# ofsouzap/DistributedMandelbrot

Hardware: AMD Instinct MI355X
Metric: G pixel-iterations/s on 4096^2 tile, max_iter=1000 fp64 (higher is better)
Workload: dtype f64

## Files before the change

distributedmandelbrot_amd/_lib.py:

```python
from __future__ import annotations

import ctypes as C
import importlib.util
import os
import sys

HERE = os.path.dirname(os.path.abspath(__file__))
SO_PATH = os.path.join(HERE, "libmbk_hip.so")

MBK_OK, MBK_ERR_INVALID, MBK_ERR_NO_DEVICE, MBK_ERR_HIP, MBK_ERR_NOMEM, MBK_ERR_NET = range(6)
MBK_WANT_COUNTS = 0x1
MBK_WANT_BYTES = 0x2
MBK_KERNEL_DEFAULT = 0x000
MBK_KERNEL_SIMPLE = 0x100
MBK_KERNEL_ASM = 0x200
MBK_KERNEL_REFILL = 0x300
MBK_KERNEL_GROUP = 0x400
MBK_KERNEL_SCAN = 0x500
KERNELS = {"default": MBK_KERNEL_DEFAULT, "simple": MBK_KERNEL_SIMPLE, "asm": MBK_KERNEL_ASM,
           "refill": MBK_KERNEL_REFILL, "group": MBK_KERNEL_GROUP, "scan": MBK_KERNEL_SCAN}
OPTIONS = {name: i for i, name in enumerate(
    ["order", "waves_per_wg", "group_steps", "exact_steps", "probe_steps", "scan_waves", "scan_xcd_map", "scan_col_period", "heavy_share",
     "rf_livemin", "rf_patience", "rf_batch", "rf_waves", "cycle_detect", "probe_mid", "prepass_overlap", "exact_long", "scan_inline", "wave_limit", "units_min_light", "xcd_balance", "m_late", "h_settled", "classify_wg", "scan_strip", "cycle_window", "spill_first", "spill_lanes", "spill_min_mrd", "spill_min_blocks", "spill_cyc_shift"])}
MBK_PRECISION_F32 = 0x1000
MBK_LAZY_UNIFORM = 0x2000
MBK_DEEP_BLA = 0x8000
PRECISIONS = {"f64": 0, "f32": MBK_PRECISION_F32}
MBK_SLOTS = 4
MBK_WORKER_DEPTH = 3
MBK_INFO_SCAN_WG_PER_CU = 100
MBK_INFO_XCD_SHARE = 110
MBK_INFO_SPILL = 130
MBK_CODEC_RAW = 0x00
MBK_CODEC_RLE = 0x01
MBK_CHUNK_DEFINITION = 4096
MBK_CHUNK_BYTES = 4096 * 4096
MBK_ABI_VERSION = 5
MBK_RENDER_BYTES = 0
MBK_RENDER_SMOOTH = 1
MBK_RENDER_DISTANCE = 3
MBK_RENDER_DISTANCE_REL = 4
MBK_RENDER_EQUALIZED = 5
RENDER_SOURCES = {"bytes": MBK_RENDER_BYTES, "smooth": MBK_RENDER_SMOOTH, "distance": MBK_RENDER_DISTANCE,
                  "distance_rel": MBK_RENDER_DISTANCE_REL, "equalized": MBK_RENDER_EQUALIZED}
MBK_HISTOGRAM_MAX_MRD = 1 << 20
RENDER_SUPERSAMPLES = (1, 2, 3, 4, 8)
MBK_RENDER_BAND_BYTES = 256 << 20
MBK_STREAM_OK, MBK_STREAM_BAD_CODEC, MBK_STREAM_BAD_SIZE, MBK_STREAM_ZERO_RUN, MBK_STREAM_TOO_LONG, MBK_STREAM_TOO_SHORT = range(6)
STREAM_REASONS = {MBK_STREAM_OK: "MBK_STREAM_OK", MBK_STREAM_BAD_CODEC: "MBK_STREAM_BAD_CODEC", MBK_STREAM_BAD_SIZE: "MBK_STREAM_BAD_SIZE",
                  MBK_STREAM_ZERO_RUN: "MBK_STREAM_ZERO_RUN", MBK_STREAM_TOO_LONG: "MBK_STREAM_TOO_LONG",
                  MBK_STREAM_TOO_SHORT: "MBK_STREAM_TOO_SHORT"}
CHUNK_SCALES = (1, 2, 4, 8, 16, 32, 64)
MBK_DENSITY_MAX_CELLS = 1 << 28
MBK_DENSITY_LINEAR = 0
MBK_DENSITY_SQRT = 1
DENSITY_MODES = {"linear": MBK_DENSITY_LINEAR, "sqrt": MBK_DENSITY_SQRT}
DENSITY_FACTORS = (1, 2, 4, 8)


class mbk_view(C.Structure):
    _fields_ = [("start_r", C.c_double), ("start_i", C.c_double),
                ("range_r", C.c_double), ("range_i", C.c_double),
                ("width", C.c_uint32), ("height", C.c_uint32),
                ("col0", C.c_uint32), ("row0", C.c_uint32),
                ("ncols", C.c_uint32), ("nrows", C.c_uint32)]


class mbk_deep_view(C.Structure):
    _fields_ = [("range_r", C.c_double), ("range_i", C.c_double),
                ("width", C.c_uint32), ("height", C.c_uint32),
                ("col0", C.c_uint32), ("row0", C.c_uint32),
                ("ncols", C.c_uint32), ("nrows", C.c_uint32)]


class mbk_deep_xview(C.Structure):
    _fields_ = [("range_r", C.c_double), ("range_i", C.c_double), ("exp2", C.c_int32),
                ("width", C.c_uint32), ("height", C.c_uint32),
                ("col0", C.c_uint32), ("row0", C.c_uint32),
                ("ncols", C.c_uint32), ("nrows", C.c_uint32)]


class mbk_render_spec(C.Structure):
    _fields_ = [("source", C.c_uint32), ("supersample", C.c_uint32), ("palette", C.c_void_p),
                ("palette_len", C.c_uint32), ("inside", C.c_uint8 * 4),
                ("scale", C.c_double), ("offset", C.c_double), ("max_band_rows", C.c_uint32)]


class mbk_chunk_spec(C.Structure):
    _fields_ = [("palette", C.c_void_p), ("scale", C.c_uint32)]


class mbk_interior_render_spec(C.Structure):
    _fields_ = [("supersample", C.c_uint32), ("palette", C.c_void_p), ("palette_len", C.c_uint32),
                ("unknown", C.c_uint8 * 4), ("outside", C.c_uint8 * 4), ("scale", C.c_double), ("max_band_rows", C.c_uint32)]


class mbk_density_target(C.Structure):
    _fields_ = [("start_r", C.c_double), ("start_i", C.c_double), ("range_r", C.c_double), ("range_i", C.c_double),
                ("width", C.c_uint32), ("height", C.c_uint32)]


class mbk_density_stats(C.Structure):
    _fields_ = [("deposits", C.c_uint64), ("dropped", C.c_uint64)]


class mbk_density_render_spec(C.Structure):
    _fields_ = [("mode", C.c_uint32), ("factor", C.c_uint32), ("palette", C.c_void_p), ("palette_len", C.c_uint32),
                ("scale", C.c_double), ("offset", C.c_double)]


class mbk_stats(C.Structure):
    _fields_ = [("kernel_ms", C.c_float), ("d2h_ms", C.c_float),
                ("pixel_iterations", C.c_uint64), ("never_pixels", C.c_uint64),
                ("all_bytes_zero", C.c_uint32), ("all_bytes_one", C.c_uint32),
                ("rle_runs", C.c_uint64)]


class mbk_device_info(C.Structure):
    _fields_ = [("name", C.c_char * 128), ("arch", C.c_char * 64),
                ("compute_units", C.c_int), ("clock_mhz", C.c_int),
                ("wavefront_size", C.c_int), ("total_mem", C.c_uint64)]


class mbk_worker_report(C.Structure):
    _fields_ = [("leased", C.c_uint64), ("accepted", C.c_uint64), ("rejected", C.c_uint64), ("resets", C.c_uint64),
                ("uniform_tiles", C.c_uint64), ("pixel_iterations", C.c_uint64),
                ("kernel_ms_sum", C.c_double), ("seconds", C.c_double), ("net_retries", C.c_uint64)]


NET_OPTIONS = {name: i for i, name in enumerate(
    ["max_connections", "connect_timeout_ms", "io_timeout_ms", "retries", "backoff_ms", "stop", "peak_connections", "feeder_slots"])}


FEEDER_SUBMIT = C.CFUNCTYPE(C.c_int, C.c_void_p, C.c_int, C.c_uint32, C.c_uint32, C.c_uint32, C.c_uint32, C.c_void_p)
FEEDER_WAIT = C.CFUNCTYPE(C.c_int, C.c_void_p, C.c_int, C.POINTER(mbk_stats))
FEEDER_ALLOC = C.CFUNCTYPE(C.c_void_p, C.c_void_p, C.c_uint64)
FEEDER_RELEASE = C.CFUNCTYPE(None, C.c_void_p, C.c_void_p)
FEEDER_ON_TILE = C.CFUNCTYPE(None, C.c_void_p, C.POINTER(C.c_uint32 * 4), C.POINTER(mbk_stats), C.c_int)


class mbk_feeder_ops(C.Structure):
    _fields_ = [("user", C.c_void_p), ("submit", FEEDER_SUBMIT), ("wait", FEEDER_WAIT), ("alloc", FEEDER_ALLOC),
                ("release", FEEDER_RELEASE), ("on_tile", FEEDER_ON_TILE)]


SIGNATURES = {
    "mbk_abi_version": (C.c_int, []),
    "mbk_device_count": (C.c_int, [C.POINTER(C.c_int)]),
    "mbk_create": (C.c_int, [C.c_int, C.POINTER(C.c_void_p)]),
    "mbk_destroy": (None, [C.c_void_p]),
    "mbk_last_error": (C.c_char_p, [C.c_void_p]),
    "mbk_get_device_info": (C.c_int, [C.c_void_p, C.POINTER(mbk_device_info)]),
    "mbk_device_pci_bus_id": (C.c_int, [C.c_void_p, C.c_char_p, C.c_int]),
    "mbk_host_alloc": (C.c_int, [C.c_void_p, C.c_uint64, C.POINTER(C.c_void_p)]),
    "mbk_host_free": (C.c_int, [C.c_void_p, C.c_void_p]),
    "mbk_datachunk_geometry": (C.c_int, [C.c_uint32, C.c_uint32, C.c_uint32,
                                         C.POINTER(C.c_double), C.POINTER(C.c_double),
                                         C.POINTER(C.c_double)]),
    "mbk_view_outside_circle": (C.c_int, [C.POINTER(mbk_view), C.c_uint32, C.POINTER(C.c_int)]),
    "mbk_view_needs_literal_doubling": (C.c_int, [C.POINTER(mbk_view), C.c_uint32, C.POINTER(C.c_int)]),
    "mbk_view_launch": (C.c_int, [C.c_void_p, C.POINTER(mbk_view), C.c_uint32, C.c_uint32,
                                  C.c_void_p, C.c_void_p, C.c_void_p]),
    "mbk_view_compute": (C.c_int, [C.c_void_p, C.POINTER(mbk_view), C.c_uint32, C.c_uint32,
                                   C.c_void_p, C.c_void_p, C.POINTER(mbk_stats)]),
    "mbk_datachunk": (C.c_int, [C.c_void_p, C.c_uint32, C.c_uint32, C.c_uint32, C.c_uint32,
                                C.c_void_p, C.c_void_p, C.POINTER(mbk_stats)]),
    "mbk_view_launch_smooth": (C.c_int, [C.c_void_p, C.POINTER(mbk_view), C.c_uint32, C.c_uint32,
                                         C.c_void_p, C.c_void_p, C.c_void_p]),
    "mbk_view_compute_smooth": (C.c_int, [C.c_void_p, C.POINTER(mbk_view), C.c_uint32, C.c_uint32,
                                          C.c_void_p, C.c_void_p, C.POINTER(mbk_stats)]),
    "mbk_view_launch_distance": (C.c_int, [C.c_void_p, C.POINTER(mbk_view), C.c_uint32, C.c_uint32,
                                           C.c_void_p, C.c_void_p, C.c_void_p]),
    "mbk_view_compute_distance": (C.c_int, [C.c_void_p, C.POINTER(mbk_view), C.c_uint32, C.c_uint32,
                                            C.c_void_p, C.c_void_p, C.POINTER(mbk_stats)]),
    "mbk_distance_value_host": (C.c_double, [C.c_double, C.c_double, C.c_int32]),
    "mbk_datachunk_submit": (C.c_int, [C.c_void_p, C.c_int, C.c_uint32, C.c_uint32, C.c_uint32, C.c_uint32,
                                       C.c_void_p, C.c_void_p]),
    "mbk_datachunk_submit_ex": (C.c_int, [C.c_void_p, C.c_int, C.c_uint32, C.c_uint32, C.c_uint32, C.c_uint32,
                                          C.c_void_p, C.c_void_p, C.c_uint32]),
    "mbk_view_submit": (C.c_int, [C.c_void_p, C.c_int, C.POINTER(mbk_view), C.c_uint32, C.c_uint32,
                                  C.c_void_p, C.c_void_p]),
    "mbk_wait": (C.c_int, [C.c_void_p, C.c_int, C.POINTER(mbk_stats)]),
    "mbk_serialize_last": (C.c_int, [C.c_void_p, C.c_void_p, C.c_uint64, C.POINTER(C.c_uint64),
                                     C.POINTER(C.c_uint32)]),
    "mbk_set_option": (C.c_int, [C.c_void_p, C.c_int, C.c_uint32]),
    "mbk_get_option": (C.c_int, [C.c_void_p, C.c_int, C.POINTER(C.c_uint32)]),
    "mbk_quantise_counts": (C.c_int, [C.c_void_p, C.c_void_p, C.c_uint64, C.c_uint32, C.c_void_p]),
    "mbk_units_plan": (C.c_int, [C.c_uint32, C.c_uint32, C.c_uint32, C.c_void_p, C.c_void_p]),
    "mbk_units_lookup": (C.c_int, [C.c_void_p, C.c_uint32, C.c_void_p, C.c_void_p]),
    "mbk_reduce_counts": (C.c_int, [C.c_void_p, C.c_void_p, C.c_uint64, C.c_uint32, C.c_void_p,
                                    C.POINTER(mbk_stats)]),
    "mbk_worker_run": (C.c_int, [C.c_void_p, C.c_char_p, C.c_uint16, C.c_uint64, C.c_uint32,
                                 C.POINTER(mbk_worker_report)]),
    "mbk_net_set_option": (C.c_int, [C.c_int, C.c_uint32]),
    "mbk_net_get_option": (C.c_int, [C.c_int, C.POINTER(C.c_uint32)]),
    "mbk_feeder_run": (C.c_int, [C.POINTER(mbk_feeder_ops), C.c_char_p, C.c_uint16, C.c_uint64, C.c_uint32,
                                 C.POINTER(mbk_worker_report)]),
    "mbk_deep_orbit_create": (C.c_int, [C.c_char_p, C.c_char_p, C.c_uint32, C.c_uint32, C.POINTER(C.c_void_p)]),
    "mbk_deep_orbit_destroy": (None, [C.c_void_p]),
    "mbk_deep_orbit_info": (C.c_int, [C.c_void_p, C.POINTER(C.c_uint32), C.POINTER(C.c_uint32), C.POINTER(C.c_uint32),
                                      C.POINTER(C.c_uint32)]),
    "mbk_deep_orbit_read": (C.c_int, [C.c_void_p, C.c_void_p, C.c_void_p, C.c_uint64]),
    "mbk_deep_view_launch": (C.c_int, [C.c_void_p, C.c_void_p, C.POINTER(mbk_deep_view), C.c_uint32, C.c_uint32,
                                       C.c_void_p, C.c_void_p, C.c_void_p, C.c_void_p]),
    "mbk_deep_view_compute": (C.c_int, [C.c_void_p, C.c_void_p, C.POINTER(mbk_deep_view), C.c_uint32, C.c_uint32,
                                        C.c_void_p, C.c_void_p, C.c_void_p, C.POINTER(mbk_stats)]),
    "mbk_deep_view_submit": (C.c_int, [C.c_void_p, C.c_int, C.c_void_p, C.POINTER(mbk_deep_view), C.c_uint32, C.c_uint32,
                                       C.c_void_p, C.c_void_p]),
    "mbk_deep_view_launch_distance": (C.c_int, [C.c_void_p, C.c_void_p, C.POINTER(mbk_deep_view), C.c_uint32, C.c_uint32,
                                                C.c_void_p, C.c_void_p, C.c_void_p]),
    "mbk_deep_view_compute_distance": (C.c_int, [C.c_void_p, C.c_void_p, C.POINTER(mbk_deep_view), C.c_uint32, C.c_uint32,
                                                 C.c_void_p, C.c_void_p, C.POINTER(mbk_stats)]),
    "mbk_deep_distance_value_host": (C.c_double, [C.c_double, C.c_double, C.c_int32, C.c_double, C.c_int32]),
    "mbk_deep_bla_info": (C.c_int, [C.c_void_p, C.POINTER(mbk_deep_view), C.POINTER(C.c_uint32), C.POINTER(C.c_uint64)]),
    "mbk_deep_bla_read": (C.c_int, [C.c_void_p, C.POINTER(mbk_deep_view), C.c_uint32, C.c_void_p, C.c_void_p, C.c_void_p,
                                    C.c_void_p, C.c_void_p, C.c_uint64]),
    "mbk_deep_bla_count_host": (C.c_int, [C.c_void_p, C.POINTER(mbk_deep_view), C.c_uint32, C.c_uint32, C.c_uint32,
                                          C.POINTER(C.c_int32), C.POINTER(C.c_double), C.POINTER(C.c_uint64)]),
    "mbk_deep_orbit_read_wide": (C.c_int, [C.c_void_p, C.c_void_p, C.c_void_p, C.c_void_p, C.c_uint64]),
    "mbk_deep_xview_launch": (C.c_int, [C.c_void_p, C.c_void_p, C.POINTER(mbk_deep_xview), C.c_uint32, C.c_uint32,
                                        C.c_void_p, C.c_void_p, C.c_void_p, C.c_void_p]),
    "mbk_deep_xview_compute": (C.c_int, [C.c_void_p, C.c_void_p, C.POINTER(mbk_deep_xview), C.c_uint32, C.c_uint32,
                                         C.c_void_p, C.c_void_p, C.c_void_p, C.POINTER(mbk_stats)]),
    "mbk_deep_xview_submit": (C.c_int, [C.c_void_p, C.c_int, C.c_void_p, C.POINTER(mbk_deep_xview), C.c_uint32, C.c_uint32,
                                        C.c_void_p, C.c_void_p]),
    "mbk_deep_xview_count_host": (C.c_int, [C.c_void_p, C.POINTER(mbk_deep_xview), C.c_uint32, C.c_uint32, C.c_uint32,
                                            C.POINTER(C.c_int32), C.POINTER(C.c_double)]),
    "mbk_deep_xview_render_launch": (C.c_int, [C.c_void_p, C.c_void_p, C.POINTER(mbk_deep_xview), C.c_uint32, C.c_uint32,
                                               C.POINTER(mbk_render_spec), C.c_void_p, C.c_void_p]),
    "mbk_deep_xview_render_compute": (C.c_int, [C.c_void_p, C.c_void_p, C.POINTER(mbk_deep_xview), C.c_uint32, C.c_uint32,
                                                C.POINTER(mbk_render_spec), C.c_void_p, C.POINTER(mbk_stats)]),
    "mbk_deep_xview_render_equalized_launch": (C.c_int, [C.c_void_p, C.c_void_p, C.POINTER(mbk_deep_xview), C.c_uint32, C.c_uint32,
                                                         C.POINTER(mbk_render_spec), C.c_void_p, C.c_uint32, C.c_void_p,
                                                         C.c_void_p]),
    "mbk_deep_xview_render_equalized_compute": (C.c_int, [C.c_void_p, C.c_void_p, C.POINTER(mbk_deep_xview), C.c_uint32,
                                                          C.c_uint32, C.POINTER(mbk_render_spec), C.c_void_p, C.c_uint32,
                                                          C.c_void_p, C.POINTER(mbk_stats)]),
    "mbk_deep_xview_histogram_launch": (C.c_int, [C.c_void_p, C.c_void_p, C.POINTER(mbk_deep_xview), C.c_uint32, C.c_uint32,
                                                  C.c_void_p, C.c_void_p]),
    "mbk_deep_xview_histogram_compute": (C.c_int, [C.c_void_p, C.c_void_p, C.POINTER(mbk_deep_xview), C.c_uint32, C.c_uint32,
                                                   C.c_void_p, C.POINTER(mbk_stats)]),
    "mbk_view_render_launch": (C.c_int, [C.c_void_p, C.POINTER(mbk_view), C.c_uint32, C.c_uint32,
                                         C.POINTER(mbk_render_spec), C.c_void_p, C.c_void_p]),
    "mbk_view_render_compute": (C.c_int, [C.c_void_p, C.POINTER(mbk_view), C.c_uint32, C.c_uint32,
                                          C.POINTER(mbk_render_spec), C.c_void_p, C.POINTER(mbk_stats)]),
    "mbk_deep_view_render_launch": (C.c_int, [C.c_void_p, C.c_void_p, C.POINTER(mbk_deep_view), C.c_uint32, C.c_uint32,
                                              C.POINTER(mbk_render_spec), C.c_void_p, C.c_void_p]),
    "mbk_deep_view_render_compute": (C.c_int, [C.c_void_p, C.c_void_p, C.POINTER(mbk_deep_view), C.c_uint32, C.c_uint32,
                                               C.POINTER(mbk_render_spec), C.c_void_p, C.POINTER(mbk_stats)]),
    "mbk_palette_viewer": (C.c_int, [C.c_void_p]),
    "mbk_render_resolve_host": (C.c_int, [C.POINTER(mbk_render_spec), C.c_uint32, C.c_uint32, C.c_void_p, C.c_void_p,
                                          C.c_void_p, C.c_void_p]),
    "mbk_counts_histogram": (C.c_int, [C.c_void_p, C.c_void_p, C.c_uint64, C.c_uint32, C.c_void_p, C.c_void_p]),
    "mbk_view_histogram_launch": (C.c_int, [C.c_void_p, C.POINTER(mbk_view), C.c_uint32, C.c_uint32, C.c_void_p, C.c_void_p]),
    "mbk_deep_view_histogram_launch": (C.c_int, [C.c_void_p, C.c_void_p, C.POINTER(mbk_deep_view), C.c_uint32, C.c_uint32,
                                                 C.c_void_p, C.c_void_p]),
    "mbk_view_histogram_compute": (C.c_int, [C.c_void_p, C.POINTER(mbk_view), C.c_uint32, C.c_uint32, C.c_void_p,
                                             C.POINTER(mbk_stats)]),
    "mbk_deep_view_histogram_compute": (C.c_int, [C.c_void_p, C.c_void_p, C.POINTER(mbk_deep_view), C.c_uint32, C.c_uint32,
                                                  C.c_void_p, C.POINTER(mbk_stats)]),
    "mbk_counts_histogram_host": (C.c_int, [C.c_void_p, C.c_uint64, C.c_uint32, C.c_void_p]),
    "mbk_equalize_lut_host": (C.c_int, [C.c_void_p, C.c_uint32, C.c_void_p]),
    "mbk_equalize_value_host": (C.c_double, [C.c_void_p, C.c_uint32, C.c_double]),
    "mbk_view_render_equalized_launch": (C.c_int, [C.c_void_p, C.POINTER(mbk_view), C.c_uint32, C.c_uint32,
                                                   C.POINTER(mbk_render_spec), C.c_void_p, C.c_uint32, C.c_void_p, C.c_void_p]),
    "mbk_view_render_equalized_compute": (C.c_int, [C.c_void_p, C.POINTER(mbk_view), C.c_uint32, C.c_uint32,
                                                    C.POINTER(mbk_render_spec), C.c_void_p, C.c_uint32, C.c_void_p,
                                                    C.POINTER(mbk_stats)]),
    "mbk_deep_view_render_equalized_launch": (C.c_int, [C.c_void_p, C.c_void_p, C.POINTER(mbk_deep_view), C.c_uint32, C.c_uint32,
                                                        C.POINTER(mbk_render_spec), C.c_void_p, C.c_uint32, C.c_void_p,
                                                        C.c_void_p]),
    "mbk_deep_view_render_equalized_compute": (C.c_int, [C.c_void_p, C.c_void_p, C.POINTER(mbk_deep_view), C.c_uint32, C.c_uint32,
                                                         C.POINTER(mbk_render_spec), C.c_void_p, C.c_uint32, C.c_void_p,
                                                         C.POINTER(mbk_stats)]),
    "mbk_render_resolve_equalized_host": (C.c_int, [C.POINTER(mbk_render_spec), C.c_void_p, C.c_uint32, C.c_uint32, C.c_uint32,
                                                    C.c_void_p, C.c_void_p, C.c_void_p]),
    "mbk_julia_view_launch": (C.c_int, [C.c_void_p, C.POINTER(mbk_view), C.c_double, C.c_double, C.c_uint32, C.c_uint32,
                                        C.c_void_p, C.c_void_p, C.c_void_p, C.c_void_p]),
    "mbk_julia_view_compute": (C.c_int, [C.c_void_p, C.POINTER(mbk_view), C.c_double, C.c_double, C.c_uint32, C.c_uint32,
                                         C.c_void_p, C.c_void_p, C.c_void_p, C.POINTER(mbk_stats)]),
    "mbk_julia_view_submit": (C.c_int, [C.c_void_p, C.c_int, C.POINTER(mbk_view), C.c_double, C.c_double, C.c_uint32, C.c_uint32,
                                        C.c_void_p, C.c_void_p]),
    "mbk_julia_view_render_launch": (C.c_int, [C.c_void_p, C.POINTER(mbk_view), C.c_double, C.c_double, C.c_uint32, C.c_uint32,
                                               C.POINTER(mbk_render_spec), C.c_void_p, C.c_void_p]),
    "mbk_julia_view_render_compute": (C.c_int, [C.c_void_p, C.POINTER(mbk_view), C.c_double, C.c_double, C.c_uint32, C.c_uint32,
                                                C.POINTER(mbk_render_spec), C.c_void_p, C.POINTER(mbk_stats)]),
    "mbk_julia_view_render_equalized_launch": (C.c_int, [C.c_void_p, C.POINTER(mbk_view), C.c_double, C.c_double, C.c_uint32,
                                                         C.c_uint32, C.POINTER(mbk_render_spec), C.c_void_p, C.c_uint32,
                                                         C.c_void_p, C.c_void_p]),
    "mbk_julia_view_render_equalized_compute": (C.c_int, [C.c_void_p, C.POINTER(mbk_view), C.c_double, C.c_double, C.c_uint32,
                                                          C.c_uint32, C.POINTER(mbk_render_spec), C.c_void_p, C.c_uint32,
                                                          C.c_void_p, C.POINTER(mbk_stats)]),
    "mbk_julia_view_histogram_launch": (C.c_int, [C.c_void_p, C.POINTER(mbk_view), C.c_double, C.c_double, C.c_uint32, C.c_uint32,
                                                  C.c_void_p, C.c_void_p]),
    "mbk_julia_view_histogram_compute": (C.c_int, [C.c_void_p, C.POINTER(mbk_view), C.c_double, C.c_double, C.c_uint32, C.c_uint32,
                                                   C.c_void_p, C.POINTER(mbk_stats)]),
    "mbk_julia_count_host": (C.c_int, [C.c_double, C.c_double, C.c_double, C.c_double, C.c_uint32, C.POINTER(C.c_int32),
                                       C.POINTER(C.c_double)]),
    "mbk_view_interior_launch": (C.c_int, [C.c_void_p, C.POINTER(mbk_view), C.c_uint32, C.c_uint32, C.c_void_p, C.c_void_p,
                                           C.c_void_p, C.c_void_p]),
    "mbk_view_interior_compute": (C.c_int, [C.c_void_p, C.POINTER(mbk_view), C.c_uint32, C.c_uint32, C.c_void_p, C.c_void_p,
                                            C.c_void_p, C.POINTER(mbk_stats)]),
    "mbk_interior_host": (C.c_int, [C.c_double, C.c_double, C.c_uint32, C.POINTER(C.c_int32), C.POINTER(C.c_int32),
                                    C.POINTER(C.c_int32), C.POINTER(C.c_double)]),
    "mbk_view_interior_render_launch": (C.c_int, [C.c_void_p, C.POINTER(mbk_view), C.c_uint32, C.c_uint32,
                                                  C.POINTER(mbk_interior_render_spec), C.c_void_p, C.c_void_p]),
    "mbk_view_interior_render_compute": (C.c_int, [C.c_void_p, C.POINTER(mbk_view), C.c_uint32, C.c_uint32,
                                                   C.POINTER(mbk_interior_render_spec), C.c_void_p, C.POINTER(mbk_stats)]),
    "mbk_interior_resolve_host": (C.c_int, [C.POINTER(mbk_interior_render_spec), C.c_uint32, C.c_uint32, C.c_void_p, C.c_void_p,
                                            C.c_void_p, C.c_void_p]),
    "mbk_view_density_launch": (C.c_int, [C.c_void_p, C.POINTER(mbk_view), C.POINTER(mbk_density_target), C.c_uint32, C.c_uint32,
                                          C.c_uint32, C.c_uint32, C.c_void_p, C.c_void_p]),
    "mbk_view_density_compute": (C.c_int, [C.c_void_p, C.POINTER(mbk_view), C.POINTER(mbk_density_target), C.c_uint32, C.c_uint32,
                                           C.c_uint32, C.c_uint32, C.c_void_p, C.POINTER(mbk_stats),
                                           C.POINTER(mbk_density_stats)]),
    "mbk_density_max": (C.c_int, [C.c_void_p, C.c_void_p, C.c_uint64, C.POINTER(C.c_uint32), C.POINTER(C.c_uint64), C.c_void_p]),
    "mbk_density_render_launch": (C.c_int, [C.c_void_p, C.c_void_p, C.c_uint32, C.c_uint32, C.POINTER(mbk_density_render_spec),
                                            C.c_void_p, C.c_void_p]),
    "mbk_density_render_compute": (C.c_int, [C.c_void_p, C.c_void_p, C.c_uint32, C.c_uint32, C.POINTER(mbk_density_render_spec),
                                             C.c_void_p, C.POINTER(mbk_stats)]),
    "mbk_density_cell_host": (C.c_int, [C.POINTER(mbk_density_target), C.c_double, C.c_double, C.POINTER(C.c_uint32),
                                        C.POINTER(C.c_uint32), C.POINTER(C.c_int)]),
    "mbk_density_accumulate_host": (C.c_int, [C.POINTER(mbk_view), C.POINTER(mbk_density_target), C.c_uint32, C.c_uint32, C.c_uint32,
                                              C.c_void_p, C.POINTER(mbk_density_stats)]),
    "mbk_density_resolve_host": (C.c_int, [C.POINTER(mbk_density_render_spec), C.c_uint32, C.c_uint32, C.c_void_p, C.c_void_p]),
    "mbk_density_build_info": (C.c_int, []),
    "mbk_chunk_stream_check": (C.c_int, [C.c_void_p, C.c_uint64, C.c_uint64, C.POINTER(C.c_uint32), C.POINTER(C.c_uint64),
                                         C.POINTER(C.c_uint32)]),
    "mbk_chunk_decode_host": (C.c_int, [C.c_void_p, C.c_uint64, C.c_uint64, C.c_void_p]),
    "mbk_chunk_resolve_host": (C.c_int, [C.POINTER(mbk_chunk_spec), C.c_void_p, C.c_void_p, C.c_uint64]),
    "mbk_chunk_decode_launch": (C.c_int, [C.c_void_p, C.c_void_p, C.c_uint64, C.c_uint64, C.c_void_p, C.c_void_p, C.c_void_p]),
    "mbk_chunk_render_launch": (C.c_int, [C.c_void_p, C.c_void_p, C.c_uint64, C.POINTER(mbk_chunk_spec), C.c_void_p, C.c_uint64,
                                          C.c_void_p, C.c_void_p]),
    "mbk_chunk_decode_compute": (C.c_int, [C.c_void_p, C.c_void_p, C.c_uint64, C.c_uint64, C.c_void_p, C.POINTER(mbk_stats)]),
    "mbk_chunk_render_compute": (C.c_int, [C.c_void_p, C.c_void_p, C.c_uint64, C.POINTER(mbk_chunk_spec), C.c_void_p, C.c_uint64,
                                           C.POINTER(mbk_stats)]),
}

_lib = None


def _share_hip_runtime_with_torch() -> None:
# ... 35 lines not shown
```

distributedmandelbrot_amd/csrc/mbk_api.hip:

```cpp
#include "../../include/mbk.h"

#include <hip/hip_runtime.h>

#include <cmath>
#include <cstdio>
#include <cstdlib>
#include <algorithm>
#include <cstring>
#include <new>
#include <string>
#include <vector>

#include "mbk_kernels.h"
#include "mbk_refill.h"
#include "mbk_persist.h"
#include "mbk_scan.h"
#include "mbk_units.h"
#include "mbk_spill.h"
#include "mbk_feeder.h"
#include "mbk_deep_orbit.h"
#include "mbk_deep.h"
#include "mbk_deep_bla.h"
#include "mbk_deep_wide.h"
#include "mbk_histogram.h"
#include "mbk_render.h"
#include "mbk_chunks.h"
#include "mbk_distance.h"
#include "mbk_interior.h"
#include "mbk_deep_distance.h"
#include "mbk_julia.h"
#include "mbk_density.h"

using mbk::Axis;
using mbk::ReduceOut;
using mbk::ReduceSlot;
using mbk::TileArgs;
using mbk::WorkQueues;

static const int kOrderRing = 3;

struct OrderRing {
    uint32_t *d_order[kOrderRing] = {};
    uint32_t *d_ctl = nullptr;
    bool ctl_dirty = true;
    size_t order_cap = 0;
    unsigned order_turn = 0;
    hipStream_t aux = nullptr;
    uint32_t aux_prio = 0;
    int pp_last = -1;
    hipEvent_t ev_cls[kOrderRing] = {};
    hipEvent_t ev_done[kOrderRing] = {};
    bool done_valid[kOrderRing] = {};

    void drop_lists()
    {
        for (int k = 0; k < kOrderRing; ++k) {
            if (d_order[k]) (void)hipFree(d_order[k]);
            d_order[k] = nullptr;
            done_valid[k] = false;
        }
        order_cap = 0;
    }
    void drop_aux()
    {
        if (aux) (void)hipStreamDestroy(aux);
        aux = nullptr;
        for (int k = 0; k < kOrderRing; ++k) {
            if (ev_cls[k]) (void)hipEventDestroy(ev_cls[k]);
            if (ev_done[k]) (void)hipEventDestroy(ev_done[k]);
            ev_cls[k] = ev_done[k] = nullptr;
            done_valid[k] = false;
        }
    }
    void release()
    {
        if (aux) (void)hipStreamSynchronize(aux);
        drop_lists();
        drop_aux();
        if (d_ctl) (void)hipFree(d_ctl);
        *this = OrderRing();
    }
};

struct SpillBuffers {
    void *d_z = nullptr;
    uint32_t *d_meta = nullptr, *d_cnt = nullptr, *d_chunks = nullptr, *d_src = nullptr;
    unsigned long long *d_total = nullptr;
    size_t cap_slots = 0, cap_blocks = 0;

    void release()
    {
        for (void *q : {d_z, (void *)d_meta, (void *)d_cnt, (void *)d_chunks, (void *)d_src, (void *)d_total})
            if (q) (void)hipFree(q);
        *this = SpillBuffers();
    }
};

struct StreamScratch {
    hipStream_t stream = nullptr;
    OrderRing ring;
    WorkQueues *d_queues = nullptr;
    mbk::ScanCursors *d_cursors = nullptr;
    uint32_t *d_entries = nullptr;
    size_t scan_cap_blocks = 0;
    unsigned scan_turn = 0;
    bool cursors_dirty = false;
    uint32_t *h_hint = nullptr;
    SpillBuffers spill;
    ReduceSlot *d_red = nullptr;
    ReduceSlot *h_red = nullptr;
    unsigned long long *h_stamps = nullptr;
    double xcd_f[8] = {0.125, 0.125, 0.125, 0.125, 0.125, 0.125, 0.125, 0.125};
    uint32_t xcd_issued = 0, xcd_consumed = 0;
    struct SharesUsed { uint32_t seq, switches; float f[8]; } xcd_ring[64] = {};
    void *d_render = nullptr;
    size_t render_cap = 0;
    uint32_t *d_palette = nullptr;
    std::vector<uint32_t> palette;
    uint8_t *d_chunk = nullptr;
    size_t chunk_cap_n = 0;
    uint8_t *d_chunk_bytes = nullptr;
    uint32_t *h_chunk_status = nullptr;
    int32_t *d_dist_counts = nullptr;
    size_t dist_cap_px = 0;
    double *d_lut = nullptr;
    size_t lut_cap = 0;
    std::vector<double> lut;
    uint32_t *d_density_bands = nullptr;
    mbk::DensityMax *d_density_max = nullptr;
};
static const size_t kMaxStreamScratch = 64;
static const uint32_t kStampSlots = 16, kShareRing = 64;

struct Slot {
    hipStream_t stream = nullptr;
    hipEvent_t ev_k0 = nullptr, ev_k1 = nullptr, ev_c0 = nullptr, ev_c1 = nullptr;
    int32_t *d_counts = nullptr;
    uint8_t *d_bytes = nullptr;
    size_t cap_px = 0;
    ReduceSlot *d_red = nullptr;
    ReduceSlot *h_red = nullptr;
    bool busy = false;
    bool with_bytes = false;
    uint8_t *lazy_h_bytes = nullptr;
    size_t lazy_px = 0;
    bool immediate = false;
    mbk_stats imm = {};
};

struct mbk_ctx {
    int device = -1;
    Slot s[MBK_SLOTS];
    std::vector<StreamScratch> scratch;
    size_t last_px = 0;
    double *d_smooth = nullptr;
    size_t smooth_cap_px = 0;
    uint32_t *d_rgba = nullptr;
    size_t rgba_cap_px = 0;
    unsigned long long *d_hist = nullptr;
    size_t hist_cap = 0;
    uint32_t *d_density = nullptr;
    size_t density_cap = 0;
    unsigned long long *d_density_stat = nullptr;
    uint8_t *d_rle = nullptr;
    size_t rle_cap_px = 0;
    uint32_t opt[MBK_OPT_COUNT_];
    hipStream_t last_tile_stream = nullptr;
    uint32_t stream_switches = 0;
    int scan_occ[2][2] = {{0, 0}, {0, 0}};
    int scan_occ_inline[2] = {0, 0};
    uint32_t wave_limit_lds[8] = {0, 0, 0, 0, 0, 0, 0, 0};
    uint32_t spill_launches = 0;
    hipStream_t last_spill_stream = nullptr;
    struct ProbeKey { Axis re, im; uint32_t col0, row0, ncols, nrows; } probe_key = {};
    double probe_share = 0.0;
    bool probe_valid = false;
    struct DeepCopy {
        uint64_t id;
        double4 *d;
        mbk::WideEntry *d_wide;
        bool has_bla;
        uint64_t dcmax_bits;
        double *d_rc;
        double4 *d_ab;
        uint32_t levels;
        uint32_t off[mbk::kBlaMaxLevels];
    };
    std::vector<DeepCopy> deep;
    hipDeviceProp_t prop;
    std::string err;
};

struct mbk_deep_orbit {
    mbk::DeepOrbit o;
};

static thread_local std::string g_err;

static int fail(mbk_ctx *ctx, int code, const std::string &msg)
{
    if (ctx) ctx->err = msg;
    g_err = msg;
    return code;
}

#define MBK_HIP(ctx, call)                                                                  \
    do {                                                                                    \
        hipError_t e_ = (call);                                                             \
        if (e_ != hipSuccess) {                                                             \
            return fail((ctx), MBK_ERR_HIP,                                                 \
                        std::string(#call) + ": " + hipGetErrorString(e_));                 \
        }                                                                                   \
    } while (0)


static Axis make_axis(double start, double range, uint32_t n)
{
    Axis a;
    std::memset(&a, 0, sizeof(a));
    a.start = start;
    a.n = n;
    volatile double stop = start + range;
    if (n <= 1) {
        a.last = start;
        a.div = 1.0;
        return a;
    }
    volatile double delta = stop - start;
    volatile double div = (double)(n - 1);
    volatile double step = delta / div;
    a.last = stop;
    a.delta = delta;
    a.div = div;
    a.step = step;
    a.step_is_zero = (step == 0.0) ? 1u : 0u;
    return a;
}

static double axis_value_host(const Axis &a, uint32_t k)
{
    if (k + 1u == a.n) return a.last;
    volatile double y;
    if (a.step_is_zero) {
        volatile double q = (double)k / a.div;
        y = q * a.delta;
    } else {
        y = (double)k * a.step;
    }
    volatile double v = y + a.start;
    return v;
}

static bool axis_end_is_regular(const Axis &a)
{
    if (a.n <= 1 || a.step_is_zero) return false;
    volatile double y = (double)(a.n - 1u) * a.step;
    volatile double v = y + a.start;
    return v == a.last;
}

static const double kMaxCoord = 0x1p500;
static const double kSafeImagMin = 0x1p-900;

static uint32_t coprime_multiplier(uint32_t n)
{
    if (n < 4) return 1u;
    uint64_t m = (uint64_t)((double)n * 0.6180339887498949);
    if (m < 1) m = 1;
    for (;; ++m) {
        uint64_t a = m, b = n;
        while (b) {
            const uint64_t t = a % b;
            a = b;
            b = t;
        }
        if (a == 1) return (uint32_t)(m % n);
    }
}

static bool axis_has_tiny_nonzero(const Axis &a, uint32_t k0, uint32_t cnt, bool f32)
{
    const double thr = f32 ? 0x1p-100 : kSafeImagMin;
    auto value = [&](uint32_t k) { const double y = axis_value_host(a, k); return f32 ? (double)(float)y : y; };
    auto tiny = [&](double y) { return y != 0.0 && std::fabs(y) < thr; };
    if (cnt == 0) return false;
    uint32_t end = k0 + cnt;
    if (a.n >= 1u && end == a.n) {
        if (tiny(value(a.n - 1u))) return true;
        if (--end == k0) return false;
    }
    const double first = value(k0), last = value(end - 1u);
    if (tiny(first) || tiny(last)) return true;
    if ((first > 0.0 && last > 0.0) || (first < 0.0 && last < 0.0) || first == last) return false;
    const double s = last > first ? 1.0 : -1.0;
    auto lower = [&](bool strict) {
        uint32_t lo = k0, hi = end;
        while (lo < hi) {
            const uint32_t mid = lo + (hi - lo) / 2u;
            const double y = s * value(mid);
            if (strict ? y > 0.0 : y >= 0.0) hi = mid;
            else lo = mid + 1u;
        }
        return lo;
    };
    const uint32_t ge = lower(false), gt = lower(true);
    if (ge > k0 && tiny(value(ge - 1u))) return true;
    if (gt < end && tiny(value(gt))) return true;
    return false;
}

static int validate_view(mbk_ctx *ctx, const mbk_view *v, bool *safe_doubling, bool f32 = false)
{
    if (!v) return fail(ctx, MBK_ERR_INVALID, "view is NULL");
    if (v->width == 0 || v->height == 0) return fail(ctx, MBK_ERR_INVALID, "empty view");
    if (v->ncols == 0 || v->nrows == 0) return fail(ctx, MBK_ERR_INVALID, "empty window");
    if ((uint64_t)v->col0 + v->ncols > v->width || (uint64_t)v->row0 + v->nrows > v->height)
        return fail(ctx, MBK_ERR_INVALID, "window exceeds the view");
    if ((uint64_t)v->ncols * v->nrows > (1ull << 31))
        return fail(ctx, MBK_ERR_INVALID, "window larger than 2^31 pixels");
    const double vals[6] = {v->start_r, v->start_i, v->range_r, v->range_i,
                            v->start_r + v->range_r, v->start_i + v->range_i};
    const double max_coord = f32 ? 0x1p60 : kMaxCoord;
    for (double x : vals)
        if (!std::isfinite(x) || std::fabs(x) > max_coord)
            return fail(ctx, MBK_ERR_INVALID, f32 ? "view coordinates must be finite and |x| <= 2^60 (fp32)"
// ... 13 lines not shown

static void free_scratch(StreamScratch &sc)
{
    sc.ring.release();
    sc.spill.release();
    if (sc.d_queues) (void)hipFree(sc.d_queues);
    if (sc.d_cursors) (void)hipFree(sc.d_cursors);
    if (sc.d_entries) (void)hipFree(sc.d_entries);
    if (sc.h_hint) (void)hipHostFree(sc.h_hint);
    if (sc.h_stamps) (void)hipHostFree(sc.h_stamps);
    if (sc.d_red) (void)hipFree(sc.d_red);
    if (sc.h_red) (void)hipHostFree(sc.h_red);
    if (sc.d_render) (void)hipFree(sc.d_render);
    if (sc.d_palette) (void)hipFree(sc.d_palette);
    if (sc.d_chunk) (void)hipFree(sc.d_chunk);
    if (sc.d_chunk_bytes) (void)hipFree(sc.d_chunk_bytes);
    if (sc.h_chunk_status) (void)hipHostFree(sc.h_chunk_status);
    if (sc.d_dist_counts) (void)hipFree(sc.d_dist_counts);
    if (sc.d_lut) (void)hipFree(sc.d_lut);
    if (sc.d_density_bands) (void)hipFree(sc.d_density_bands);
    if (sc.d_density_max) (void)hipFree(sc.d_density_max);
    sc = StreamScratch();
}

static int get_scratch(mbk_ctx *ctx, hipStream_t stream, StreamScratch **out)
{
    for (StreamScratch &sc : ctx->scratch)
        if (sc.stream == stream) {
            *out = &sc;
            return MBK_OK;
        }
    if (ctx->scratch.size() >= kMaxStreamScratch) {
        MBK_HIP(ctx, hipDeviceSynchronize());
        for (StreamScratch &sc : ctx->scratch) free_scratch(sc);
        ctx->scratch.clear();
    }
    ctx->scratch.emplace_back();
    StreamScratch &sc = ctx->scratch.back();
    sc.stream = stream;
    *out = &sc;
    MBK_HIP(ctx, hipHostMalloc((void **)&sc.h_hint, 2 * sizeof(uint32_t), hipHostMallocDefault));
    sc.h_hint[0] = sc.h_hint[1] = 0xffffffffu;
    return MBK_OK;
}

static void set_window_facts(TileArgs &a, bool f32);
static void shares_from_fractions(const double *f, uint32_t *cum);
static double window_heavy_share(const TileArgs &a);
static double window_heavy_share(mbk_ctx *ctx, const TileArgs &a);

static void xcd_shares_update(const mbk_ctx *ctx, StreamScratch &sc)
{
    const unsigned long long kMask = 0xffffffffffffull;
    uint32_t first = sc.xcd_issued >= kStampSlots ? sc.xcd_issued - kStampSlots + 1u : 1u;
    first = std::max(first, sc.xcd_consumed + 1u);
    for (uint32_t c = first; c <= sc.xcd_issued; ++c) {
        const volatile unsigned long long *st = sc.h_stamps + (size_t)(c % kStampSlots) * mbk::kStampWords;
        const StreamScratch::SharesUsed &used = sc.xcd_ring[c % kShareRing];
        if (used.seq != c) continue;
        const StreamScratch::SharesUsed &before = sc.xcd_ring[(c - 1u) % kShareRing], &after = sc.xcd_ring[(c + 1u) % kShareRing];
        const bool alone = c > 1u && before.seq == c - 1u && before.switches == used.switches &&
                           (c == sc.xcd_issued ? ctx->stream_switches == used.switches : after.seq == c + 1u && after.switches == used.switches);
        unsigned long long v[mbk::kStampWords];
        bool whole = true;
        for (uint32_t i = 0; i < mbk::kStampWords; ++i) {
            v[i] = st[i];
            whole = whole && (v[i] >> 48) == (c & 0xffffu);
        }
        if (!whole) continue;
        unsigned long long start = v[0] & kMask;
        for (uint32_t x = 1; x < 8u; ++x)
            if ((((v[x] & kMask) - start) & kMask) >> 47) start = v[x] & kMask;
        double T[8], tmin = 1e300, tmax = 0.0, speed[8], sum = 0.0;
        for (uint32_t x = 0; x < 8u; ++x) {
            unsigned long long last = 0;
            for (uint32_t t = 0; t < mbk::kStampTail; ++t)
                last = std::max(last, ((v[8u + x * mbk::kStampTail + t] & kMask) - start) & kMask);
            T[x] = (double)last;
            tmin = std::min(tmin, T[x]);
            tmax = std::max(tmax, T[x]);
        }
        sc.xcd_consumed = c;
        if (!alone || tmin < 1000.0 || tmax > 1.25 * tmin) continue;
        for (uint32_t x = 0; x < 8u; ++x) {
            speed[x] = (double)used.f[x] / T[x];
            sum += speed[x];
        }
        double fs = 0.0;
        for (uint32_t x = 0; x < 8u; ++x) {
            const double f = 0.7 * sc.xcd_f[x] + 0.3 * speed[x] / sum;
            sc.xcd_f[x] = std::min(0.14, std::max(0.11, f));
            fs += sc.xcd_f[x];
        }
        for (uint32_t x = 0; x < 8u; ++x) sc.xcd_f[x] /= fs;
    }
}

struct FuseStats { ReduceSlot *slots; bool counts_unwanted; bool fused; };

static uint32_t quant_table4(int32_t mrd, bool want_bytes)
{
    uint32_t qtab = 0u;
    if (want_bytes && mrd > 0)
        for (uint32_t c = 1; c <= 4u; ++c)
            qtab |= (uint32_t)(((uint64_t)c * 256u + (uint32_t)mrd - 1u) / (uint32_t)mrd & 0xffu) << (8u * (c - 1u));
    return qtab;
}

struct BlockLaunchPlan {
    uint32_t wpw, by;
    dim3 grid, block;
    uint32_t order_mode, probe_steps;
    bool cyc, units, ordered;
    double unit_share;
};

static BlockLaunchPlan block_launch_plan(mbk_ctx *ctx, TileArgs &a, uint32_t kernel, bool safe, bool f32)
{
    BlockLaunchPlan p;
    p.wpw = ctx->opt[MBK_OPT_WAVES_PER_WG];
    a.blocks_x = (a.ncols + 8u * p.wpw - 1u) / (8u * p.wpw);
    p.by = (a.nrows + 7u) / 8u;
    set_window_facts(a, f32);
    p.cyc = ctx->opt[MBK_OPT_CYCLE_DETECT] != 0u;
    p.grid = dim3(a.blocks_x * p.by);
    p.block = dim3(64u * p.wpw);
    p.order_mode = ctx->opt[MBK_OPT_ORDER];
    p.probe_steps = ctx->opt[MBK_OPT_PROBE_STEPS];
    a.perm_mul = p.order_mode == 1 ? coprime_multiplier(p.grid.x) : 1u;
    a.order = nullptr;
    p.units = p.order_mode == 3 && p.wpw == 1u && kernel == MBK_KERNEL_GROUP && !safe && a.smooth == nullptr &&
              (a.counts || a.bytes) && !(a.bytes && a.quant_wide) && a.blocks_x % 8u == 0u && a.blocks_x <= 2048u &&
              a.fast_bx_end > 0u && a.fast_by_end > 0u && (f32 || ctx->opt[MBK_OPT_GROUP_STEPS] == 16u) &&
              p.grid.x >= 16384u && (uint32_t)a.mrd > 2u * p.probe_steps && p.by <= 0xffffu;
    p.unit_share = 0.0;
    if (p.units) {
        p.unit_share = window_heavy_share(ctx, a);
        p.units = (1.0 - p.unit_share) * 65536.0 >= (double)ctx->opt[MBK_OPT_UNITS_MIN_LIGHT];
    }
    p.ordered = p.order_mode >= 2 && p.grid.x >= 16384u && (uint32_t)a.mrd > 2u * p.probe_steps && a.blocks_x <= 0xffffu && p.by <= 0xffffu;
    return p;
}

struct OrderList {
    StreamScratch *sc = nullptr;
    unsigned k = 0;
    uint32_t *list = nullptr;
    hipStream_t pre = nullptr;
    bool overlap = false;
    bool whole = false;
    ~OrderList() { if (sc && !whole) sc->ring.ctl_dirty = true; }
};

static int acquire_order_list(mbk_ctx *ctx, hipStream_t stream, uint32_t nblocks, OrderList *out)
{
    StreamScratch *sc = nullptr;
    int rc = get_scratch(ctx, stream, &sc);
    if (rc != MBK_OK) return rc;
    OrderRing &ring = sc->ring;
    const uint32_t pp_mode = ctx->opt[MBK_OPT_PREPASS_OVERLAP];
    const bool overlap = pp_mode != 0u;
    const uint32_t want_prio = pp_mode == 2u ? 2u : 1u;
    if (ring.pp_last != (int)pp_mode) {
        if (ring.pp_last >= 0) {
            MBK_HIP(ctx, hipStreamSynchronize(stream));
            if (ring.aux) MBK_HIP(ctx, hipStreamSynchronize(ring.aux));
        }
        for (int k = 0; k < kOrderRing; ++k) ring.done_valid[k] = false;
        ring.pp_last = (int)pp_mode;
    }
    if (overlap && ring.aux && ring.aux_prio != want_prio) {
        MBK_HIP(ctx, hipStreamSynchronize(stream));
        MBK_HIP(ctx, hipStreamSynchronize(ring.aux));
        ring.drop_aux();
    }
    if (overlap && !ring.aux) {
        if (want_prio == 2u) {
            int least = 0, greatest = 0;
            MBK_HIP(ctx, hipDeviceGetStreamPriorityRange(&least, &greatest));
            MBK_HIP(ctx, hipStreamCreateWithPriority(&ring.aux, hipStreamNonBlocking, greatest));
        } else {
            MBK_HIP(ctx, hipStreamCreateWithFlags(&ring.aux, hipStreamNonBlocking));
        }
        ring.aux_prio = want_prio;
        for (int k = 0; k < kOrderRing; ++k) {
            MBK_HIP(ctx, hipEventCreateWithFlags(&ring.ev_cls[k], hipEventDisableTiming));
            MBK_HIP(ctx, hipEventCreateWithFlags(&ring.ev_done[k], hipEventDisableTiming));
        }
    }
    if (nblocks > ring.order_cap) {
        MBK_HIP(ctx, hipStreamSynchronize(stream));
        if (ring.aux) MBK_HIP(ctx, hipStreamSynchronize(ring.aux));
        ring.drop_lists();
        for (int k = 0; k < kOrderRing; ++k)
            MBK_HIP(ctx, hipMalloc((void **)&ring.d_order[k], mbk::units_list_words(nblocks) * sizeof(uint32_t)));
        ring.order_cap = nblocks;
    }
    const unsigned k = ring.order_turn++ % (unsigned)kOrderRing;
    if (overlap && ring.done_valid[k]) MBK_HIP(ctx, hipStreamWaitEvent(ring.aux, ring.ev_done[k], 0));
    out->k = k;
    out->list = ring.d_order[k];
    out->pre = overlap ? ring.aux : stream;
    out->overlap = overlap;
    out->sc = sc;
    return MBK_OK;
}

static int enqueue_units_prepass(mbk_ctx *ctx, TileArgs &a, const BlockLaunchPlan &p, const OrderList &ol, hipStream_t stream)
{
    StreamScratch *sc = ol.sc;
    OrderRing &ring = sc->ring;
    const uint32_t hs = p.cyc ? ctx->opt[MBK_OPT_H_SETTLED] : 0u;
    const double settle_thr = hs ? std::pow(10.0, -(double)hs) : 0.0;
    if (!ring.d_ctl) {
        MBK_HIP(ctx, hipMalloc((void **)&ring.d_ctl, (size_t)kOrderRing * 8u * sizeof(uint32_t)));
        ring.ctl_dirty = true;
    }
    if (ring.ctl_dirty) {
        if (ring.aux) MBK_HIP(ctx, hipStreamSynchronize(ring.aux));
        MBK_HIP(ctx, hipStreamSynchronize(stream));
        MBK_HIP(ctx, hipMemsetAsync(ring.d_ctl, 0, (size_t)kOrderRing * 8u * sizeof(uint32_t), ol.pre));
        ring.ctl_dirty = false;
    }
    uint32_t *ctl = ring.d_ctl + 8u * ol.k;
    const uint32_t balance = ctx->opt[MBK_OPT_XCD_BALANCE] == 1u && (p.cyc || ctx->prop.multiProcessorCount != 256)
                                 ? 0u : ctx->opt[MBK_OPT_XCD_BALANCE];
    static const double kUneven[8] = {0.110, 0.140, 0.125, 0.120, 0.130, 0.125, 0.115, 0.135};
    if (balance == 1u && !sc->h_stamps) {
        MBK_HIP(ctx, hipHostMalloc((void **)&sc->h_stamps, (size_t)kStampSlots * mbk::kStampWords * sizeof(unsigned long long),
                                   hipHostMallocDefault));
        std::memset(sc->h_stamps, 0xff, (size_t)kStampSlots * mbk::kStampWords * sizeof(unsigned long long));
    }
    if (balance == 1u) xcd_shares_update(ctx, *sc);
    mbk::XcdShares w;
    double f[8];
    const uint32_t seq = ++sc->xcd_issued;
    StreamScratch::SharesUsed &used = sc->xcd_ring[seq % kShareRing];
    used.seq = seq;
    used.switches = ctx->stream_switches;
    for (uint32_t x = 0; x < 8u; ++x) {
        f[x] = balance == 1u ? sc->xcd_f[x] : (balance == 2u ? kUneven[x] : 0.125);
        used.f[x] = (float)f[x];
    }
    shares_from_fractions(f, w.cum);
    a.plan = ol.list + ((2u * (size_t)p.grid.x + 5u + 15u) & ~(size_t)15u);
    a.stamps = balance == 1u ? sc->h_stamps + (size_t)(seq % kStampSlots) * mbk::kStampWords : nullptr;
    a.stamp_tag = seq & 0xffffu;
    const uint32_t cwg = ctx->opt[MBK_OPT_CLASSIFY_WG];
    hipLaunchKernelGGL(mbk::classify_units_kernel, dim3((p.grid.x + cwg - 1u) / cwg), dim3(cwg), 0, ol.pre, a, p.grid.x,
                       (int32_t)p.probe_steps, ol.list, ctl, (int32_t)ctx->opt[MBK_OPT_M_LATE], settle_thr, ctl + 3, (uint32_t *)a.plan, w,
                       a.stamps ? 1u : 0u);
    return MBK_OK;
}

static int enqueue_classify_prepass(mbk_ctx *ctx, const TileArgs &a, const BlockLaunchPlan &p, const OrderList &ol, bool *mid_first)
{
    const uint32_t nblocks = p.grid.x;
    uint32_t *cursors = ol.list + nblocks;
    MBK_HIP(ctx, hipMemsetAsync(cursors, 0, 3 * sizeof(uint32_t), ol.pre));
    *mid_first = p.order_mode == 3 && ctx->opt[MBK_OPT_PROBE_MID] > p.probe_steps && ctx->opt[MBK_OPT_M_LATE] >= 2u &&
                 ctx->opt[MBK_OPT_M_LATE] <= p.probe_steps;
    hipLaunchKernelGGL(mbk::classify_blocks_kernel, dim3((nblocks + 1023u) / 1024u), dim3(1024), 0, ol.pre, a,
                       nblocks, 8u * p.wpw, (int32_t)p.probe_steps, (int32_t)(*mid_first ? ctx->opt[MBK_OPT_M_LATE] : ctx->opt[MBK_OPT_PROBE_MID]),
                       ol.list, cursors);
    return MBK_OK;
}

static bool spill_wanted(const mbk_ctx *ctx, const TileArgs &a, const BlockLaunchPlan &p, uint32_t kernel, bool safe, bool f32)
{
    const uint32_t spill_first = ctx->opt[MBK_OPT_SPILL_FIRST], spill_lanes = ctx->opt[MBK_OPT_SPILL_LANES];
    return !p.units && a.order != nullptr && p.order_mode >= 2u && kernel == MBK_KERNEL_GROUP && !safe && a.smooth == nullptr && p.wpw == 1u &&
           (a.counts || a.bytes) && spill_first != 0u && (f32 || ctx->opt[MBK_OPT_GROUP_STEPS] == 16u) &&
           (uint32_t)a.mrd >= ctx->opt[MBK_OPT_SPILL_MIN_MRD] && (uint32_t)a.mrd < (1u << 26) &&
           ((uint64_t)p.grid.x >> ctx->opt[MBK_OPT_SPILL_MIN_BLOCKS]) != 0ull &&
           (uint64_t)a.mrd > (uint64_t)ctx->opt[MBK_OPT_EXACT_STEPS] + spill_first + 66u &&
           (uint64_t)p.grid.x * spill_lanes < (1ull << 32) && a.fast_bx_end > 0u && a.fast_by_end > 0u;
}

static int acquire_spill(mbk_ctx *ctx, StreamScratch *sc, hipStream_t stream, TileArgs &a, uint32_t nblocks, SpillBuffers **out)
{
    SpillBuffers &sp = sc->spill;
    const uint32_t spill_lanes = ctx->opt[MBK_OPT_SPILL_LANES];
    const size_t slots = (size_t)nblocks * spill_lanes, nchunks = (nblocks + mbk::kSpillChunk - 1u) / mbk::kSpillChunk;
    *out = nullptr;
    if (slots > sp.cap_slots || nblocks > sp.cap_blocks) {
        MBK_HIP(ctx, hipStreamSynchronize(stream));
        sp.release();
        const bool got = hipMalloc(&sp.d_z, slots * 16u) == hipSuccess &&
                         hipMalloc((void **)&sp.d_meta, slots * sizeof(uint32_t)) == hipSuccess &&
                         hipMalloc((void **)&sp.d_src, slots * sizeof(uint32_t)) == hipSuccess &&
                         hipMalloc((void **)&sp.d_cnt, (size_t)nblocks * sizeof(uint32_t)) == hipSuccess &&
                         hipMalloc((void **)&sp.d_chunks, (nchunks * mbk::kSpillLevels + 1u) * sizeof(uint32_t)) == hipSuccess &&
                         hipMalloc((void **)&sp.d_total, sizeof(unsigned long long)) == hipSuccess;
        if (got) {
            sp.cap_slots = slots;
            sp.cap_blocks = nblocks;
        } else {
            (void)hipGetLastError();
            sp.release();
        }
    }
    if (sp.cap_slots >= slots && sp.cap_blocks >= nblocks && sp.d_z) {
        a.spill_first = ctx->opt[MBK_OPT_SPILL_FIRST];
        a.spill_lanes = spill_lanes;
        a.spill_win_shift = ctx->opt[MBK_OPT_SPILL_CYC_SHIFT];
        a.spill_z = sp.d_z;
        a.spill_meta = sp.d_meta;
        a.spill_cnt = sp.d_cnt;
        MBK_HIP(ctx, hipMemsetAsync(sp.d_cnt, 0, (size_t)nblocks * sizeof(uint32_t), stream));
        *out = &sp;
    }
    return MBK_OK;
}

typedef void (*UnitsKernel)(TileArgs, uint32_t);
typedef void (*BlockKernel)(TileArgs);
typedef void (*SpillKernel)(TileArgs, const uint32_t *, const unsigned long long *, uint32_t);

static UnitsKernel pick_units_kernel(bool f32, bool cyc, bool stats, bool counts, bool bytes)
{
    static const UnitsKernel forms[4][4] = {
        {mbk::tile_units_kernel<float, 8, true, false, true, true>, mbk::tile_units_kernel<float, 8, true, true, true>,
         mbk::tile_units_kernel<float, 8, true, false, true>, mbk::tile_units_kernel<float, 8, true, true, false>},
        {mbk::tile_units_kernel<float, 8, false, false, true, true>, mbk::tile_units_kernel<float, 8, false, true, true>,
         mbk::tile_units_kernel<float, 8, false, false, true>, mbk::tile_units_kernel<float, 8, false, true, false>},
        {mbk::tile_units_kernel<double, 16, true, false, true, true>, mbk::tile_units_kernel<double, 16, true, true, true>,
         mbk::tile_units_kernel<double, 16, true, false, true>, mbk::tile_units_kernel<double, 16, true, true, false>},
        {mbk::tile_units_kernel<double, 16, false, false, true, true>, mbk::tile_units_kernel<double, 16, false, true, true>,
         mbk::tile_units_kernel<double, 16, false, false, true>, mbk::tile_units_kernel<double, 16, false, true, false>},
    };
    return forms[(f32 ? 0 : 2) + (cyc ? 0 : 1)][stats ? 0 : (counts && bytes) ? 1 : bytes ? 2 : 3];
}

static BlockKernel pick_block_kernel(uint32_t kernel, bool safe, bool f32, bool cyc, uint32_t group_steps, bool spill)
{
    if (spill && f32 && cyc) return mbk::tile_asm_kernel<float, true, 8, true, true>;
    if (spill && f32) return mbk::tile_asm_kernel<float, true, 8, false, true>;
    if (spill && cyc) return mbk::tile_asm_kernel<double, true, 16, true, true>;
    if (spill) return mbk::tile_asm_kernel<double, true, 16, false, true>;
    if (f32 && safe) return mbk::tile_asm_kernel<float, false, 0>;
    if (f32 && kernel == MBK_KERNEL_ASM) return mbk::tile_asm_kernel<float, true, 0>;
    if (f32 && cyc) return mbk::tile_asm_kernel<float, true, 8, true>;
    if (f32) return mbk::tile_asm_kernel<float, true, 8>;
    if (safe) return mbk::tile_asm_kernel<double, false, 0>;
    if (kernel == MBK_KERNEL_ASM) return mbk::tile_asm_kernel<double, true, 0>;
    if (group_steps == 32 && !cyc) return mbk::tile_asm_kernel<double, true, 32>;
    if (group_steps >= 16 && cyc) return mbk::tile_asm_kernel<double, true, 16, true>;
    if (group_steps >= 16) return mbk::tile_asm_kernel<double, true, 16>;
    if (group_steps == 8 && cyc) return mbk::tile_asm_kernel<double, true, 8, true>;
    if (group_steps == 8) return mbk::tile_asm_kernel<double, true, 8>;
    return mbk::tile_asm_kernel<double, true, 4>;
}

static SpillKernel pick_spill_kernels(bool f32, bool cyc)
{
    if (f32 && cyc) return mbk::tile_spill_kernel<float, true>;
    if (f32) return mbk::tile_spill_kernel<float, false>;
    if (cyc) return mbk::tile_spill_kernel<double, true>;
    return mbk::tile_spill_kernel<double, false>;
}

static void enqueue_units_tile(mbk_ctx *ctx, TileArgs &a, const BlockLaunchPlan &p, bool f32, uint32_t lds, hipStream_t stream, FuseStats *fuse)
{
    const double est = (double)p.grid.x * (p.unit_share + (1.0 - p.unit_share) / 8.0);
    const uint32_t cus = (uint32_t)ctx->prop.multiProcessorCount;
    uint32_t g = (uint32_t)std::min<double>((double)p.grid.x, est * 1.15 + 2048.0);
    g = (std::max(std::max(g, std::min(p.grid.x, cus * 64u)), 16384u) + 7u) & ~7u;
    a.unit_stride = g;
    const bool stats = fuse != nullptr && fuse->slots != nullptr && fuse->counts_unwanted && a.bytes != nullptr;
    if (stats) {
        a.stats = fuse->slots;
        a.counts = nullptr;
        fuse->fused = true;
    }
    hipLaunchKernelGGL(pick_units_kernel(f32, p.cyc, stats, a.counts != nullptr, a.bytes != nullptr), dim3(g), dim3(64), lds, stream, a,
                       quant_table4(a.mrd, a.bytes != nullptr));
}

static int enqueue_spill_second_pass(mbk_ctx *ctx, const TileArgs &a, const SpillBuffers &sp, uint32_t nblocks, bool f32, bool cyc, hipStream_t stream)
{
    const uint32_t nchunks = (nblocks + mbk::kSpillChunk - 1u) / mbk::kSpillChunk;
    hipLaunchKernelGGL(mbk::spill_count_kernel, dim3(nchunks), dim3(mbk::kSpillChunk), 0, stream, sp.d_cnt, nblocks, nchunks, sp.d_chunks);
    hipLaunchKernelGGL(mbk::rle_scan_kernel, dim3(1), dim3(1024), 0, stream, sp.d_chunks, nchunks * mbk::kSpillLevels, sp.d_total);
    hipLaunchKernelGGL(mbk::spill_expand_kernel, dim3(nchunks), dim3(mbk::kSpillChunk), 0, stream, sp.d_cnt, nblocks, nchunks,
                       sp.d_chunks, a.spill_lanes, sp.d_src);
    const uint32_t nwg = (uint32_t)std::min<uint64_t>(((uint64_t)nblocks * a.spill_lanes + 63u) / 64u, 16384u);
    const uint32_t lds2 = 0u;
    hipLaunchKernelGGL(pick_spill_kernels(f32, cyc), dim3(nwg), dim3(64), lds2, stream, a, sp.d_src, sp.d_total, nwg);
    MBK_HIP(ctx, hipGetLastError());
    ++ctx->spill_launches;
    ctx->last_spill_stream = stream;
    return MBK_OK;
}

static int launch_blocks(mbk_ctx *ctx, TileArgs a, uint32_t kernel, bool safe, bool f32, hipStream_t stream, FuseStats *fuse = nullptr)
{
    const BlockLaunchPlan p = block_launch_plan(ctx, a, kernel, safe, f32);
    OrderList ol;
    if (p.ordered) {
        int rc = acquire_order_list(ctx, stream, p.grid.x, &ol);
        if (rc != MBK_OK) return rc;
        OrderRing &ring = ol.sc->ring;
        bool mid_first = false;
        rc = p.units ? enqueue_units_prepass(ctx, a, p, ol, stream) : enqueue_classify_prepass(ctx, a, p, ol, &mid_first);
        if (rc != MBK_OK) return rc;
        if (ol.overlap) {
            MBK_HIP(ctx, hipEventRecord(ring.ev_cls[ol.k], ring.aux));
            MBK_HIP(ctx, hipStreamWaitEvent(stream, ring.ev_cls[ol.k], 0));
        }
        a.order = ol.list;
        a.ngrid = p.grid.x;
        a.order_mid = mid_first ? 2u : (ctx->opt[MBK_OPT_PROBE_MID] <= p.probe_steps ? 1u : 0u);
    }
    SpillBuffers *spill = nullptr;
    if (spill_wanted(ctx, a, p, kernel, safe, f32)) {
        const int rc = acquire_spill(ctx, ol.sc, stream, a, p.grid.x, &spill);
        if (rc != MBK_OK) return rc;
    }
    const uint32_t lds = p.wpw == 1u ? ctx->wave_limit_lds[ctx->opt[MBK_OPT_WAVE_LIMIT] & 7u] : 0u;
    if (p.units && a.order)
        enqueue_units_tile(ctx, a, p, f32, lds, stream, fuse);
    else
        hipLaunchKernelGGL(pick_block_kernel(kernel, safe, f32, p.cyc, ctx->opt[MBK_OPT_GROUP_STEPS], spill != nullptr), p.grid, p.block, lds, stream, a);
    const hipError_t e = hipGetLastError();
    if (e != hipSuccess) return fail(ctx, MBK_ERR_HIP, std::string("tile launch: ") + hipGetErrorString(e));
    if (ol.overlap) {
        MBK_HIP(ctx, hipEventRecord(ol.sc->ring.ev_done[ol.k], stream));
        ol.sc->ring.done_valid[ol.k] = true;
    }
    if (spill) {
        const int rc = enqueue_spill_second_pass(ctx, a, *spill, p.grid.x, f32, p.cyc, stream);
        if (rc != MBK_OK) return rc;
    }
    ol.whole = true;
    return MBK_OK;
}

static bool window_may_touch_ring(const TileArgs &a, double margin = 1e-6)
{
    const double x0 = axis_value_host(a.re, a.col0), x1 = axis_value_host(a.re, a.col0 + a.ncols - 1u);
    const double y0 = axis_value_host(a.im, a.row0), y1 = axis_value_host(a.im, a.row0 + a.nrows - 1u);
    const double xlo = std::fmin(x0, x1), xhi = std::fmax(x0, x1), ylo = std::fmin(y0, y1), yhi = std::fmax(y0, y1);
    const double dx = (xlo <= 0.0 && 0.0 <= xhi) ? 0.0 : std::fmin(std::fabs(xlo), std::fabs(xhi));
    const double dy = (ylo <= 0.0 && 0.0 <= yhi) ? 0.0 : std::fmin(std::fabs(ylo), std::fabs(yhi));
    const double fx = std::fmax(std::fabs(xlo), std::fabs(xhi)), fy = std::fmax(std::fabs(ylo), std::fabs(yhi));
    const double rmin2 = dx * dx + dy * dy, rmax2 = fx * fx + fy * fy;
    return !(rmax2 < 4.0 - margin || rmin2 > 4.0 + margin);
}

static void set_window_facts(TileArgs &a, bool f32)
{
    a.ring_possible = window_may_touch_ring(a, f32 ? 2e-3 : 1e-6) ? 1u : 0u;
    a.fast_bx_end = a.fast_by_end = 0u;
    if (a.re.step_is_zero || a.im.step_is_zero) return;
    const uint64_t re_n = (uint64_t)a.re.n - (axis_end_is_regular(a.re) ? 0u : 1u), im_n = (uint64_t)a.im.n - (axis_end_is_regular(a.im) ? 0u : 1u);
    const uint64_t cols_ok = std::min<uint64_t>(a.ncols, re_n - std::min<uint64_t>(a.col0, re_n));
    const uint64_t rows_ok = std::min<uint64_t>(a.nrows, im_n - std::min<uint64_t>(a.row0, im_n));
    a.fast_bx_end = (uint32_t)(cols_ok / 8u);
    a.fast_by_end = (uint32_t)(rows_ok / 8u);
}

static int launch_refill(mbk_ctx *ctx, const TileArgs &a, bool safe, hipStream_t stream)
{
    const bool eligible = !safe && a.mrd >= 2 && a.counts != nullptr && !a.re.step_is_zero &&
                          !a.im.step_is_zero && !window_may_touch_ring(a, 1e-6);
    const uint32_t cols_ok = a.re.n > 0 ? std::min<uint64_t>(a.ncols, (uint64_t)(a.re.n - 1u) - std::min<uint64_t>(a.col0, a.re.n - 1u)) : 0u;
    const uint32_t rows_ok = a.im.n > 0 ? std::min<uint64_t>(a.nrows, (uint64_t)(a.im.n - 1u) - std::min<uint64_t>(a.row0, a.im.n - 1u)) : 0u;
    const uint32_t icols = eligible ? (cols_ok / 8u) * 8u : 0u, irows = eligible ? (rows_ok / 8u) * 8u : 0u;
    if (icols == 0 || irows == 0) return launch_blocks(ctx, a, MBK_KERNEL_GROUP, safe, false, stream);

    mbk::PersistArgs q;
    std::memset(&q, 0, sizeof(q));
    q.re_start = a.re.start;
    q.re_step = a.re.step;
    q.im_start = a.im.start;
    q.im_step = a.im.step;
    q.col0 = a.col0;
    q.row0 = a.row0;
    q.pitch = a.out_pitch;
    q.bxn = icols / 8u;
    q.nblocks = q.bxn * (irows / 8u);
    q.total = (uint32_t)a.mrd - 1u;
    q.livemin = ctx->opt[MBK_OPT_RF_LIVEMIN];
    q.patience = ctx->opt[MBK_OPT_RF_PATIENCE];
    q.batch = ctx->opt[MBK_OPT_RF_BATCH];
    q.counts = a.counts;
    StreamScratch *sc = nullptr;
    int rcs = get_scratch(ctx, stream, &sc);
    if (rcs != MBK_OK) return rcs;
    if (!sc->d_queues) MBK_HIP(ctx, hipMalloc((void **)&sc->d_queues, sizeof(WorkQueues)));
    WorkQueues *wq = sc->d_queues;
    hipLaunchKernelGGL(mbk::init_queues_kernel, dim3(1), dim3(64), 0, stream, wq, q.nblocks);
    uint32_t waves = (uint32_t)ctx->prop.multiProcessorCount * 4u * ctx->opt[MBK_OPT_RF_WAVES];
    if (waves > q.nblocks) waves = q.nblocks;
    hipLaunchKernelGGL(mbk::tile_persist_kernel, dim3((waves + 3u) / 4u), dim3(256), 0, stream, q, wq);
    MBK_HIP(ctx, hipGetLastError());
    TileArgs e = a;
    e.bytes = nullptr;
    if (icols < a.ncols) {
        e.col0 = a.col0 + icols;
        e.ncols = a.ncols - icols;
        e.out_col0 = a.out_col0 + icols;
        int rc = launch_blocks(ctx, e, MBK_KERNEL_GROUP, safe, false, stream);
        if (rc != MBK_OK) return rc;
    }
    if (irows < a.nrows) {
        e = a;
        e.bytes = nullptr;
        e.ncols = icols;
        e.row0 = a.row0 + irows;
        e.nrows = a.nrows - irows;
        e.out_row0 = a.out_row0 + irows;
        int rc = launch_blocks(ctx, e, MBK_KERNEL_GROUP, safe, false, stream);
        if (rc != MBK_OK) return rc;
    }
    if (a.bytes) {
        const uint64_t npx = (uint64_t)a.ncols * a.nrows;
        hipLaunchKernelGGL(mbk::quantise_kernel, dim3(2048), dim3(256), 0, stream, a.counts, a.bytes, npx, a.mrd,
                           a.quant_wide, a.quant_rcp);
        MBK_HIP(ctx, hipGetLastError());
    }
    return MBK_OK;
}

static double window_heavy_share(const TileArgs &a)
{
    const uint32_t k = 16;
    uint32_t inside = 0;
    for (uint32_t j = 0; j < k; ++j) {
        const double ci = axis_value_host(a.im, a.row0 + (uint32_t)(((uint64_t)(2u * j + 1u) * a.nrows) / (2u * k)));
        for (uint32_t i = 0; i < k; ++i) {
            const double cr = axis_value_host(a.re, a.col0 + (uint32_t)(((uint64_t)(2u * i + 1u) * a.ncols) / (2u * k)));
            double zr = cr, zi = ci;
            bool in = true;
            for (int n = 0; n < 4 && in; ++n) {
                const double t = zr * zr - zi * zi + cr;
                zi = 2.0 * zr * zi + ci;
                zr = t;
                in = zr * zr + zi * zi < 4.0;
            }
            inside += in ? 1u : 0u;
        }
    }
    return (double)inside / (double)(k * k);
}

static double window_heavy_share(mbk_ctx *ctx, const TileArgs &a)
{
    mbk_ctx::ProbeKey k;
    std::memset(&k, 0, sizeof(k));
    k.re = a.re;
    k.im = a.im;
    k.col0 = a.col0;
    k.row0 = a.row0;
    k.ncols = a.ncols;
    k.nrows = a.nrows;
    if (ctx->probe_valid && std::memcmp(&k, &ctx->probe_key, sizeof(k)) == 0) return ctx->probe_share;
// ... 466 lines not shown
        case Target::kDeep: set_geometry(p.deep, p.g); break;
        case Target::kJulia:
        case Target::kPlain: set_geometry(p.view, p.g); break;
    }
    return p;
}

struct BandPlan {
    uint32_t ncols, nrows, tile_cols, band_rows;
    size_t cap_px() const { return (size_t)tile_cols * band_rows; }
};

static BandPlan band_plan(uint32_t ncols, uint32_t nrows, uint64_t bytes_per_px, uint32_t max_rows = 0u)
{
    const uint64_t budget = MBK_RENDER_BAND_BYTES - 1024u;
    BandPlan p = {ncols, nrows, ncols, 1u};
    if ((uint64_t)ncols * bytes_per_px <= budget)
        p.band_rows = (uint32_t)std::min<uint64_t>(nrows, budget / ((uint64_t)ncols * bytes_per_px));
    else
        p.tile_cols = (uint32_t)(budget / bytes_per_px);
    if (max_rows) p.band_rows = std::min(p.band_rows, max_rows);
    return p;
}

template <typename Piece>
static int for_each_band(mbk_ctx *ctx, const BandPlan &p, const int32_t *d_counts, uint64_t samples_per_px, uint32_t mrd,
                         hipStream_t stream, Slot *stat, Piece piece)
{
    for (uint32_t r = 0; r < p.nrows; r += p.band_rows) {
        const uint32_t nr = std::min(p.band_rows, p.nrows - r);
        for (uint32_t c = 0; c < p.ncols; c += p.tile_cols) {
            const uint32_t nc = std::min(p.tile_cols, p.ncols - c);
            const bool is_last = r + nr == p.nrows && c + nc == p.ncols;
            int rc = piece(r, c, nr, nc, is_last);
            if (rc != MBK_OK) return rc;
            if (stat) {
                if (is_last) MBK_HIP(ctx, hipEventRecord(stat->ev_k1, stream));
                rc = launch_reduce(ctx, stat->d_red, stat->h_red, d_counts, nullptr, (uint64_t)nc * nr * samples_per_px, mrd, stream, false);
                if (rc != MBK_OK) return rc;
            }
        }
    }
    return MBK_OK;
}


static double deep_step(double range, uint32_t n)
{
    if (n <= 1u) return 0.0;
    volatile double s = range / (double)(n - 1u);
    return s;
}

static double deep_dc(uint32_t k, uint32_t n, double range)
{
    volatile double dc = ((double)k - (double)(n - 1u) * 0.5) * deep_step(range, n);
    return dc;
}

template <typename V>
static bool deep_ranges_within(const V *v, double lo)
{
    for (double r : {v->range_r, v->range_i})
        if (!std::isfinite(r) || !(r >= lo) || !(r <= 4.0)) return false;
    return true;
}

template <typename V, typename FlagRules, typename RangeRules>
static int validate_deep_view(mbk_ctx *ctx, const mbk_deep_orbit *orbit, const V *v, uint32_t mrd, uint32_t flags, FlagRules flag_rules,
                              RangeRules range_rules)
{
    if (!orbit) return fail(ctx, MBK_ERR_INVALID, "orbit is NULL");
    if (!v) return fail(ctx, MBK_ERR_INVALID, "view is NULL");
    int rc = flag_rules();
    if (rc != MBK_OK) return rc;
    if (v->width == 0 || v->height == 0) return fail(ctx, MBK_ERR_INVALID, "empty view");
    if (v->ncols == 0 || v->nrows == 0) return fail(ctx, MBK_ERR_INVALID, "empty window");
    if ((uint64_t)v->col0 + v->ncols > v->width || (uint64_t)v->row0 + v->nrows > v->height)
        return fail(ctx, MBK_ERR_INVALID, "window exceeds the view");
    if ((uint64_t)v->ncols * v->nrows > (1ull << 31)) return fail(ctx, MBK_ERR_INVALID, "window larger than 2^31 pixels");
    rc = range_rules();
    if (rc != MBK_OK) return rc;
    if (mrd > orbit->o.mrd) return fail(ctx, MBK_ERR_INVALID, "mrd exceeds the mrd the reference orbit was computed for");
    if ((flags & MBK_WANT_BYTES) && mrd == 0) return fail(ctx, MBK_ERR_INVALID, "mrd == 0 has no quantised form (division by zero)");
    return MBK_OK;
}

template <typename Args, typename V>
static void fill_deep_window(Args &a, const V *v, uint32_t mrd)
{
    a.half_r = (double)(v->width - 1u) * 0.5;
    a.half_i = (double)(v->height - 1u) * 0.5;
    a.step_r = deep_step(v->range_r, v->width);
    a.step_i = deep_step(v->range_i, v->height);
    a.col0 = v->col0;
    a.row0 = v->row0;
    a.ncols = v->ncols;
    a.nrows = v->nrows;
    a.blocks_x = (v->ncols + 7u) / 8u;
    a.mrd = (int32_t)mrd;
}

template <typename Args>
static void fill_outputs(Args &a, uint32_t mrd, int32_t *d_counts, uint8_t *d_bytes, double *d_smooth)
{
    a.quant_wide = (mrd >= (1u << 23)) ? 1u : 0u;
    a.quant_rcp = mrd ? 1.0 / (double)mrd : 0.0;
    a.counts = d_counts;
    a.bytes = d_bytes;
    a.smooth = d_smooth;
}

template <typename Args>
static dim3 block_grid(const Args &a) { return dim3(a.blocks_x * ((a.nrows + 7u) / 8u)); }


extern "C" {

int mbk_abi_version(void) { return MBK_ABI_VERSION; }

int mbk_device_count(int *count)
{
    if (!count) return fail(nullptr, MBK_ERR_INVALID, "count is NULL");
    int n = 0;
    hipError_t e = hipGetDeviceCount(&n);
    if (e != hipSuccess) {
        *count = 0;
        return fail(nullptr, MBK_ERR_NO_DEVICE, std::string("hipGetDeviceCount: ") + hipGetErrorString(e));
    }
    *count = n;
    return MBK_OK;
}

int mbk_create(int device, mbk_ctx **out)
{
    if (!out) return fail(nullptr, MBK_ERR_INVALID, "out is NULL");
    *out = nullptr;
    int n = 0;
    hipError_t e = hipGetDeviceCount(&n);
    if (e != hipSuccess || n <= 0)
        return fail(nullptr, MBK_ERR_NO_DEVICE,
                    std::string("no HIP device visible (") + hipGetErrorString(e) +
                        "); libmbk_hip has no CPU fallback");
    if (device < 0 || device >= n) return fail(nullptr, MBK_ERR_NO_DEVICE, "device index out of range");
    mbk_ctx *ctx = new (std::nothrow) mbk_ctx();
    if (!ctx) return fail(nullptr, MBK_ERR_NOMEM, "out of host memory");
    ctx->device = device;
    static const uint32_t kDefaults[MBK_OPT_COUNT_] = {
         3u,  1u,  16u,  8u,  32u,
         8u,  1u,  4u,  655u,
         48u,  256u,  1u,  8u,  1u,
         65537u,  1u,  0u,  1u,  0u,
         32768u,  0u,  8u,  6u,  1024u,
         1u,  32u,  256u,  16u,  2048u,  19u,  5u};
    std::memcpy(ctx->opt, kDefaults, sizeof(kDefaults));
#define MBK_CREATE_HIP(call)                                                        \
    do {                                                                            \
        hipError_t e2_ = (call);                                                    \
        if (e2_ != hipSuccess) {                                                    \
            fail(nullptr, MBK_ERR_HIP, std::string(#call) + ": " + hipGetErrorString(e2_)); \
            mbk_destroy(ctx);                                                       \
            return MBK_ERR_HIP;                                                     \
        }                                                                           \
    } while (0)
    MBK_CREATE_HIP(hipSetDevice(device));
    MBK_CREATE_HIP(hipGetDeviceProperties(&ctx->prop, device));
    if (std::strncmp(ctx->prop.gcnArchName, "gfx950", 6) != 0) {
        fail(nullptr, MBK_ERR_NO_DEVICE,
             std::string("device is ") + ctx->prop.gcnArchName + ", this library is built for gfx950 only");
        mbk_destroy(ctx);
        return MBK_ERR_NO_DEVICE;
    }
    for (Slot &sl : ctx->s) {
        MBK_CREATE_HIP(hipStreamCreateWithFlags(&sl.stream, hipStreamNonBlocking));
        MBK_CREATE_HIP(hipEventCreate(&sl.ev_k0));
        MBK_CREATE_HIP(hipEventCreate(&sl.ev_k1));
        MBK_CREATE_HIP(hipEventCreate(&sl.ev_c0));
        MBK_CREATE_HIP(hipEventCreate(&sl.ev_c1));
        MBK_CREATE_HIP(hipMalloc((void **)&sl.d_red, sizeof(ReduceSlot) * mbk::kReduceSlots));
        MBK_CREATE_HIP(hipHostMalloc((void **)&sl.h_red, sizeof(ReduceSlot) * mbk::kReduceSlots, hipHostMallocDefault));
    }
    {
        const void *fns[2][2] = {{(const void *)mbk::tile_light_kernel<double, true, true>, (const void *)mbk::tile_todo_kernel<double>},
                                 {(const void *)mbk::tile_light_kernel<float, true, true>, (const void *)mbk::tile_todo_kernel<float>}};
        for (int f = 0; f < 2; ++f)
            for (int k = 0; k < 2; ++k) {
                int n = 0;
                MBK_CREATE_HIP(hipOccupancyMaxActiveBlocksPerMultiprocessor(&n, fns[f][k], 64, 0));
                ctx->scan_occ[f][k] = n > 0 ? n : 1;
            }
        const void *fi[2][6] = {{(const void *)mbk::tile_light_kernel<double, true, true, 2>, (const void *)mbk::tile_light_kernel<double, true, true, 1>,
                                 (const void *)mbk::tile_light_kernel<double, true, true, 2, true>, (const void *)mbk::tile_light_kernel<double, false, true, 2, true>,
                                 (const void *)mbk::tile_light_kernel<double, true, false, 2, true>, (const void *)mbk::tile_light_kernel<double, true, false, 1>},
                                {(const void *)mbk::tile_light_kernel<float, true, true, 2>, (const void *)mbk::tile_light_kernel<float, true, true, 1>,
                                 (const void *)mbk::tile_light_kernel<float, true, true, 2, true>, (const void *)mbk::tile_light_kernel<float, false, true, 2, true>,
                                 (const void *)mbk::tile_light_kernel<float, true, false, 2, true>, (const void *)mbk::tile_light_kernel<float, true, false, 1>}};
        for (int f = 0; f < 2; ++f) {
            int least = 0;
            for (int k = 0; k < 6; ++k) {
                int n = 0;
                MBK_CREATE_HIP(hipOccupancyMaxActiveBlocksPerMultiprocessor(&n, fi[f][k], 64, 0));
                n = n > 0 ? n : 1;
                least = (k == 0 || n < least) ? n : least;
            }
            ctx->scan_occ_inline[f] = least;
        }
    }
    {
        const void *fn = (const void *)mbk::tile_asm_kernel<double, true, 16, false>;
        for (int k = 1; k <= 7; ++k) {
            uint32_t lo = 0, hi = 65536;
            int n = 0;
            MBK_CREATE_HIP(hipOccupancyMaxActiveBlocksPerMultiprocessor(&n, fn, 64, hi));
            if (n > 4 * k) {
                ctx->wave_limit_lds[k] = hi;
                continue;
            }
            while (hi - lo > 64) {
                const uint32_t mid = (lo + hi) / 2;
                MBK_CREATE_HIP(hipOccupancyMaxActiveBlocksPerMultiprocessor(&n, fn, 64, mid));
                if (n > 4 * k) lo = mid;
                else hi = mid;
            }
            ctx->wave_limit_lds[k] = hi;
        }
    }
#undef MBK_CREATE_HIP
    *out = ctx;
    return MBK_OK;
}

void mbk_destroy(mbk_ctx *ctx)
{
    if (!ctx) return;
    if (ctx->device >= 0) (void)hipSetDevice(ctx->device);
    for (Slot &sl : ctx->s) {
        if (sl.stream) (void)hipStreamSynchronize(sl.stream);
        if (sl.d_counts) (void)hipFree(sl.d_counts);
        if (sl.d_bytes) (void)hipFree(sl.d_bytes);
        if (sl.d_red) (void)hipFree(sl.d_red);
        if (sl.h_red) (void)hipHostFree(sl.h_red);
        if (sl.ev_k0) (void)hipEventDestroy(sl.ev_k0);
        if (sl.ev_k1) (void)hipEventDestroy(sl.ev_k1);
        if (sl.ev_c0) (void)hipEventDestroy(sl.ev_c0);
        if (sl.ev_c1) (void)hipEventDestroy(sl.ev_c1);
        if (sl.stream) (void)hipStreamDestroy(sl.stream);
    }
    if (!ctx->scratch.empty() || !ctx->deep.empty()) (void)hipDeviceSynchronize();
    for (StreamScratch &sc : ctx->scratch) free_scratch(sc);
    for (mbk_ctx::DeepCopy &c : ctx->deep) free_deep_copy(c);
    if (ctx->d_rle) (void)hipFree(ctx->d_rle);
    if (ctx->d_smooth) (void)hipFree(ctx->d_smooth);
    if (ctx->d_rgba) (void)hipFree(ctx->d_rgba);
    if (ctx->d_hist) (void)hipFree(ctx->d_hist);
    if (ctx->d_density) (void)hipFree(ctx->d_density);
    if (ctx->d_density_stat) (void)hipFree(ctx->d_density_stat);
    delete ctx;
}

const char *mbk_last_error(const mbk_ctx *ctx) { return ctx ? ctx->err.c_str() : g_err.c_str(); }

int mbk_get_device_info(mbk_ctx *ctx, mbk_device_info *info)
{
    if (!ctx || !info) return fail(ctx, MBK_ERR_INVALID, "NULL argument");
    std::memset(info, 0, sizeof(*info));
    std::snprintf(info->name, sizeof(info->name), "%s", ctx->prop.name);
    std::snprintf(info->arch, sizeof(info->arch), "%s", ctx->prop.gcnArchName);
    info->compute_units = ctx->prop.multiProcessorCount;
    info->clock_mhz = ctx->prop.clockRate / 1000;
    info->wavefront_size = ctx->prop.warpSize;
    info->total_mem = ctx->prop.totalGlobalMem;
    return MBK_OK;
}

int mbk_device_pci_bus_id(mbk_ctx *ctx, char *buf, int len)
{
    if (!ctx || !buf || len < 16) return fail(ctx, MBK_ERR_INVALID, "buffer of at least 16 bytes needed");
    MBK_HIP(ctx, hipDeviceGetPCIBusId(buf, len, ctx->device));
    return MBK_OK;
}

int mbk_host_alloc(mbk_ctx *ctx, uint64_t bytes, void **out)
{
    if (!ctx || !out || bytes == 0) return fail(ctx, MBK_ERR_INVALID, "bad argument");
    MBK_HIP(ctx, hipSetDevice(ctx->device));
    MBK_HIP(ctx, hipHostMalloc(out, bytes, hipHostMallocDefault));
    return MBK_OK;
}

int mbk_host_free(mbk_ctx *ctx, void *ptr)
{
    if (!ctx) return fail(ctx, MBK_ERR_INVALID, "ctx is NULL");
    if (!ptr) return MBK_OK;
    MBK_HIP(ctx, hipSetDevice(ctx->device));
    MBK_HIP(ctx, hipHostFree(ptr));
    return MBK_OK;
}

int mbk_datachunk_geometry(uint32_t level, uint32_t index_real, uint32_t index_imag,
                           double *start_r, double *start_i, double *range)
{
    if (!start_r || !start_i || !range) return fail(nullptr, MBK_ERR_INVALID, "NULL output pointer");
    if (level == 0) return fail(nullptr, MBK_ERR_INVALID, "level must be > 0 (DataChunk.cs:99-100)");
    if (index_real >= level || index_imag >= level)
        return fail(nullptr, MBK_ERR_INVALID, "chunk index must be < level (DataChunk.cs:102-106)");
    volatile double chunk_range = (2.0 - (-2.0)) / (double)level;
    volatile double pr = chunk_range * (double)index_real;
// ... 326 lines not shown
static int launch_interior(mbk_ctx *ctx, const mbk_view *v, uint32_t mrd, uint32_t flags, bool safe, int32_t *d_counts,
                           int32_t *d_period, double *d_distance, hipStream_t stream)
{
    const size_t px = (size_t)v->ncols * v->nrows;
    if (!d_counts) {
        StreamScratch *sc = nullptr;
        int rc = get_scratch(ctx, stream, &sc);
        if (rc == MBK_OK) rc = grow(ctx, sc->d_dist_counts, sc->dist_cap_px, px, px * sizeof(int32_t));
        if (rc != MBK_OK) return rc;
        d_counts = sc->d_dist_counts;
    }
    int rc = launch_tile(ctx, v, mrd, (flags & MBK_KERNEL_MASK) | MBK_WANT_COUNTS, d_counts, nullptr, stream);
    if (rc != MBK_OK) return rc;
    mbk::InteriorArgs a;
    std::memset(&a, 0, sizeof(a));
    fill_window(a, v);
    a.blocks_x = (v->ncols + 7u) / 8u;
    a.mrd = (int32_t)mrd;
    a.counts_in = d_counts;
    a.period = d_period;
    a.distance = d_distance;
    const dim3 grid(a.blocks_x * ((v->nrows + 7u) / 8u)), block(64);
    if (safe) hipLaunchKernelGGL(mbk::interior_kernel<false>, grid, block, 0, stream, a);
    else hipLaunchKernelGGL(mbk::interior_kernel<true>, grid, block, 0, stream, a);
    MBK_HIP(ctx, hipGetLastError());
    return MBK_OK;
}

int mbk_view_interior_launch(mbk_ctx *ctx, const mbk_view *view, uint32_t mrd, uint32_t flags, int32_t *d_counts,
                             int32_t *d_period, double *d_distance, void *hip_stream)
{
    if (!ctx || (!d_period && !d_distance)) return fail(ctx, MBK_ERR_INVALID, "NULL argument");
    bool safe = false;
    int rc = interior_check(ctx, view, mrd, flags, &safe);
    if (rc != MBK_OK) return rc;
    MBK_HIP(ctx, hipSetDevice(ctx->device));
    return launch_interior(ctx, view, mrd, flags, safe, d_counts, d_period, d_distance, (hipStream_t)hip_stream);
}

int mbk_view_interior_compute(mbk_ctx *ctx, const mbk_view *view, uint32_t mrd, uint32_t flags, int32_t *h_counts,
                              int32_t *h_period, double *h_distance, mbk_stats *stats)
{
    if (!ctx || !view || (!h_period && !h_distance)) return fail(ctx, MBK_ERR_INVALID, "NULL argument");
    bool safe = false;
    int rc = interior_check(ctx, view, mrd, flags, &safe);
    if (rc != MBK_OK) return rc;
    rc = sync_begin(ctx);
    if (rc != MBK_OK) return rc;
    const size_t px = (size_t)view->ncols * view->nrows;
    return compute_values(ctx, px, mrd, h_counts, h_distance, stats,
                          [&](int32_t *d_counts, double *d_distance, hipStream_t stream) {
                              return launch_interior(ctx, view, mrd, flags, safe, d_counts, h_period ? (int32_t *)(d_distance + px) : nullptr,
                                                     h_distance ? d_distance : nullptr, stream);
                          },
                          true, h_period);
}

int mbk_interior_host(double c_r, double c_i, uint32_t mrd, int32_t *count, int32_t *period, int32_t *cycle_len, double *de)
{
    if (!count) return fail(nullptr, MBK_ERR_INVALID, "count is NULL");
    if (mrd > 0x7fffffffu) return fail(nullptr, MBK_ERR_INVALID, "mrd must fit int32 (calc_mb_value returns int32)");
    double mag = 0.0, d = 0.0;
    int32_t L = 0, p = 0;
    *count = mbk::julia_count<false>(c_r, c_i, c_r, c_i, (int32_t)mrd, &mag);
    mbk::interior_pixel<false>(c_r, c_i, (int32_t)mrd, *count, L, p, d);
    if (period) *period = p;
    if (cycle_len) *cycle_len = L;
    if (de) *de = d;
    return MBK_OK;
}

int mbk_serialize_last(mbk_ctx *ctx, uint8_t *h_out, uint64_t cap, uint64_t *size, uint32_t *codec)
{
    if (!ctx || !h_out || !size || !codec) return fail(ctx, MBK_ERR_INVALID, "NULL argument");
    int rc = sync_begin(ctx);
    if (rc != MBK_OK) return rc;
    const size_t n = ctx->last_px;
    if (n == 0) return fail(ctx, MBK_ERR_INVALID, "no tile with quantised bytes has been computed on this ctx");
    const uint32_t nblocks = (uint32_t)((n + mbk::kRleBlock - 1) / mbk::kRleBlock);
    auto align = [](size_t x) { return (x + 255) & ~(size_t)255; };
    const size_t max_runs = n / 5 + 1;
    const size_t off_cnt = 0, off_tot = align(off_cnt + (size_t)nblocks * 4), off_start = align(off_tot + 8),
                 off_val = align(off_start + max_runs * 4), off_out = align(off_val + max_runs),
                 total_bytes = off_out + 1 + n;
    rc = grow(ctx, ctx->d_rle, ctx->rle_cap_px, n, total_bytes);
    if (rc != MBK_OK) return rc;
    uint32_t *d_cnt = (uint32_t *)(ctx->d_rle + off_cnt);
    unsigned long long *d_tot = (unsigned long long *)(ctx->d_rle + off_tot);
    uint32_t *d_start = (uint32_t *)(ctx->d_rle + off_start);
    uint8_t *d_val = ctx->d_rle + off_val, *d_out = ctx->d_rle + off_out;
    hipStream_t s = ctx->s[0].stream;
    hipLaunchKernelGGL(mbk::rle_count_kernel, dim3(nblocks), dim3(mbk::kRleBlock), 0, s, ctx->s[0].d_bytes, (uint64_t)n, d_cnt);
    hipLaunchKernelGGL(mbk::rle_scan_kernel, dim3(1), dim3(1024), 0, s, d_cnt, nblocks, d_tot);
    MBK_HIP(ctx, hipGetLastError());
    unsigned long long runs = 0;
    MBK_HIP(ctx, hipMemcpyAsync(&runs, d_tot, sizeof(runs), hipMemcpyDeviceToHost, s));
    MBK_HIP(ctx, hipStreamSynchronize(s));
    const uint64_t raw_size = 1 + (uint64_t)n, rle_size = 1 + 5 * (uint64_t)runs;
    const bool use_rle = rle_size < raw_size;
    *codec = use_rle ? MBK_CODEC_RLE : MBK_CODEC_RAW;
    *size = use_rle ? rle_size : raw_size;
    if (cap < *size) return fail(ctx, MBK_ERR_INVALID, "output buffer too small for the serialised chunk");
    if (use_rle) {
        hipLaunchKernelGGL(mbk::rle_scatter_kernel, dim3(nblocks), dim3(mbk::kRleBlock), 0, s, ctx->s[0].d_bytes,
                           (uint64_t)n, d_cnt, d_start, d_val);
        hipLaunchKernelGGL(mbk::rle_emit_kernel, dim3((uint32_t)((runs + 255) / 256)), dim3(256), 0, s, d_start,
                           d_val, (uint64_t)runs, (uint64_t)n, d_out);
        MBK_HIP(ctx, hipGetLastError());
        MBK_HIP(ctx, hipMemcpyAsync(h_out, d_out, rle_size, hipMemcpyDeviceToHost, s));
    } else {
        h_out[0] = MBK_CODEC_RAW;
        MBK_HIP(ctx, hipMemcpyAsync(h_out + 1, ctx->s[0].d_bytes, n, hipMemcpyDeviceToHost, s));
    }
    MBK_HIP(ctx, hipStreamSynchronize(s));
    return MBK_OK;
}

int mbk_set_option(mbk_ctx *ctx, int option, uint32_t value)
{
    if (!ctx) return fail(ctx, MBK_ERR_INVALID, "ctx is NULL");
    bool ok = false;
    switch (option) {
        case MBK_OPT_ORDER: ok = value <= 3u; break;
        case MBK_OPT_WAVES_PER_WG: ok = value == 1u || value == 2u || value == 4u; break;
        case MBK_OPT_GROUP_STEPS: ok = value == 4u || value == 8u || value == 16u || value == 32u; break;
        case MBK_OPT_EXACT_STEPS: ok = value <= 4096u; break;
        case MBK_OPT_PROBE_STEPS: ok = value >= 2u && value <= 65536u; break;
        case MBK_OPT_SCAN_WAVES: ok = value >= 1u && value <= 8u; break;
        case MBK_OPT_SCAN_XCD_MAP: ok = value <= 1u; break;
        case MBK_OPT_SCAN_COL_PERIOD: ok = value <= 65536u; break;
        case MBK_OPT_HEAVY_SHARE: ok = value <= 65536u; break;
        case MBK_OPT_RF_LIVEMIN: ok = value <= 63u; break;
        case MBK_OPT_RF_PATIENCE: ok = value >= 16u && value <= (1u << 20); break;
        case MBK_OPT_RF_BATCH: ok = value >= 1u && value <= 64u; break;
        case MBK_OPT_RF_WAVES: ok = value >= 1u && value <= 8u; break;
        case MBK_OPT_CYCLE_DETECT: ok = value <= 1u; break;
        case MBK_OPT_PROBE_MID: ok = value >= 2u && value <= 65537u; break;
        case MBK_OPT_PREPASS_OVERLAP: ok = value <= 2u; break;
        case MBK_OPT_CLASSIFY_WG: ok = value >= 64u && value <= 1024u && value % 64u == 0u; break;
        case MBK_OPT_SCAN_STRIP: ok = value <= 1u; break;
        case MBK_OPT_CYCLE_WINDOW: ok = value <= 65536u; break;
        case MBK_OPT_EXACT_LONG: ok = value <= 4096u; break;
        case MBK_OPT_SCAN_INLINE: ok = value <= 1u; break;
        case MBK_OPT_WAVE_LIMIT: ok = value <= 7u; break;
        case MBK_OPT_UNITS_MIN_LIGHT: ok = value <= 65536u; break;
        case MBK_OPT_XCD_BALANCE: ok = value <= 2u; break;
        case MBK_OPT_M_LATE: ok = value <= 65536u; break;
        case MBK_OPT_H_SETTLED: ok = value <= 30u; break;
        case MBK_OPT_SPILL_FIRST: ok = value <= 65536u && value % 32u == 0u; break;
        case MBK_OPT_SPILL_LANES: ok = value >= 1u && value <= 32u; break;
        case MBK_OPT_SPILL_MIN_MRD: ok = true; break;
        case MBK_OPT_SPILL_MIN_BLOCKS: ok = value <= 31u; break;
        case MBK_OPT_SPILL_CYC_SHIFT: ok = value <= 31u; break;
        default: return fail(ctx, MBK_ERR_INVALID, "unknown MBK_OPT_* selector");
    }
    if (!ok) return fail(ctx, MBK_ERR_INVALID, "option value out of range");
    ctx->opt[option] = value;
    return MBK_OK;
}

int mbk_get_option(mbk_ctx *ctx, int option, uint32_t *value)
{
    if (!ctx || !value) return fail(ctx, MBK_ERR_INVALID, "NULL argument");
    if (option >= MBK_INFO_SCAN_WG_PER_CU && option < MBK_INFO_SCAN_WG_PER_CU + 4) {
        const int k = option - MBK_INFO_SCAN_WG_PER_CU;
        *value = (uint32_t)ctx->scan_occ[k >> 1][k & 1];
        return MBK_OK;
    }
    if (option >= MBK_INFO_XCD_SHARE && option < MBK_INFO_XCD_SHARE + 10) {
        const StreamScratch *best = nullptr;
        for (const StreamScratch &sc : ctx->scratch)
            if (!best || sc.xcd_consumed > best->xcd_consumed) best = &sc;
        const int k = option - MBK_INFO_XCD_SHARE;
        *value = !best ? 0u : k < 8 ? (uint32_t)std::lround(best->xcd_f[k] * 1048576.0) : k == 8 ? best->xcd_consumed : best->xcd_issued;
        return MBK_OK;
    }
    if (option == MBK_INFO_SPILL || option == MBK_INFO_SPILL + 1) {
        *value = ctx->spill_launches;
        if (option == MBK_INFO_SPILL) {
            *value = 0u;
            for (const StreamScratch &sc : ctx->scratch)
                if (sc.stream == ctx->last_spill_stream && sc.spill.d_total && ctx->spill_launches) {
                    unsigned long long t = 0;
                    MBK_HIP(ctx, hipSetDevice(ctx->device));
                    MBK_HIP(ctx, hipStreamSynchronize(sc.stream));
                    MBK_HIP(ctx, hipMemcpy(&t, sc.spill.d_total, sizeof(t), hipMemcpyDeviceToHost));
                    *value = (uint32_t)std::min<unsigned long long>(t, 0xffffffffull);
                }
        }
        return MBK_OK;
    }
    if (option < 0 || option >= MBK_OPT_COUNT_) return fail(ctx, MBK_ERR_INVALID, "unknown MBK_OPT_* selector");
    *value = ctx->opt[option];
    return MBK_OK;
}

static void shares_from_fractions(const double *f, uint32_t *cum)
{
    double c = 0.0;
    for (uint32_t x = 0; x < 8u; ++x) {
        c += f[x];
        cum[x] = x == 7u ? (1u << 24) : (uint32_t)std::lround(std::min(1.0, std::max(0.0, c)) * (double)(1u << 24));
    }
}

int mbk_units_plan(uint32_t n_h, uint32_t n_v, uint32_t n_m, const double *fractions, uint32_t *plan)
{
    if (!fractions || !plan) return MBK_ERR_INVALID;
    if ((uint64_t)n_h + n_v + n_m > 0x7fffffffull) return MBK_ERR_INVALID;
    uint32_t cum[8];
    shares_from_fractions(fractions, cum);
    mbk::units_plan(n_h, n_v, n_m, cum, 0u, plan, 0u, 0u);
    return MBK_OK;
}

int mbk_units_lookup(const uint32_t *plan, uint32_t id, uint32_t *list, uint32_t *index)
{
    if (!plan || !list || !index) return MBK_ERR_INVALID;
    const uint32_t x = id & 7u;
    bool is_h = false;
    uint32_t i = 0;
    *list = 0u;
    *index = 0u;
    if (id >= plan[2] || !mbk::units_lookup(id, plan[3], plan[4], plan[8u + x], plan[16u + x], plan[24u + x], plan[32u + x], is_h, i))
        return MBK_OK;
    *list = is_h ? 1u : (i < plan[1] ? 2u : 3u);
    *index = is_h ? i : (i < plan[1] ? i : i - plan[1]);
    return MBK_OK;
}

int mbk_quantise_counts(mbk_ctx *ctx, const int32_t *h_counts, uint64_t n, uint32_t mrd, uint8_t *h_bytes)
{
    if (!ctx || !h_counts || !h_bytes) return fail(ctx, MBK_ERR_INVALID, "NULL argument");
    if (mrd == 0 || mrd > 0x7fffffffu) return fail(ctx, MBK_ERR_INVALID, "mrd must be in [1, 2^31)");
    if (n == 0) return MBK_OK;
    if (n > (1ull << 31)) return fail(ctx, MBK_ERR_INVALID, "more than 2^31 counts");
    int rc = sync_begin(ctx);
    if (rc != MBK_OK) return rc;
    Slot &sl = ctx->s[0];
    rc = ensure_buffers(ctx, sl, (size_t)n);
    if (rc != MBK_OK) return rc;
    MBK_HIP(ctx, hipMemcpyAsync(sl.d_counts, h_counts, n * sizeof(int32_t), hipMemcpyHostToDevice, sl.stream));
    hipLaunchKernelGGL(mbk::quantise_kernel, dim3(2048), dim3(256), 0, sl.stream, sl.d_counts, sl.d_bytes, n,
                       (int32_t)mrd, mrd >= (1u << 23) ? 1u : 0u, 1.0 / (double)mrd);
    MBK_HIP(ctx, hipGetLastError());
    MBK_HIP(ctx, hipMemcpyAsync(h_bytes, sl.d_bytes, n, hipMemcpyDeviceToHost, sl.stream));
    MBK_HIP(ctx, hipStreamSynchronize(sl.stream));
    ctx->last_px = 0;
    return MBK_OK;
}

int mbk_reduce_counts(mbk_ctx *ctx, const int32_t *d_counts, uint64_t n, uint32_t mrd,
                      void *hip_stream, mbk_stats *stats)
{
    if (!ctx || !d_counts || !stats) return fail(ctx, MBK_ERR_INVALID, "NULL argument");
    MBK_HIP(ctx, hipSetDevice(ctx->device));
    hipStream_t s = (hipStream_t)hip_stream;
    StreamScratch *sc = nullptr;
    int rc = get_scratch(ctx, s, &sc);
    if (rc != MBK_OK) return rc;
    if (!sc->d_red) {
        MBK_HIP(ctx, hipMalloc((void **)&sc->d_red, sizeof(ReduceSlot) * mbk::kReduceSlots));
        MBK_HIP(ctx, hipHostMalloc((void **)&sc->h_red, sizeof(ReduceSlot) * mbk::kReduceSlots, hipHostMallocDefault));
    }
    rc = launch_reduce(ctx, sc->d_red, sc->h_red, d_counts, nullptr, n, mrd, s);
    if (rc != MBK_OK) return rc;
    MBK_HIP(ctx, hipStreamSynchronize(s));
    std::memset(stats, 0, sizeof(*stats));
    fill_stats_from_reduce(sc->h_red, stats, false);
    return MBK_OK;
}


int mbk_deep_orbit_create(const char *center_r, const char *center_i, uint32_t precision_bits, uint32_t mrd,
                          mbk_deep_orbit **out)
{
    if (!out) return fail(nullptr, MBK_ERR_INVALID, "out is NULL");
    *out = nullptr;
    mbk_deep_orbit *o = new (std::nothrow) mbk_deep_orbit();
    if (!o) return fail(nullptr, MBK_ERR_NOMEM, "out of host memory");
    std::string why;
    bool ok = false;
    try {
        ok = mbk::build_deep_orbit(center_r, center_i, precision_bits, mrd, &o->o, &why);
    } catch (const std::bad_alloc &) {
        delete o;
        return fail(nullptr, MBK_ERR_NOMEM, "out of host memory for the reference orbit");
    }
    if (!ok) {
        delete o;
        return fail(nullptr, MBK_ERR_INVALID, why);
    }
    *out = o;
    return MBK_OK;
}

void mbk_deep_orbit_destroy(mbk_deep_orbit *orbit) { delete orbit; }

int mbk_deep_orbit_info(const mbk_deep_orbit *orbit, uint32_t *length, uint32_t *escaped, uint32_t *precision_bits,
                        uint32_t *mrd)
{
    if (!orbit) return fail(nullptr, MBK_ERR_INVALID, "orbit is NULL");
    if (length) *length = orbit->o.length;
    if (escaped) *escaped = orbit->o.escaped;
    if (precision_bits) *precision_bits = orbit->o.precision_bits;
    if (mrd) *mrd = orbit->o.mrd;
    return MBK_OK;
}

int mbk_deep_orbit_read(const mbk_deep_orbit *orbit, double *zr, double *zi, uint64_t n)
{
    if (!orbit || !zr || !zi) return fail(nullptr, MBK_ERR_INVALID, "NULL argument");
    const uint64_t entries = (uint64_t)orbit->o.length + 1u;
    if (n < entries) return fail(nullptr, MBK_ERR_INVALID, "the output holds fewer than length + 1 entries");
    for (uint64_t k = 0; k < entries; ++k) {
        zr[k] = orbit->o.table[4 * k];
        zi[k] = orbit->o.table[4 * k + 1];
    }
    return MBK_OK;
}

int mbk_deep_orbit_read_wide(const mbk_deep_orbit *orbit, double *xr, double *xi, int32_t *xe, uint64_t n)
{
    if (!orbit || !xr || !xi || !xe) return fail(nullptr, MBK_ERR_INVALID, "NULL argument");
    const uint64_t entries = (uint64_t)orbit->o.length + 1u;
    if (n < entries) return fail(nullptr, MBK_ERR_INVALID, "the output holds fewer than length + 1 entries");
    for (uint64_t k = 0; k < entries; ++k) {
        xr[k] = orbit->o.wide[k].xr;
        xi[k] = orbit->o.wide[k].xi;
        xe[k] = orbit->o.wide[k].xe;
    }
    return MBK_OK;
}

static const size_t kMaxDeepCopies = 8;

static int deep_copy(mbk_ctx *ctx, const mbk_deep_orbit *orbit, mbk_ctx::DeepCopy **out)
{
    for (mbk_ctx::DeepCopy &c : ctx->deep)
        if (c.id == orbit->o.id) {
            *out = &c;
            return MBK_OK;
        }
    if (ctx->deep.size() >= kMaxDeepCopies) {
        MBK_HIP(ctx, hipDeviceSynchronize());
        for (mbk_ctx::DeepCopy &c : ctx->deep) free_deep_copy(c);
        ctx->deep.clear();
    }
    const size_t bytes = orbit->o.table.size() * sizeof(double);
    double4 *d = nullptr;
    MBK_HIP(ctx, hipMalloc((void **)&d, bytes));
    const hipError_t e = hipMemcpy(d, orbit->o.table.data(), bytes, hipMemcpyHostToDevice);
    if (e != hipSuccess) {
        (void)hipFree(d);
        return fail(ctx, MBK_ERR_HIP, std::string("hipMemcpy (reference orbit): ") + hipGetErrorString(e));
    }
    mbk_ctx::DeepCopy c = mbk_ctx::DeepCopy();
    c.id = orbit->o.id;
    c.d = d;
    ctx->deep.push_back(c);
    *out = &ctx->deep.back();
    return MBK_OK;
}

static int validate_deep(mbk_ctx *ctx, const mbk_deep_orbit *orbit, const mbk_deep_view *v, uint32_t mrd, uint32_t flags)
{
    return validate_deep_view(
        ctx, orbit, v, mrd, flags,
        [&]() -> int {
            if (flags & ~(MBK_WANT_COUNTS | MBK_WANT_BYTES | MBK_DEEP_BLA))
                return fail(ctx, MBK_ERR_INVALID, "deep views take MBK_WANT_COUNTS / MBK_WANT_BYTES / MBK_DEEP_BLA only (no kernel selection, no fp32)");
            if ((flags & MBK_DEEP_BLA) && orbit->o.length > (1u << 31))
                return fail(ctx, MBK_ERR_INVALID, "MBK_DEEP_BLA: the orbit is longer than 2^31 (the table's indices are 32 bits wide)");
            return MBK_OK;
        },
        [&]() -> int {
            if (!deep_ranges_within(v, 0x1p-960)) return fail(ctx, MBK_ERR_INVALID, "deep view ranges must be finite and lie in [2^-960, 4]");
            return MBK_OK;
        });
}
// ... 1882 lines not shown
```

distributedmandelbrot_amd/csrc/mbk_kernels.h:

```cpp
#pragma once

#include <hip/hip_runtime.h>
#include <stdint.h>

namespace mbk {

struct Axis {
    double start;
    double step;
    double last;
    double delta;
    double div;
    uint32_t n;
    uint32_t step_is_zero;
};

struct ReduceSlot;

constexpr uint32_t kSpillLevels = 12;

struct TileArgs {
    Axis re, im;
    uint32_t col0, row0, ncols, nrows;
    uint32_t blocks_x;
    uint32_t out_pitch, out_col0, out_row0;
    int32_t mrd;
    uint32_t quant_wide;
    double quant_rcp;
    uint32_t exact_steps;
    uint32_t exact_steps_long;
    uint32_t ring_possible;
    uint32_t fast_bx_end, fast_by_end;
    uint32_t perm_mul;
    const uint32_t *order;
    uint32_t ngrid;
    uint32_t order_mid;
    uint32_t unit_stride;
    uint32_t stamp_tag;
    const uint32_t *plan;
    unsigned long long *stamps;
    int32_t *counts;
    uint8_t *bytes;
    double *smooth;
    ReduceSlot *stats;
    uint32_t cyc_window;
    uint32_t spill_first;
    uint32_t spill_lanes;
    uint32_t spill_win_shift;
    void *spill_z;
    uint32_t *spill_meta;
    uint32_t *spill_cnt;
};

__device__ __forceinline__ double axis_value(const Axis &a, uint32_t k)
{
    double y;
    if (a.step_is_zero) {
        double q = (double)k / a.div;
        y = q * a.delta;
    } else {
        y = (double)k * a.step;
    }
    double v = y + a.start;
    return (k + 1u == a.n) ? a.last : v;
}

__device__ __forceinline__ uint8_t quantise(int32_t count, int32_t mrd, uint32_t wide, double rcp)
{
    if (wide) {
        uint64_t x = (uint64_t)(uint32_t)count * 256ull + (uint64_t)(uint32_t)mrd - 1ull;
        return (uint8_t)(x / (uint64_t)(uint32_t)mrd);
    }
    const uint32_t x = (uint32_t)count * 256u + (uint32_t)mrd - 1u;
    return (uint8_t)(uint32_t)__builtin_fma((double)x, rcp, 0x1p-30);
}
__device__ __forceinline__ uint8_t quantise(int32_t count, const TileArgs &p)
{
    return quantise(count, p.mrd, p.quant_wide, p.quant_rcp);
}

__device__ __forceinline__ double smooth_value(int32_t count, double m)
{
    return count > 0 ? (double)count + 1.0 - log2(0.5 * log(m)) : 0.0;
}

template <bool kFmaDouble>
__device__ __forceinline__ int32_t escape_count(double cr, double ci, int32_t mrd)
{
    double zr = cr, zi = ci;
    double a = zr * zr, b = zi * zi;
    int32_t result = 0;
    for (int32_t n = 1; n < mrd; ++n) {
        double t = a - b;
        double zi_new;
        if (kFmaDouble) {
            double p = zr * zi;
            zi_new = __builtin_fma(2.0, p, ci);
        } else {
            double w = 2.0 * zr;
            double u = w * zi;
            zi_new = u + ci;
        }
        zr = t + cr;
        zi = zi_new;
        a = zr * zr;
        b = zi * zi;
        double m = a + b;
        if (m >= 4.0) {
            result = n;
            break;
        }
    }
    return result;
}

template <bool kFmaDouble>
__global__ __launch_bounds__(256) void tile_simple_kernel(TileArgs p)
{
    const uint32_t lane = threadIdx.x & 63u;
    const uint32_t wave = threadIdx.x >> 6;
    const uint32_t by = blockIdx.x / p.blocks_x, bx = blockIdx.x - by * p.blocks_x;
    const uint32_t lc = bx * 32u + wave * 8u + (lane & 7u);
    const uint32_t lr = by * 8u + (lane >> 3);
    if (lc >= p.ncols || lr >= p.nrows) return;
    const double cr = axis_value(p.re, p.col0 + lc);
    const double ci = axis_value(p.im, p.row0 + lr);
    const int32_t count = escape_count<kFmaDouble>(cr, ci, p.mrd);
    const size_t o = (size_t)lr * p.ncols + lc;
    if (p.counts) p.counts[o] = count;
    if (p.bytes) p.bytes[o] = quantise(count, p);
}

#define MBK_T double
#define MBK_F "f64"
#define MBK_CI_FROM_T64 "v_add_f64 %[ci], %[t64], %[start]\n"
#define MBK_CR_FROM_T64 "v_add_f64 %[cr], %[t64], %[start]\n"
#define MBK_CYC_BITS "u64"
#define MBK_CYC_MOV "b64"
#include "mbk_loops.inc"
#undef MBK_T
#undef MBK_F
#undef MBK_CI_FROM_T64
#undef MBK_CR_FROM_T64
#undef MBK_CYC_BITS
#undef MBK_CYC_MOV
#define MBK_T float
#define MBK_F "f32"
#define MBK_CI_FROM_T64 "v_add_f64 %[t64], %[t64], %[start]\nv_cvt_f32_f64 %[ci], %[t64]\n"
#define MBK_CR_FROM_T64 "v_add_f64 %[t64], %[t64], %[start]\nv_cvt_f32_f64 %[cr], %[t64]\n"
#define MBK_CYC_BITS "u32"
#define MBK_CYC_MOV "b32"
#include "mbk_loops.inc"
#undef MBK_T
#undef MBK_F
#undef MBK_CI_FROM_T64
#undef MBK_CR_FROM_T64
#undef MBK_CYC_BITS
#undef MBK_CYC_MOV


template <typename T, bool kFmaDouble, int kGroup, bool kCycle = false>
__device__ __forceinline__ int32_t block_pixel(const TileArgs &p, uint32_t ucol, uint32_t urow, uint32_t lx, uint32_t ly,
                                               bool long_groups, bool interior = false)
{
    const uint32_t lc = ucol + lx, lr = urow + ly;
    T cr, ci;
    bool ring_test = kGroup != 0 && kFmaDouble;
    if (interior) {
        cr = (T)((double)(p.col0 + lc) * p.re.step + p.re.start);
        ci = (T)((double)(p.row0 + lr) * p.im.step + p.im.start);
        ring_test = ring_test && p.ring_possible != 0u;
    } else {
        if (lc >= p.ncols || lr >= p.nrows) return -1;
        cr = (T)axis_value(p.re, p.col0 + lc);
        ci = (T)axis_value(p.im, p.row0 + lr);
    }
    int32_t count;
    T m = 0;
    if (kGroup != 0 && kFmaDouble) {
        bool risky = false;
        if (ring_test) {
            const T c2 = cr * cr + ci * ci;
            const T margin = sizeof(T) == 8 ? (T)1e-9 : (T)1e-3;
            risky = __ballot(__builtin_fabs((double)(c2 - (T)4)) < (double)margin) != 0ull;
        }
        if (risky) {
            count = escape_count_asm<true>(cr, ci, p.mrd, &m);
        } else if (kGroup == 32) {
            count = long_groups ? escape_count_group<32, false>(cr, ci, p.mrd, &m, p.exact_steps_long)
                                : escape_count_group<8, false>(cr, ci, p.mrd, &m, p.exact_steps);
        } else if (kGroup == 16) {
            count = long_groups ? escape_count_group<16, kCycle>(cr, ci, p.mrd, &m, p.exact_steps_long, p.cyc_window)
                                : escape_count_group<8, kCycle>(cr, ci, p.mrd, &m, p.exact_steps, p.cyc_window);
        } else {
            count = escape_count_group<kGroup == 8 ? 8 : 4, kCycle>(cr, ci, p.mrd, &m, p.exact_steps, p.cyc_window);
        }
    } else {
        count = escape_count_asm<kFmaDouble>(cr, ci, p.mrd, &m);
    }
    const size_t ubase = (size_t)(urow + p.out_row0) * p.out_pitch + ucol + p.out_col0;
    const uint32_t loff = ly * p.out_pitch + lx;
    if (p.counts) (p.counts + ubase)[loff] = count;
    if (p.bytes) (p.bytes + ubase)[loff] = quantise(count, p);
    if (p.smooth) (p.smooth + ubase)[loff] = smooth_value(count, (double)m);
// ... 391 lines not shown
```

distributedmandelbrot_amd/csrc/mbk_units.h:

```cpp
#pragma once

#include "mbk_refill.h"

namespace mbk {

__host__ __device__ inline size_t units_settled_base(size_t n) { return 2u * n + 64u; }
__host__ __device__ inline size_t units_list_words(size_t n) { return 3u * n + 64u; }

struct XcdShares { uint32_t cum[8]; };
__host__ __device__ inline void units_plan(uint32_t n_h, uint32_t n_v, uint32_t n_m, const uint32_t *cum, uint32_t stamps, uint32_t *plan,
                                           uint32_t n_ml, uint32_t n_hs);

__device__ __forceinline__ int32_t probe_settling(double cr, double ci, int32_t cap, double *delta)
{
    double zr = cr, zi = ci;
    int32_t n = 1;
    for (; n < cap - 9; ++n) {
        const double t = zr * zr - zi * zi;
        zi = __builtin_fma(2.0, zr * zi, ci);
        zr = t + cr;
        if (zr * zr + zi * zi >= 4.0) { *delta = 1e300; return n; }
    }
    double hr[9], hi[9];
#pragma unroll
    for (int k = 0; k < 9; ++k) hr[k] = hi[k] = 1e150;
    for (; n < cap; ++n) {
        const double t = zr * zr - zi * zi;
        zi = __builtin_fma(2.0, zr * zi, ci);
        zr = t + cr;
        if (zr * zr + zi * zi >= 4.0) { *delta = 1e300; return n; }
#pragma unroll
        for (int k = 8; k > 0; --k) { hr[k] = hr[k - 1]; hi[k] = hi[k - 1]; }
        hr[0] = zr;
        hi[0] = zi;
    }
    double d = 1e300;
#pragma unroll
    for (int k = 1; k <= 8; ++k) {
        if (k == 7) continue;
        const double dr = hr[0] - hr[k], di = hi[0] - hi[k], q = dr * dr + di * di;
        d = q < d ? q : d;
    }
    *delta = d;
    return 0;
}

__global__ __launch_bounds__(1024) void classify_units_kernel(TileArgs p, uint32_t nregions, int32_t probe_steps,
                                                              uint32_t *order, uint32_t *counters, int32_t m_late, double settle_thr,
                                                              uint32_t *extra, uint32_t *plan, XcdShares shares, uint32_t stamps)
{
    __shared__ uint32_t s_last;
    __shared__ uint32_t s_cnt[5][16], s_base[5];
    const uint32_t r = blockIdx.x * blockDim.x + threadIdx.x;
    const uint32_t lane = threadIdx.x & 63u, wave = threadIdx.x >> 6;
    const bool valid = r < nregions;
    uint32_t cls = 5u;
    uint32_t by = 0, bx = 0;
    if (valid) {
        by = r / p.blocks_x;
        bx = r - by * p.blocks_x;
        uint32_t lc = bx * 8u + 4u, lr = by * 8u + 4u;
        lc = lc < p.ncols ? lc : p.ncols - 1u;
        lr = lr < p.nrows ? lr : p.nrows - 1u;
        const double cr = axis_value(p.re, p.col0 + lc), ci = axis_value(p.im, p.row0 + lr);
        const int32_t cap = p.mrd < probe_steps ? p.mrd : probe_steps;
        double delta = 1e300;
        const int32_t cnt = cap > 1 ? (settle_thr > 0.0 ? probe_settling(cr, ci, cap, &delta) : escape_count<true>(cr, ci, cap)) : 1;
        const bool regular = bx < p.fast_bx_end && by < p.fast_by_end;
        cls = cnt == 0 ? (delta <= settle_thr ? 4u : 0u) : (cnt <= 3 && regular ? 1u : (m_late > 0 && cnt >= m_late ? 3u : 2u));
    }
    const unsigned long long vmask = __ballot(cls == 1u);
    const uint32_t seg = (uint32_t)(vmask >> (lane & ~7u)) & 0xffu;
    const bool emit[5] = {cls == 0u, (lane & 7u) == 0u && seg != 0u, cls == 2u, cls == 3u, cls == 4u};
    unsigned long long m[5];
#pragma unroll
    for (uint32_t k = 0; k < 5u; ++k) {
        m[k] = __ballot(emit[k]);
        if (lane == 0) s_cnt[k][wave] = (uint32_t)__popcll(m[k]);
    }
    __syncthreads();
    if (threadIdx.x < 5u) {
        const uint32_t k = threadIdx.x, nw = (blockDim.x + 63u) >> 6;
        uint32_t t = 0;
        for (uint32_t w = 0; w < nw; ++w) {
            const uint32_t c = s_cnt[k][w];
            s_cnt[k][w] = t;
            t += c;
        }
        s_base[k] = t ? atomicAdd(k < 3u ? &counters[k] : &extra[k - 3u], t) : 0u;
    }
    __syncthreads();
    const unsigned long long below = (1ull << lane) - 1ull;
    if (emit[0]) order[s_base[0] + s_cnt[0][wave] + (uint32_t)__popcll(m[0] & below)] = (by << 16) | bx;
    if (emit[1]) order[nregions - 1u - (s_base[1] + s_cnt[1][wave] + (uint32_t)__popcll(m[1] & below))] = (by << 16) | ((bx >> 3) << 8) | seg;
    if (emit[2]) order[nregions + 3u + s_base[2] + s_cnt[2][wave] + (uint32_t)__popcll(m[2] & below)] = (by << 16) | bx;
    if (emit[3]) order[2u * nregions + 2u - (s_base[3] + s_cnt[3][wave] + (uint32_t)__popcll(m[3] & below))] = (by << 16) | bx;
    if (emit[4]) order[units_settled_base(nregions) + s_base[4] + s_cnt[4][wave] + (uint32_t)__popcll(m[4] & below)] = (by << 16) | bx;
    if (plan == nullptr) return;
    __syncthreads();
    if (threadIdx.x == 0) {
        __threadfence();
        s_last = atomicAdd(&extra[2], 1u) == gridDim.x - 1u ? 1u : 0u;
    }
    __syncthreads();
    if (s_last != 0u && threadIdx.x == 0) {
        __threadfence();
        const uint32_t n_h = atomicExch(&counters[0], 0u), n_v = atomicExch(&counters[1], 0u), n_m = atomicExch(&counters[2], 0u);
        const uint32_t n_ml = atomicExch(&extra[0], 0u), n_hs = atomicExch(&extra[1], 0u);
        atomicExch(&extra[2], 0u);
        units_plan(n_h + n_ml + n_hs, n_v, n_m, shares.cum, stamps, plan, n_ml, n_hs);
    }
}

constexpr uint32_t kStampTail = 8;
constexpr uint32_t kStampWords = 8u + 8u * kStampTail;
constexpr uint32_t kPlanWords = 40;

__host__ __device__ inline void units_plan(uint32_t n_h, uint32_t n_v, uint32_t n_m, const uint32_t *cum, uint32_t stamps, uint32_t *plan,
                                           uint32_t n_ml, uint32_t n_hs)
{
    const uint32_t n_l = n_m + n_v, total = n_h + n_l;
    uint32_t h[8], l[8], prev = 0, slots = (total + 7u) >> 3;
    for (uint32_t x = 0; x < 8u; ++x) {
        uint32_t c = x == 7u ? n_h : (uint32_t)(((unsigned long long)n_h * cum[x]) >> 24);
        c = c < prev ? prev : (c > n_h ? n_h : c);
        h[x] = c - prev;
        prev = c;
        slots = slots > h[x] ? slots : h[x];
    }
    uint32_t left = n_l, hmin = 0xffffffffu, lmin = 0xffffffffu;
    for (uint32_t x = 0; x < 8u; ++x) {
        const uint32_t room = slots - h[x];
        l[x] = room < left ? room : left;
        left -= l[x];
        hmin = hmin < h[x] ? hmin : h[x];
        lmin = lmin < l[x] ? lmin : l[x];
    }
    plan[0] = n_h; plan[1] = n_m; plan[2] = slots * 8u; plan[3] = hmin; plan[4] = lmin; plan[5] = stamps; plan[6] = n_ml < n_h ? n_ml : n_h; plan[7] = n_hs < n_h ? n_h - n_hs : 0u;
    uint32_t hb = 8u * hmin, lb = 8u * lmin;
    for (uint32_t x = 0; x < 8u; ++x) {
        plan[8u + x] = h[x];
        plan[16u + x] = l[x];
        plan[24u + x] = hb - hmin;
        plan[32u + x] = lb - lmin;
        hb += h[x] - hmin;
        lb += l[x] - lmin;
    }
}

__host__ __device__ __forceinline__ bool units_lookup(uint32_t u, uint32_t hmin, uint32_t lmin, uint32_t h_x, uint32_t l_x,
                                                      uint32_t hbase_x, uint32_t lbase_x, bool &is_h, uint32_t &i)
{
    const uint32_t x = u & 7u, j = u >> 3, k = j - h_x;
    is_h = j < h_x;
    if (!is_h && k >= l_x) return false;
    i = is_h ? (j < hmin ? u : hbase_x + j) : (k < lmin ? 8u * k + x : lbase_x + k);
    return true;
}

__device__ __forceinline__ void load_shares(const uint32_t *plan, uint32_t x, uint32_t &n_m, uint32_t &total, uint32_t &hmin,
                                            uint32_t &lmin, uint32_t &stamps, uint32_t &n_ml, uint32_t &hs0, uint32_t &h_x, uint32_t &l_x,
                                            uint32_t &hbase_x, uint32_t &lbase_x)
{
    const uint32_t *pl = plan, *px = plan + x;
    asm volatile("s_load_dword %0, %11, 0x4\n\t"
                 "s_load_dword %1, %11, 0x8\n\t"
                 "s_load_dword %2, %11, 0xc\n\t"
                 "s_load_dword %3, %11, 0x10\n\t"
                 "s_load_dword %4, %11, 0x14\n\t"
                 "s_load_dword %5, %11, 0x18\n\t"
                 "s_load_dword %6, %11, 0x1c\n\t"
                 "s_load_dword %7, %12, 0x20\n\t"
                 "s_load_dword %8, %12, 0x40\n\t"
                 "s_load_dword %9, %12, 0x60\n\t"
                 "s_load_dword %10, %12, 0x80\n\t"
                 "s_waitcnt lgkmcnt(0)"
                 : "=&s"(n_m), "=&s"(total), "=&s"(hmin), "=&s"(lmin), "=&s"(stamps), "=&s"(n_ml), "=&s"(hs0), "=&s"(h_x), "=&s"(l_x),
                   "=&s"(hbase_x), "=&s"(lbase_x)
                 : "s"(pl), "s"(px)
                 : "memory");
}

__device__ __forceinline__ void leave_stamp(uint32_t slot)
{
    unsigned long long base;
    uint32_t tag;
    asm volatile("s_load_dwordx2 %0, %2, %3\n\t"
                 "s_load_dword %1, %2, %4\n\t"
                 "s_waitcnt lgkmcnt(0)"
                 : "=&s"(base), "=&s"(tag)
                 : "s"(__builtin_amdgcn_kernarg_segment_ptr()), "n"(offsetof(TileArgs, stamps)), "n"(offsetof(TileArgs, stamp_tag))
                 : "memory");
    if (__lane_id() == 0)
        reinterpret_cast<unsigned long long *>(base)[slot] = (wall_clock64() & 0xffffffffffffull) | ((unsigned long long)tag << 48);
}

template <typename T, int kGroup, bool kCycle, bool kCounts, bool kBytes, bool kStats = false>
__global__ __launch_bounds__(64) __attribute__((amdgpu_waves_per_eu(8, 8))) void tile_units_kernel(TileArgs args, uint32_t qtab)
{
    static_assert(!kStats || (!kCounts && kBytes), "fused statistics exist for the bytes-only instantiation");
    unsigned long long heavy = 0;
    uint32_t acc = 0;
    const uint32_t never_cap = args.mrd > 1 ? (uint32_t)args.mrd - 1u : 0u;
    TileArgs p = args;
    p.smooth = nullptr;
    p.stats = nullptr;
    p.quant_wide = 0u;
    p.re.step_is_zero = p.im.step_is_zero = 0u;
    if (!kCounts) p.counts = nullptr;
    if (!kBytes) p.bytes = nullptr;
    const uint32_t lane = threadIdx.x;
    const uint32_t lx = lane & 7u, ly = lane >> 3;
    const uint32_t n = p.ngrid;
    const uint32_t x = blockIdx.x & 7u;
    const uint32_t oscale = kCounts ? 4u : 1u;
    for (uint32_t u = blockIdx.x;; u += p.unit_stride) {
        uint32_t n_m, total, hmin, lmin, stamps, n_ml, hs0, h_x, l_x, hbase_x, lbase_x;
        load_shares(args.plan, x, n_m, total, hmin, lmin, stamps, n_ml, hs0, h_x, l_x, hbase_x, lbase_x);
        if (stamps && u < p.unit_stride) {
            const uint32_t j0 = u >> 3, slots = total >> 3;
            if (j0 == 0u) leave_stamp(x);
            if (j0 < slots && j0 + kStampTail >= slots) leave_stamp(8u + x * kStampTail + (j0 + kStampTail - slots));
        }
        if (u >= total) break;
        bool is_h;
        uint32_t i;
        if (!units_lookup(u, hmin, lmin, h_x, l_x, hbase_x, lbase_x, is_h, i)) break;
        if (is_h || i < n_m) {
            const bool late = is_h && i < n_ml;
            const uint32_t e = scalar_load_u32(p.order, is_h ? (late ? 2u * n + 2u - i : (i < hs0 ? i - n_ml : (uint32_t)units_settled_base(n) + (i - hs0)))
                                                              : n + 3u + i);
            const uint32_t by = e >> 16, bx = e & 0xffffu;
            const int32_t c = block_pixel<T, true, kGroup, kCycle>(p, bx * 8u, by * 8u, lx, ly, kGroup >= 16 && is_h && !late,
                                                                   bx < p.fast_bx_end && by < p.fast_by_end);
            if (kStats && c >= 0) heavy += c > 0 ? (unsigned long long)(uint32_t)c : (1ull << 47) + never_cap;
        } else {
            const uint32_t v = scalar_load_u32(p.order, n - 1u - (i - n_m));
            const uint32_t by = v >> 16, bx0 = ((v >> 8) & 0xffu) << 3, mask = v & 0xffu;
            const T ci = (T)((double)(p.row0 + by * 8u + ly) * p.im.step + p.im.start);
            const T b0 = ci * ci;
            const size_t elem0 = (size_t)(by * 8u + p.out_row0) * p.out_pitch + bx0 * 8u + p.out_col0;
            int32_t *cb = reinterpret_cast<int32_t *>(uniform_u64(reinterpret_cast<unsigned long long>(kCounts ? p.counts + elem0 : nullptr)));
            uint8_t *bb = reinterpret_cast<uint8_t *>(uniform_u64(reinterpret_cast<unsigned long long>(kBytes ? p.bytes + elem0 : nullptr)));
            const uint32_t col = p.col0 + bx0 * 8u + lx, off = (ly * p.out_pitch + lx) * oscale;
            uint32_t k = 0;
            int32_t cnt;
            while (escape_light_row<kCounts, kBytes, kStats>(ci, b0, col, p.re.step, p.re.start, cnt, cb, bb, off, 8u * oscale, qtab, mask, k, &acc) != 0u) {
                const int32_t c = block_pixel<T, true, kGroup, kCycle>(p, (bx0 + k) * 8u, by * 8u, lx, ly, false, true);
                if (kStats && c >= 0) heavy += c > 0 ? (unsigned long long)(uint32_t)c : (1ull << 47) + never_cap;
                if (++k >= 8u) break;
            }
        }
    }
    if (kStats) {
        const unsigned long long iters = wave_sum_u64((heavy & ((1ull << 47) - 1ull)) + acc), never = wave_sum_u64(heavy >> 47);
        ReduceOut *out = &args.stats[blockIdx.x % kReduceSlots].r;
        if (lane == 0) {
            if (iters) atomicAdd(&out->pixel_iterations, iters);
            if (never) atomicAdd(&out->never_pixels, never);
        }
    }
}

}
```

distributedmandelbrot_amd/device.py:

```python
from __future__ import annotations

import ctypes as C
import math
from dataclasses import dataclass
from decimal import Decimal
from fractions import Fraction
from typing import Optional, Tuple, Union

import numpy as np

from . import _lib as L


class MbkError(RuntimeError):
    def __init__(self, status: int, message: str):
        super().__init__(f"libmbk_hip status {status}: {message}")
        self.status = status


def _error_text(lib, ctx=None) -> str:
    return (lib.mbk_last_error(ctx) or b"").decode()


def _check(lib, st: int, ctx=None) -> None:
# ... 239 lines not shown
                                              out.ctypes.data if out.size else None))
    return out


def density_cell_host(target: DensityTarget, z) -> Optional[Tuple[int, int]]:
    lib = L.load()
    ct = target.ctarget()
    cx, cy, inside = C.c_uint32(0), C.c_uint32(0), C.c_int(0)
    _check(lib, lib.mbk_density_cell_host(C.byref(ct), float(z[0]), float(z[1]), C.byref(cx), C.byref(cy), C.byref(inside)))
    return (int(cx.value), int(cy.value)) if inside.value else None


def density_host(view: View, target: DensityTarget, mrd: int, *, min_count: int = 1, max_count: int = 0, window=None,
                 out: Optional[np.ndarray] = None):
    lib = L.load()
    cv = MandelbrotDevice._cview(view, window)
    ct = target.ctarget()
    shape = (max(int(target.height), 0), max(int(target.width), 0))
    table = np.zeros(shape, np.uint32) if out is None else _out_array(out, shape, np.uint32)
    ds = L.mbk_density_stats()
    _check(lib, lib.mbk_density_accumulate_host(C.byref(cv), C.byref(ct), mrd, min_count, max_count,
                                                table.ctypes.data if table.size else None, C.byref(ds)))
    return table.reshape(shape), DensityStats(int(ds.deposits), int(ds.dropped))


def _stream_array(stream) -> np.ndarray:
    if isinstance(stream, np.ndarray):
        a = np.ascontiguousarray(stream, dtype=np.uint8).ravel()
    else:
        a = np.frombuffer(stream, np.uint8)
    return a


_EMPTY_STREAM = (C.c_uint8 * 1)()


def _stream_ptr(a: np.ndarray) -> int:
    return a.ctypes.data if a.size else C.addressof(_EMPTY_STREAM)


class ChunkStreamError(MbkError):

    def __init__(self, reason: int, message: str):
        super().__init__(L.MBK_ERR_INVALID, message)
        self.reason = reason


def chunk_stream_check(stream, n: int = L.MBK_CHUNK_BYTES) -> Tuple[int, int]:
    lib = L.load()
    a = _stream_array(stream)
    codec, runs, reason = C.c_uint32(0), C.c_uint64(0), C.c_uint32(0)
    st = lib.mbk_chunk_stream_check(_stream_ptr(a), a.size, n, C.byref(codec), C.byref(runs), C.byref(reason))
    if st != L.MBK_OK:
        raise ChunkStreamError(int(reason.value), _error_text(lib))
    return int(codec.value), int(runs.value)


def decode_chunk_host(stream, n: int = L.MBK_CHUNK_BYTES, out: Optional[np.ndarray] = None) -> np.ndarray:
    lib = L.load()
    a = _stream_array(stream)
    out = _out_array(out, n, np.uint8)
    _check(lib, lib.mbk_chunk_decode_host(_stream_ptr(a), a.size, n, out.ctypes.data))
    return out


class MandelbrotDevice:

    SLOTS = L.MBK_SLOTS
    WORKER_DEPTH = L.MBK_WORKER_DEPTH

    def __init__(self, device: int = 0):
        self._lib = L.load()
        h = C.c_void_p()
        _check(self._lib, self._lib.mbk_create(device, C.byref(h)))
        self._h = h
        self.device = device
        self._pinned = []
        self._ser_buf = np.empty(1 + L.MBK_CHUNK_BYTES, np.uint8)

    def close(self) -> None:
        if getattr(self, "_h", None):
            for p in self._pinned:
                self._lib.mbk_host_free(self._h, p)
            self._pinned = []
            self._lib.mbk_destroy(self._h)
            self._h = None

    def __enter__(self):
        return self

    def __exit__(self, *exc):
        self.close()

    def __del__(self):
        try:
            self.close()
        except Exception:
            pass

    def _check(self, st: int) -> None:
        _check(self._lib, st, self._h)

    def info(self) -> dict:
        inf = L.mbk_device_info()
        self._check(self._lib.mbk_get_device_info(self._h, C.byref(inf)))
        return {"name": inf.name.decode(), "arch": inf.arch.decode(),
                "compute_units": inf.compute_units, "clock_mhz": inf.clock_mhz,
                "wavefront_size": inf.wavefront_size, "total_mem": inf.total_mem}

    def pci_bus_id(self) -> str:
        buf = C.create_string_buffer(32)
        self._check(self._lib.mbk_device_pci_bus_id(self._h, buf, 32))
        return buf.value.decode()

    def pinned_empty(self, shape, dtype) -> np.ndarray:
        dtype = np.dtype(dtype)
        n = int(np.prod(shape)) * dtype.itemsize
        p = C.c_void_p()
        self._check(self._lib.mbk_host_alloc(self._h, max(n, 1), C.byref(p)))
        self._pinned.append(p)
        buf = (C.c_uint8 * max(n, 1)).from_address(p.value)
        return np.frombuffer(buf, dtype=dtype, count=int(np.prod(shape))).reshape(shape)

    def set_option(self, name: str, value: int) -> None:
        self._check(self._lib.mbk_set_option(self._h, L.OPTIONS[name], int(value)))

    def get_option(self, name: str) -> int:
        v = C.c_uint32(0)
        self._check(self._lib.mbk_get_option(self._h, L.OPTIONS[name], C.byref(v)))
        return int(v.value)

    def scan_occupancy(self) -> dict:
        out = {}
        for k, name in enumerate(["f64_scan", "f64_heavy", "f32_scan", "f32_heavy"]):
            v = C.c_uint32(0)
            self._check(self._lib.mbk_get_option(self._h, L.MBK_INFO_SCAN_WG_PER_CU + k, C.byref(v)))
            out[name] = int(v.value)
        return out

    def xcd_shares(self) -> dict:
        vals = []
        for k in range(10):
            v = C.c_uint32(0)
            self._check(self._lib.mbk_get_option(self._h, L.MBK_INFO_XCD_SHARE + k, C.byref(v)))
            vals.append(int(v.value))
        return {"shares": [round(v / 1048576.0, 5) for v in vals[:8]], "last_launch_read": vals[8], "units_launches": vals[9]}

    def spill_info(self) -> dict:
        a, b = C.c_uint32(0), C.c_uint32(0)
        self._check(self._lib.mbk_get_option(self._h, L.MBK_INFO_SPILL, C.byref(a)))
        self._check(self._lib.mbk_get_option(self._h, L.MBK_INFO_SPILL + 1, C.byref(b)))
        return {"lanes_last_launch": int(a.value), "launches": int(b.value)}

    def quantise_counts(self, counts: np.ndarray, mrd: int) -> np.ndarray:
        counts = np.ascontiguousarray(counts, dtype=np.int32)
        out = np.empty(counts.shape, np.uint8)
        self._check(self._lib.mbk_quantise_counts(self._h, counts.ctypes.data, counts.size, mrd, out.ctypes.data))
        return out

    @staticmethod
    def _cview(view: View, window) -> L.mbk_view:
        col0, row0, ncols, nrows = window if window is not None else (0, 0, view.width, view.height)
        return L.mbk_view(view.start_r, view.start_i, view.range_r, view.range_i,
                          view.width, view.height, col0, row0, ncols, nrows)

    def compute_view(self, view: View, mrd: int, *, window=None, want_counts: bool = True,
                     want_bytes: bool = True, kernel: str = "default", precision: str = "f64",
                     out_counts: Optional[np.ndarray] = None, out_bytes: Optional[np.ndarray] = None):
        cv = self._cview(view, window)
        shape = (cv.nrows, cv.ncols)
        counts = _out_array(out_counts, shape, np.int32) if want_counts else None
        byts = _out_array(out_bytes, shape, np.uint8) if want_bytes else None
        flags, p_counts, p_bytes = _wanted(shape, counts, byts)
        st = L.mbk_stats()
        self._check(self._lib.mbk_view_compute(self._h, C.byref(cv), mrd, L.KERNELS[kernel] | L.PRECISIONS[precision] | flags,
                                               p_counts, p_bytes, C.byref(st)))
        return counts, byts, _stats(st)

    def datachunk(self, level: int, mrd: int, index_real: int, index_imag: int, *,
                  want_counts: bool = False, out_bytes: Optional[np.ndarray] = None):
        byts = _out_array(out_bytes, L.MBK_CHUNK_BYTES, np.uint8)
        counts = np.empty(L.MBK_CHUNK_BYTES, np.int32) if want_counts else None
        st = L.mbk_stats()
        self._check(self._lib.mbk_datachunk(
            self._h, level, mrd, index_real, index_imag, byts.ctypes.data,
            counts.ctypes.data if counts is not None else None, C.byref(st)))
        return byts, counts, _stats(st)

    def compute_view_smooth(self, view: View, mrd: int, *, window=None, kernel: str = "default"):
        cv = self._cview(view, window)
        shape = (cv.nrows, cv.ncols)
        smooth = np.empty(shape, np.float64)
        counts = np.empty(shape, np.int32)
        st = L.mbk_stats()
        self._check(self._lib.mbk_view_compute_smooth(self._h, C.byref(cv), mrd, L.KERNELS[kernel],
                                                      counts.ctypes.data, smooth.ctypes.data, C.byref(st)))
        return smooth, counts, _stats(st)

    def launch_view_smooth(self, view: View, mrd: int, *, d_smooth: int, d_counts: int = 0, stream: int = 0,
                           window=None, kernel: str = "default") -> None:
        cv = self._cview(view, window)
        self._check(self._lib.mbk_view_launch_smooth(self._h, C.byref(cv), mrd, L.KERNELS[kernel],
                                                     d_counts or None, d_smooth, stream or None))

    def compute_view_distance(self, view: View, mrd: int, *, window=None, kernel: str = "default"):
        cv = self._cview(view, window)
        shape = (cv.nrows, cv.ncols)
        dist = np.empty(shape, np.float64)
        counts = np.empty(shape, np.int32)
        st = L.mbk_stats()
        self._check(self._lib.mbk_view_compute_distance(self._h, C.byref(cv), mrd, L.KERNELS[kernel],
                                                        counts.ctypes.data, dist.ctypes.data, C.byref(st)))
        return dist, counts, _stats(st)

    def launch_view_distance(self, view: View, mrd: int, *, d_distance: int, d_counts: int = 0, stream: int = 0,
                             window=None, kernel: str = "default") -> None:
        cv = self._cview(view, window)
        self._check(self._lib.mbk_view_launch_distance(self._h, C.byref(cv), mrd, L.KERNELS[kernel],
                                                       d_counts or None, d_distance, stream or None))

    def compute_view_interior(self, view: View, mrd: int, *, window=None, kernel: str = "default", want_counts: bool = True,
                              want_period: bool = True, want_distance: bool = True):
        cv = self._cview(view, window)
        shape = (cv.nrows, cv.ncols)
        period = np.empty(shape, np.int32) if want_period else None
        dist = np.empty(shape, np.float64) if want_distance else None
        counts = np.empty(shape, np.int32) if want_counts else None
        st = L.mbk_stats()
        ptr = lambda a: a.ctypes.data if a is not None else None
        self._check(self._lib.mbk_view_interior_compute(self._h, C.byref(cv), mrd, L.KERNELS[kernel], ptr(counts), ptr(period),
                                                        ptr(dist), C.byref(st)))
        return period, dist, counts, _stats(st)

    def launch_view_interior(self, view: View, mrd: int, *, d_period: int = 0, d_distance: int = 0, d_counts: int = 0,
                             stream: int = 0, window=None, kernel: str = "default") -> None:
        cv = self._cview(view, window)
        self._check(self._lib.mbk_view_interior_launch(self._h, C.byref(cv), mrd, L.KERNELS[kernel], d_counts or None,
                                                       d_period or None, d_distance or None, stream or None))

    def render_view_interior(self, view: View, mrd: int, *, palette, scale: float = 2.0 ** 80, supersample: int = 1,
                             unknown=(0, 0, 0, 255), outside=(255, 255, 255, 255), window=None, kernel: str = "default",
                             max_band_rows: int = 0, out: Optional[np.ndarray] = None):
        cv = self._cview(view, window)
        spec, pal = _interior_spec(palette, supersample, unknown, outside, scale, max_band_rows)
        img = self._render_out(cv, out)
        st = L.mbk_stats()
        self._check(self._lib.mbk_view_interior_render_compute(self._h, C.byref(cv), mrd, L.KERNELS[kernel], C.byref(spec),
                                                               img.ctypes.data, C.byref(st)))
        return img, _stats(st)

    def launch_render_view_interior(self, view: View, mrd: int, *, palette, d_rgba: int, scale: float = 2.0 ** 80,
                                    supersample: int = 1, unknown=(0, 0, 0, 255), outside=(255, 255, 255, 255), stream: int = 0,
                                    window=None, kernel: str = "default", max_band_rows: int = 0) -> None:
        cv = self._cview(view, window)
        spec, pal = _interior_spec(palette, supersample, unknown, outside, scale, max_band_rows)
        self._check(self._lib.mbk_view_interior_render_launch(self._h, C.byref(cv), mrd, L.KERNELS[kernel], C.byref(spec),
                                                              d_rgba or None, stream or None))

    def serialize_last(self) -> Tuple[bytes, int]:
        cap = len(self._ser_buf)
        size, codec = C.c_uint64(0), C.c_uint32(0)
        st = self._lib.mbk_serialize_last(self._h, self._ser_buf.ctypes.data, cap, C.byref(size), C.byref(codec))
        if st == L.MBK_ERR_INVALID and size.value > cap:
            self._ser_buf = np.empty(size.value, np.uint8)
            st = self._lib.mbk_serialize_last(self._h, self._ser_buf.ctypes.data, size.value, C.byref(size),
                                              C.byref(codec))
        self._check(st)
        return self._ser_buf[:size.value].tobytes(), int(codec.value)

    def submit_datachunk(self, slot: int, level: int, mrd: int, index_real: int, index_imag: int,
                         out_bytes: np.ndarray, lazy_uniform: bool = False) -> None:
        assert out_bytes.dtype == np.uint8 and out_bytes.size == L.MBK_CHUNK_BYTES and out_bytes.flags.c_contiguous
        self._check(self._lib.mbk_datachunk_submit_ex(self._h, slot, level, mrd, index_real, index_imag,
                                                      out_bytes.ctypes.data, None,
                                                      L.MBK_LAZY_UNIFORM if lazy_uniform else 0))

    def submit_view(self, slot: int, view: View, mrd: int, *, window=None, out_counts: Optional[np.ndarray] = None,
                    out_bytes: Optional[np.ndarray] = None, kernel: str = "default", precision: str = "f64") -> None:
        cv = self._cview(view, window)
        flags, p_counts, p_bytes = _wanted((cv.nrows, cv.ncols), out_counts, out_bytes)
        self._check(self._lib.mbk_view_submit(self._h, slot, C.byref(cv), mrd, L.KERNELS[kernel] | L.PRECISIONS[precision] | flags,
                                              p_counts, p_bytes))

    def wait(self, slot: int) -> TileStats:
        st = L.mbk_stats()
        self._check(self._lib.mbk_wait(self._h, slot, C.byref(st)))
        return _stats(st)

    def launch_view(self, view: View, mrd: int, *, d_counts: int = 0, d_bytes: int = 0,
                    stream: int = 0, window=None, kernel: str = "default", precision: str = "f64") -> None:
        cv = self._cview(view, window)
        flags = (L.KERNELS[kernel] | L.PRECISIONS[precision] | (L.MBK_WANT_COUNTS if d_counts else 0)
                 | (L.MBK_WANT_BYTES if d_bytes else 0))
        self._check(self._lib.mbk_view_launch(self._h, C.byref(cv), mrd, flags,
                                              d_counts or None, d_bytes or None, stream or None))

    @staticmethod
    def _cdeep(view: Union[DeepView, WideDeepView], window):
        col0, row0, ncols, nrows = window if window is not None else (0, 0, view.width, view.height)
        if isinstance(view, WideDeepView):
            return L.mbk_deep_xview(view.range_r, view.range_i, view.exp2, view.width, view.height, col0, row0, ncols, nrows)
        return L.mbk_deep_view(view.span_r, view.span_i, view.width, view.height, col0, row0, ncols, nrows)

    def _deep_fn(self, view, name: str, bla: bool = False, source: Optional[str] = None):
        if isinstance(view, WideDeepView):
            if bla:
# ... 298 lines not shown
```

include/mbk.h:

```cpp
#ifndef MBK_H
#define MBK_H

#include <stdint.h>

#ifdef __cplusplus
extern "C" {
#endif

#define MBK_ABI_VERSION 5

#define MBK_CHUNK_DEFINITION 4096u
#define MBK_CHUNK_BYTES (4096u * 4096u)

enum mbk_status {
    MBK_OK = 0,
    MBK_ERR_INVALID = 1,
    MBK_ERR_NO_DEVICE = 2,
    MBK_ERR_HIP = 3,
    MBK_ERR_NOMEM = 4,
    MBK_ERR_NET = 5
};

#define MBK_WANT_COUNTS 0x1u
#define MBK_WANT_BYTES 0x2u
// ... 198 lines not shown
                                          uint32_t flags, const mbk_render_spec *spec, const double *h_lut, uint32_t lut_len,
                                          uint8_t *d_rgba, void *hip_stream);
int mbk_deep_view_render_equalized_compute(mbk_ctx *ctx, const mbk_deep_orbit *orbit, const mbk_deep_view *view, uint32_t mrd,
                                           uint32_t flags, const mbk_render_spec *spec, const double *h_lut, uint32_t lut_len,
                                           uint8_t *h_rgba, mbk_stats *stats);
int mbk_deep_xview_render_equalized_launch(mbk_ctx *ctx, const mbk_deep_orbit *orbit, const mbk_deep_xview *view, uint32_t mrd,
                                           uint32_t flags, const mbk_render_spec *spec, const double *h_lut, uint32_t lut_len,
                                           uint8_t *d_rgba, void *hip_stream);
int mbk_deep_xview_render_equalized_compute(mbk_ctx *ctx, const mbk_deep_orbit *orbit, const mbk_deep_xview *view, uint32_t mrd,
                                            uint32_t flags, const mbk_render_spec *spec, const double *h_lut, uint32_t lut_len,
                                            uint8_t *h_rgba, mbk_stats *stats);
int mbk_render_resolve_equalized_host(const mbk_render_spec *spec, const double *h_lut, uint32_t lut_len, uint32_t width,
                                      uint32_t height, const int32_t *counts, const double *smooth, uint8_t *rgba);

int mbk_julia_view_launch(mbk_ctx *ctx, const mbk_view *view, double c_r, double c_i, uint32_t mrd, uint32_t flags,
                          int32_t *d_counts, uint8_t *d_bytes, double *d_smooth, void *hip_stream);
int mbk_julia_view_compute(mbk_ctx *ctx, const mbk_view *view, double c_r, double c_i, uint32_t mrd, uint32_t flags,
                           int32_t *h_counts, uint8_t *h_bytes, double *h_smooth, mbk_stats *stats);
int mbk_julia_view_submit(mbk_ctx *ctx, int slot, const mbk_view *view, double c_r, double c_i, uint32_t mrd, uint32_t flags,
                          int32_t *h_counts, uint8_t *h_bytes);
int mbk_julia_view_render_launch(mbk_ctx *ctx, const mbk_view *view, double c_r, double c_i, uint32_t mrd, uint32_t flags,
                                 const mbk_render_spec *spec, uint8_t *d_rgba, void *hip_stream);
int mbk_julia_view_render_compute(mbk_ctx *ctx, const mbk_view *view, double c_r, double c_i, uint32_t mrd, uint32_t flags,
                                  const mbk_render_spec *spec, uint8_t *h_rgba, mbk_stats *stats);
int mbk_julia_view_render_equalized_launch(mbk_ctx *ctx, const mbk_view *view, double c_r, double c_i, uint32_t mrd,
                                           uint32_t flags, const mbk_render_spec *spec, const double *h_lut, uint32_t lut_len,
                                           uint8_t *d_rgba, void *hip_stream);
int mbk_julia_view_render_equalized_compute(mbk_ctx *ctx, const mbk_view *view, double c_r, double c_i, uint32_t mrd,
                                            uint32_t flags, const mbk_render_spec *spec, const double *h_lut, uint32_t lut_len,
                                            uint8_t *h_rgba, mbk_stats *stats);
int mbk_julia_view_histogram_launch(mbk_ctx *ctx, const mbk_view *view, double c_r, double c_i, uint32_t mrd, uint32_t flags,
                                    uint64_t *d_hist, void *hip_stream);
int mbk_julia_view_histogram_compute(mbk_ctx *ctx, const mbk_view *view, double c_r, double c_i, uint32_t mrd, uint32_t flags,
                                     uint64_t *h_hist, mbk_stats *stats);
int mbk_julia_count_host(double z_r, double z_i, double c_r, double c_i, uint32_t mrd, int32_t *count, double *mag);

#define MBK_DENSITY_MAX_CELLS (1u << 28)
#define MBK_DENSITY_LINEAR 0u
#define MBK_DENSITY_SQRT 1u
typedef struct mbk_density_target {
    double start_r, start_i;
    double range_r, range_i;
    uint32_t width, height;
} mbk_density_target;
typedef struct mbk_density_stats {
    uint64_t deposits;
    uint64_t dropped;
} mbk_density_stats;
typedef struct mbk_density_render_spec {
    uint32_t mode;
    uint32_t factor;
    const uint8_t *palette;
    uint32_t palette_len;
    double scale, offset;
} mbk_density_render_spec;
int mbk_view_density_launch(mbk_ctx *ctx, const mbk_view *view, const mbk_density_target *target, uint32_t mrd, uint32_t min_count,
                            uint32_t max_count, uint32_t flags, uint32_t *d_density, void *hip_stream);
int mbk_view_density_compute(mbk_ctx *ctx, const mbk_view *view, const mbk_density_target *target, uint32_t mrd, uint32_t min_count,
                             uint32_t max_count, uint32_t flags, uint32_t *h_density, mbk_stats *stats, mbk_density_stats *dstats);
int mbk_density_max(mbk_ctx *ctx, const uint32_t *d_density, uint64_t n, uint32_t *max, uint64_t *total, void *hip_stream);
int mbk_density_render_launch(mbk_ctx *ctx, const uint32_t *d_density, uint32_t width, uint32_t height,
                              const mbk_density_render_spec *spec, uint8_t *d_rgba, void *hip_stream);
int mbk_density_render_compute(mbk_ctx *ctx, const uint32_t *h_density, uint32_t width, uint32_t height,
                               const mbk_density_render_spec *spec, uint8_t *h_rgba, mbk_stats *stats);
int mbk_density_cell_host(const mbk_density_target *target, double z_r, double z_i, uint32_t *cell_x, uint32_t *cell_y, int *inside);
int mbk_density_accumulate_host(const mbk_view *view, const mbk_density_target *target, uint32_t mrd, uint32_t min_count,
                                uint32_t max_count, uint32_t *density, mbk_density_stats *dstats);
int mbk_density_resolve_host(const mbk_density_render_spec *spec, uint32_t width, uint32_t height, const uint32_t *density,
                             uint8_t *rgba);
int mbk_density_build_info(void);

typedef struct mbk_interior_render_spec {
    uint32_t supersample;
    const uint8_t *palette;
    uint32_t palette_len;
    uint8_t unknown[4];
    uint8_t outside[4];
    double scale;
    uint32_t max_band_rows;
} mbk_interior_render_spec;
int mbk_view_interior_launch(mbk_ctx *ctx, const mbk_view *view, uint32_t mrd, uint32_t flags, int32_t *d_counts,
                             int32_t *d_period, double *d_distance, void *hip_stream);
int mbk_view_interior_compute(mbk_ctx *ctx, const mbk_view *view, uint32_t mrd, uint32_t flags, int32_t *h_counts,
                              int32_t *h_period, double *h_distance, mbk_stats *stats);
int mbk_interior_host(double c_r, double c_i, uint32_t mrd, int32_t *count, int32_t *period, int32_t *cycle_len, double *de);
int mbk_view_interior_render_launch(mbk_ctx *ctx, const mbk_view *view, uint32_t mrd, uint32_t flags,
                                    const mbk_interior_render_spec *spec, uint8_t *d_rgba, void *hip_stream);
int mbk_view_interior_render_compute(mbk_ctx *ctx, const mbk_view *view, uint32_t mrd, uint32_t flags,
                                     const mbk_interior_render_spec *spec, uint8_t *h_rgba, mbk_stats *stats);
int mbk_interior_resolve_host(const mbk_interior_render_spec *spec, uint32_t width, uint32_t height, const int32_t *counts,
                              const int32_t *period, const double *de, uint8_t *rgba);

#define MBK_CODEC_RAW 0x00u
#define MBK_CODEC_RLE 0x01u

int mbk_serialize_last(mbk_ctx *ctx, uint8_t *h_out, uint64_t cap, uint64_t *size, uint32_t *codec);

#define MBK_STREAM_OK 0u
#define MBK_STREAM_BAD_CODEC 1u
#define MBK_STREAM_BAD_SIZE 2u
#define MBK_STREAM_ZERO_RUN 3u
#define MBK_STREAM_TOO_LONG 4u
#define MBK_STREAM_TOO_SHORT 5u

typedef struct mbk_chunk_spec {
    const uint8_t *palette;
    uint32_t scale;
} mbk_chunk_spec;

int mbk_chunk_stream_check(const uint8_t *stream, uint64_t size, uint64_t n, uint32_t *codec, uint64_t *runs, uint32_t *reason);
int mbk_chunk_decode_host(const uint8_t *stream, uint64_t size, uint64_t n, uint8_t *bytes);
int mbk_chunk_resolve_host(const mbk_chunk_spec *spec, const uint8_t *bytes, uint8_t *rgba, uint64_t pitch_px);
int mbk_chunk_decode_launch(mbk_ctx *ctx, const uint8_t *h_stream, uint64_t size, uint64_t n, uint8_t *d_bytes,
                            uint32_t *d_status, void *hip_stream);
int mbk_chunk_render_launch(mbk_ctx *ctx, const uint8_t *h_stream, uint64_t size, const mbk_chunk_spec *spec, uint8_t *d_rgba,
                            uint64_t pitch_px, uint32_t *d_status, void *hip_stream);
int mbk_chunk_decode_compute(mbk_ctx *ctx, const uint8_t *h_stream, uint64_t size, uint64_t n, uint8_t *h_bytes,
                             mbk_stats *stats);
int mbk_chunk_render_compute(mbk_ctx *ctx, const uint8_t *h_stream, uint64_t size, const mbk_chunk_spec *spec, uint8_t *h_rgba,
                             uint64_t pitch_px, mbk_stats *stats);

enum mbk_option {
    MBK_OPT_ORDER = 0,
    MBK_OPT_WAVES_PER_WG,
    MBK_OPT_GROUP_STEPS,
    MBK_OPT_EXACT_STEPS,
    MBK_OPT_PROBE_STEPS,
    MBK_OPT_SCAN_WAVES,
    MBK_OPT_SCAN_XCD_MAP,
    MBK_OPT_SCAN_COL_PERIOD,
    MBK_OPT_HEAVY_SHARE,
    MBK_OPT_RF_LIVEMIN,
    MBK_OPT_RF_PATIENCE,
    MBK_OPT_RF_BATCH,
    MBK_OPT_RF_WAVES,
    MBK_OPT_CYCLE_DETECT,
    MBK_OPT_PROBE_MID,
    MBK_OPT_PREPASS_OVERLAP,
    MBK_OPT_EXACT_LONG,
    MBK_OPT_SCAN_INLINE,
    MBK_OPT_WAVE_LIMIT,
    MBK_OPT_UNITS_MIN_LIGHT,
    MBK_OPT_XCD_BALANCE,
    MBK_OPT_M_LATE,
    MBK_OPT_H_SETTLED,
    MBK_OPT_CLASSIFY_WG,
    MBK_OPT_SCAN_STRIP,
    MBK_OPT_CYCLE_WINDOW,
    MBK_OPT_SPILL_FIRST,
    MBK_OPT_SPILL_LANES,
    MBK_OPT_SPILL_MIN_MRD,
    MBK_OPT_SPILL_MIN_BLOCKS,
    MBK_OPT_SPILL_CYC_SHIFT,
    MBK_OPT_COUNT_
};
#define MBK_INFO_SCAN_WG_PER_CU 100
#define MBK_INFO_XCD_SHARE 110
#define MBK_INFO_SPILL 130
int mbk_set_option(mbk_ctx *ctx, int option, uint32_t value);
int mbk_get_option(mbk_ctx *ctx, int option, uint32_t *value);

int mbk_units_plan(uint32_t n_h, uint32_t n_v, uint32_t n_m, const double *fractions, uint32_t *plan);
int mbk_units_lookup(const uint32_t *plan, uint32_t id, uint32_t *list, uint32_t *index);

int mbk_quantise_counts(mbk_ctx *ctx, const int32_t *h_counts, uint64_t n, uint32_t mrd, uint8_t *h_bytes);

int mbk_reduce_counts(mbk_ctx *ctx, const int32_t *d_counts, uint64_t n, uint32_t mrd,
                      void *hip_stream, mbk_stats *stats);

typedef struct mbk_worker_report {
    uint64_t leased;
    uint64_t accepted;
    uint64_t rejected;
    uint64_t resets;
    uint64_t uniform_tiles;
    uint64_t pixel_iterations;
    double kernel_ms_sum;
    double seconds;
    uint64_t net_retries;
} mbk_worker_report;
int mbk_worker_run(mbk_ctx *ctx, const char *addr, uint16_t port, uint64_t max_tiles, uint32_t senders,
                   mbk_worker_report *report);

enum mbk_net_option {
    MBK_NET_MAX_CONNECTIONS = 0,
    MBK_NET_CONNECT_TIMEOUT_MS = 1,
    MBK_NET_IO_TIMEOUT_MS = 2,
    MBK_NET_RETRIES = 3,
    MBK_NET_BACKOFF_MS = 4,
    MBK_NET_STOP = 5,
    MBK_NET_PEAK_CONNECTIONS = 6,
    MBK_NET_FEEDER_SLOTS = 7,
    MBK_NET_OPT_COUNT_
};
int mbk_net_set_option(int option, uint32_t value);
int mbk_net_get_option(int option, uint32_t *value);

typedef struct mbk_feeder_ops {
    void *user;
    int (*submit)(void *user, int slot, uint32_t level, uint32_t mrd, uint32_t index_real, uint32_t index_imag, uint8_t *h_bytes);
    int (*wait)(void *user, int slot, mbk_stats *stats);
    void *(*alloc)(void *user, uint64_t bytes);
    void (*release)(void *user, void *ptr);
    void (*on_tile)(void *user, const uint32_t workload[4], const mbk_stats *stats, int status);
} mbk_feeder_ops;
int mbk_feeder_run(const mbk_feeder_ops *ops, const char *addr, uint16_t port, uint64_t max_tiles, uint32_t senders,
                   mbk_worker_report *report);

#ifdef __cplusplus
}
#endif
#endif
```

Baseline: 5348.

## Pack late-escaping lanes into shared per-level pools to compact divergent waves

Adds a packed mode, on by default for f64, in which blocks classified as late or bordering late regions are grouped into jobs of 16 blocks. Each wave iterates in geometric levels, and when only some lanes are still alive it pushes their z state into a per-slice pool in device memory. Later waves refill full 64-lane batches from that pool, which removes the idle lanes left when a divergent wave keeps running after most pixels have escaped. The classify pass now works in 32x32 block patches and reclassifies blocks next to the boundary into the packed class. The cost is extra memory traffic for pool save and restore, fences, and more work in the classify pass.

Measured after the change: 5370 (median of 6 runs). Within noise of the previous version (+0.4%).

```diff
diff --git a/distributedmandelbrot_amd/_lib.py b/distributedmandelbrot_amd/_lib.py
--- a/distributedmandelbrot_amd/_lib.py
+++ b/distributedmandelbrot_amd/_lib.py
@@ -21,7 +21,7 @@
            "refill": MBK_KERNEL_REFILL, "group": MBK_KERNEL_GROUP, "scan": MBK_KERNEL_SCAN}
 OPTIONS = {name: i for i, name in enumerate(
     ["order", "waves_per_wg", "group_steps", "exact_steps", "probe_steps", "scan_waves", "scan_xcd_map", "scan_col_period", "heavy_share",
-     "rf_livemin", "rf_patience", "rf_batch", "rf_waves", "cycle_detect", "probe_mid", "prepass_overlap", "exact_long", "scan_inline", "wave_limit", "units_min_light", "xcd_balance", "m_late", "h_settled", "classify_wg", "scan_strip", "cycle_window", "spill_first", "spill_lanes", "spill_min_mrd", "spill_min_blocks", "spill_cyc_shift"])}
+     "rf_livemin", "rf_patience", "rf_batch", "rf_waves", "cycle_detect", "probe_mid", "prepass_overlap", "exact_long", "scan_inline", "wave_limit", "units_min_light", "xcd_balance", "m_late", "h_settled", "classify_wg", "scan_strip", "cycle_window", "spill_first", "spill_lanes", "spill_min_mrd", "spill_min_blocks", "spill_cyc_shift", "pack"])}
 MBK_PRECISION_F32 = 0x1000
 MBK_LAZY_UNIFORM = 0x2000
 MBK_DEEP_BLA = 0x8000
@@ -31,6 +31,7 @@
 MBK_INFO_SCAN_WG_PER_CU = 100
 MBK_INFO_XCD_SHARE = 110
 MBK_INFO_SPILL = 130
+MBK_INFO_PACK = 140
 MBK_CODEC_RAW = 0x00
 MBK_CODEC_RLE = 0x01
 MBK_CHUNK_DEFINITION = 4096
@@ -188,6 +189,8 @@
     "mbk_quantise_counts": (C.c_int, [C.c_void_p, C.c_void_p, C.c_uint64, C.c_uint32, C.c_void_p]),
     "mbk_units_plan": (C.c_int, [C.c_uint32, C.c_uint32, C.c_uint32, C.c_void_p, C.c_void_p]),
     "mbk_units_lookup": (C.c_int, [C.c_void_p, C.c_uint32, C.c_void_p, C.c_void_p]),
+    "mbk_units_pack": (C.c_int, [C.c_void_p, C.c_uint32, C.c_uint32, C.c_uint32, C.c_uint32, C.c_uint32, C.c_uint32, C.c_void_p, C.c_void_p,
+                                 C.c_void_p, C.c_void_p]),
     "mbk_reduce_counts": (C.c_int, [C.c_void_p, C.c_void_p, C.c_uint64, C.c_uint32, C.c_void_p,
                                     C.POINTER(mbk_stats)]),
     "mbk_worker_run": (C.c_int, [C.c_void_p, C.c_char_p, C.c_uint16, C.c_uint64, C.c_uint32,
diff --git a/distributedmandelbrot_amd/csrc/mbk_api.hip b/distributedmandelbrot_amd/csrc/mbk_api.hip
--- a/distributedmandelbrot_amd/csrc/mbk_api.hip
+++ b/distributedmandelbrot_amd/csrc/mbk_api.hip
@@ -41,6 +41,8 @@
 
 struct OrderRing {
     uint32_t *d_order[kOrderRing] = {};
+    void *d_pack = nullptr;
+    uint32_t pack_cap = 0;
     uint32_t *d_ctl = nullptr;
     bool ctl_dirty = true;
     size_t order_cap = 0;
@@ -60,6 +62,9 @@
             done_valid[k] = false;
         }
         order_cap = 0;
+        if (d_pack) (void)hipFree(d_pack);
+        d_pack = nullptr;
+        pack_cap = 0;
     }
     void drop_aux()
     {
@@ -171,6 +176,7 @@
     int scan_occ_inline[2] = {0, 0};
     uint32_t wave_limit_lds[8] = {0, 0, 0, 0, 0, 0, 0, 0};
     uint32_t spill_launches = 0;
+    uint32_t pack_launches = 0;
     hipStream_t last_spill_stream = nullptr;
     struct ProbeKey { Axis re, im; uint32_t col0, row0, ncols, nrows; } probe_key = {};
     double probe_share = 0.0;
@@ -490,6 +496,9 @@
     ~OrderList() { if (sc && !whole) sc->ring.ctl_dirty = true; }
 };
 
+constexpr uint32_t kPackG = 16, kPackFirst = 64;
+static size_t pack_pool_bytes(uint32_t nblocks) { return ((size_t)nblocks / kPackG + 2u) * mbk::kPackSliceBytes; }
+
 static int acquire_order_list(mbk_ctx *ctx, hipStream_t stream, uint32_t nblocks, OrderList *out)
 {
     StreamScratch *sc = nullptr;
@@ -534,6 +543,17 @@
             MBK_HIP(ctx, hipMalloc((void **)&ring.d_order[k], mbk::units_list_words(nblocks) * sizeof(uint32_t)));
         ring.order_cap = nblocks;
     }
+    if (ctx->opt[MBK_OPT_PACK] != 0u && nblocks > ring.pack_cap && pack_pool_bytes(nblocks) <= (1ull << 30)) {
+        MBK_HIP(ctx, hipStreamSynchronize(stream));
+        if (ring.d_pack) (void)hipFree(ring.d_pack);
+        ring.d_pack = nullptr;
+        ring.pack_cap = 0;
+        if (hipMalloc(&ring.d_pack, pack_pool_bytes(nblocks)) == hipSuccess) ring.pack_cap = nblocks;
+        else {
+            (void)hipGetLastError();
+            ring.d_pack = nullptr;
+        }
+    }
     const unsigned k = ring.order_turn++ % (unsigned)kOrderRing;
     if (overlap && ring.done_valid[k]) MBK_HIP(ctx, hipStreamWaitEvent(ring.aux, ring.ev_done[k], 0));
     out->k = k;
@@ -544,7 +564,7 @@
     return MBK_OK;
 }
 
-static int enqueue_units_prepass(mbk_ctx *ctx, TileArgs &a, const BlockLaunchPlan &p, const OrderList &ol, hipStream_t stream)
+static int enqueue_units_prepass(mbk_ctx *ctx, TileArgs &a, const BlockLaunchPlan &p, const OrderList &ol, hipStream_t stream, bool f32)
 {
     StreamScratch *sc = ol.sc;
     OrderRing &ring = sc->ring;
@@ -585,9 +605,17 @@
     a.stamps = balance == 1u ? sc->h_stamps + (size_t)(seq % kStampSlots) * mbk::kStampWords : nullptr;
     a.stamp_tag = seq & 0xffffu;
     const uint32_t cwg = ctx->opt[MBK_OPT_CLASSIFY_WG];
+    uint32_t pack = ctx->opt[MBK_OPT_PACK];
+    if (pack == 2u && !p.cyc) pack = 1u;
+    if (f32 || cwg != 1024u || a.blocks_x % mbk::kPackPatch != 0u || p.by % mbk::kPackPatch != 0u || p.by > 0x7fffu || a.blocks_x > 2048u ||
+        ring.pack_cap < p.grid.x || !ring.d_pack)
+        pack = 0u;
+    a.pack_g = pack ? kPackG : 0u;
+    a.pack_first = kPackFirst;
+    a.pack_pool = pack ? ring.d_pack : nullptr;
     hipLaunchKernelGGL(mbk::classify_units_kernel, dim3((p.grid.x + cwg - 1u) / cwg), dim3(cwg), 0, ol.pre, a, p.grid.x,
                        (int32_t)p.probe_steps, ol.list, ctl, (int32_t)ctx->opt[MBK_OPT_M_LATE], settle_thr, ctl + 3, (uint32_t *)a.plan, w,
-                       a.stamps ? 1u : 0u);
+                       a.stamps ? 1u : 0u, pack, kPackG);
     return MBK_OK;
 }
 
@@ -655,8 +683,17 @@
 typedef void (*BlockKernel)(TileArgs);
 typedef void (*SpillKernel)(TileArgs, const uint32_t *, const unsigned long long *, uint32_t);
 
-static UnitsKernel pick_units_kernel(bool f32, bool cyc, bool stats, bool counts, bool bytes)
-{
+static UnitsKernel pick_units_kernel(bool f32, bool cyc, bool stats, bool counts, bool bytes, bool pack)
+{
+    if (pack && !f32) {
+        static const UnitsKernel packed[2][4] = {
+            {mbk::tile_units_kernel<double, 16, true, false, true, true, true>, mbk::tile_units_kernel<double, 16, true, true, true, false, true>,
+             mbk::tile_units_kernel<double, 16, true, false, true, false, true>, mbk::tile_units_kernel<double, 16, true, true, false, false, true>},
+            {mbk::tile_units_kernel<double, 16, false, false, true, true, true>, mbk::tile_units_kernel<double, 16, false, true, true, false, true>,
+             mbk::tile_units_kernel<double, 16, false, false, true, false, true>, mbk::tile_units_kernel<double, 16, false, true, false, false, true>},
+        };
+        return packed[cyc ? 0 : 1][stats ? 0 : (counts && bytes) ? 1 : bytes ? 2 : 3];
+    }
     static const UnitsKernel forms[4][4] = {
         {mbk::tile_units_kernel<float, 8, true, false, true, true>, mbk::tile_units_kernel<float, 8, true, true, true>,
          mbk::tile_units_kernel<float, 8, true, false, true>, mbk::tile_units_kernel<float, 8, true, true, false>},
@@ -705,13 +742,14 @@
     uint32_t g = (uint32_t)std::min<double>((double)p.grid.x, est * 1.15 + 2048.0);
     g = (std::max(std::max(g, std::min(p.grid.x, cus * 64u)), 16384u) + 7u) & ~7u;
     a.unit_stride = g;
+    if (a.pack_g != 0u) ++ctx->pack_launches;
     const bool stats = fuse != nullptr && fuse->slots != nullptr && fuse->counts_unwanted && a.bytes != nullptr;
     if (stats) {
         a.stats = fuse->slots;
         a.counts = nullptr;
         fuse->fused = true;
     }
-    hipLaunchKernelGGL(pick_units_kernel(f32, p.cyc, stats, a.counts != nullptr, a.bytes != nullptr), dim3(g), dim3(64), lds, stream, a,
+    hipLaunchKernelGGL(pick_units_kernel(f32, p.cyc, stats, a.counts != nullptr, a.bytes != nullptr, a.pack_g != 0u), dim3(g), dim3(64), lds, stream, a,
                        quant_table4(a.mrd, a.bytes != nullptr));
 }
 
@@ -740,7 +778,7 @@
         if (rc != MBK_OK) return rc;
         OrderRing &ring = ol.sc->ring;
         bool mid_first = false;
-        rc = p.units ? enqueue_units_prepass(ctx, a, p, ol, stream) : enqueue_classify_prepass(ctx, a, p, ol, &mid_first);
+        rc = p.units ? enqueue_units_prepass(ctx, a, p, ol, stream, f32) : enqueue_classify_prepass(ctx, a, p, ol, &mid_first);
         if (rc != MBK_OK) return rc;
         if (ol.overlap) {
             MBK_HIP(ctx, hipEventRecord(ring.ev_cls[ol.k], ring.aux));
@@ -1513,7 +1551,8 @@
          48u,  256u,  1u,  8u,  1u,
          65537u,  1u,  0u,  1u,  0u,
          32768u,  0u,  8u,  6u,  1024u,
-         1u,  32u,  256u,  16u,  2048u,  19u,  5u};
+         1u,  32u,  256u,  16u,  2048u,  19u,  5u,
+         1u};
     std::memcpy(ctx->opt, kDefaults, sizeof(kDefaults));
 #define MBK_CREATE_HIP(call)                                                        \
     do {                                                                            \
@@ -2146,6 +2185,7 @@
         case MBK_OPT_SPILL_MIN_MRD: ok = true; break;
         case MBK_OPT_SPILL_MIN_BLOCKS: ok = value <= 31u; break;
         case MBK_OPT_SPILL_CYC_SHIFT: ok = value <= 31u; break;
+        case MBK_OPT_PACK: ok = value <= 2u; break;
         default: return fail(ctx, MBK_ERR_INVALID, "unknown MBK_OPT_* selector");
     }
     if (!ok) return fail(ctx, MBK_ERR_INVALID, "option value out of range");
@@ -2167,6 +2207,10 @@
             if (!best || sc.xcd_consumed > best->xcd_consumed) best = &sc;
         const int k = option - MBK_INFO_XCD_SHARE;
         *value = !best ? 0u : k < 8 ? (uint32_t)std::lround(best->xcd_f[k] * 1048576.0) : k == 8 ? best->xcd_consumed : best->xcd_issued;
+        return MBK_OK;
+    }
+    if (option == MBK_INFO_PACK) {
+        *value = ctx->pack_launches;
         return MBK_OK;
     }
     if (option == MBK_INFO_SPILL || option == MBK_INFO_SPILL + 1) {
@@ -2220,6 +2264,40 @@
         return MBK_OK;
     *list = is_h ? 1u : (i < plan[1] ? 2u : 3u);
     *index = is_h ? i : (i < plan[1] ? i : i - plan[1]);
+    return MBK_OK;
+}
+
+int mbk_units_pack(const uint8_t *classes, uint32_t blocks_x, uint32_t blocks_y, uint32_t fast_bx_end, uint32_t fast_by_end, uint32_t pack,
+                   uint32_t pack_g, uint8_t *filed, uint32_t *order, uint32_t *n_packed, uint32_t *n_jobs)
+{
+    if (!classes || !filed || !n_packed || !n_jobs) return MBK_ERR_INVALID;
+    if (blocks_x == 0u || blocks_y == 0u || blocks_x % mbk::kPackPatch != 0u || blocks_y % mbk::kPackPatch != 0u || pack == 0u || pack > 2u ||
+        pack_g == 0u || (uint64_t)blocks_x * blocks_y > 0x7fffffffull)
+        return MBK_ERR_INVALID;
+    const uint32_t nwg = (blocks_x / mbk::kPackPatch) * (blocks_y / mbk::kPackPatch), nt = mbk::kPackPatch * mbk::kPackPatch;
+    uint32_t np = 0;
+    std::vector<uint8_t> map(nt);
+    for (uint32_t w = 0; w < nwg; ++w) {
+        uint32_t bx = 0, by = 0;
+        for (uint32_t t = 0; t < nt; ++t) {
+            mbk::pack_patch_block(w, t, blocks_x, bx, by);
+            const uint8_t c = classes[(size_t)by * blocks_x + bx];
+            if (c > 4u) return MBK_ERR_INVALID;
+            map[t] = c;
+        }
+        for (uint32_t t = 0; t < nt; ++t) {
+            mbk::pack_patch_block(w, t, blocks_x, bx, by);
+            const uint32_t c = mbk::pack_class(map.data(), t & (mbk::kPackPatch - 1u), t / mbk::kPackPatch, map[t],
+                                               bx < fast_bx_end && by < fast_by_end, pack);
+            filed[(size_t)by * blocks_x + bx] = (uint8_t)c;
+            if (c == 3u) {
+                if (order) order[np] = (by << 16) | bx;
+                ++np;
+            }
+        }
+    }
+    *n_packed = np;
+    *n_jobs = (np + pack_g - 1u) / pack_g;
     return MBK_OK;
 }
 
diff --git a/distributedmandelbrot_amd/csrc/mbk_kernels.h b/distributedmandelbrot_amd/csrc/mbk_kernels.h
--- a/distributedmandelbrot_amd/csrc/mbk_kernels.h
+++ b/distributedmandelbrot_amd/csrc/mbk_kernels.h
@@ -50,6 +50,9 @@
     void *spill_z;
     uint32_t *spill_meta;
     uint32_t *spill_cnt;
+    uint32_t pack_g;
+    uint32_t pack_first;
+    void *pack_pool;
 };
 
 __device__ __forceinline__ double axis_value(const Axis &a, uint32_t k)
diff --git a/distributedmandelbrot_amd/csrc/mbk_units.h b/distributedmandelbrot_amd/csrc/mbk_units.h
--- a/distributedmandelbrot_amd/csrc/mbk_units.h
+++ b/distributedmandelbrot_amd/csrc/mbk_units.h
@@ -7,6 +7,33 @@
 __host__ __device__ inline size_t units_settled_base(size_t n) { return 2u * n + 64u; }
 __host__ __device__ inline size_t units_list_words(size_t n) { return 3u * n + 64u; }
 
+constexpr uint32_t kPackPatch = 32;
+__host__ __device__ inline uint32_t pack_class(const uint8_t *map, uint32_t tx, uint32_t ty, uint32_t cls, bool regular, uint32_t pack)
+{
+    if (cls == 3u) return regular ? 3u : 2u;
+    if ((cls != 0u && cls != 4u) || !regular) return cls;
+    if (pack >= 2u && cls == 0u) return 3u;
+    bool near = false;
+    for (uint32_t dy = 0; dy < 3u; ++dy)
+        for (uint32_t dx = 0; dx < 3u; ++dx) {
+            const uint32_t y = ty + dy - 1u, x = tx + dx - 1u;
+            if (y < kPackPatch && x < kPackPatch) {
+                const uint32_t c = map[y * kPackPatch + x];
+                near = near || (c != 0u && c != 4u);
+            }
+        }
+    return near ? 3u : cls;
+}
+__host__ __device__ inline void pack_patch_block(uint32_t w, uint32_t t, uint32_t blocks_x, uint32_t &bx, uint32_t &by)
+{
+    const uint32_t patches_x = blocks_x / kPackPatch, py = w / patches_x, px = w - py * patches_x;
+    bx = px * kPackPatch + (t & (kPackPatch - 1u));
+    by = py * kPackPatch + t / kPackPatch;
+}
+constexpr uint32_t kPackLevels = 4, kPackCap = 128;
+constexpr uint32_t kPackLevelBytes = kPackCap * 36u, kPackSliceBytes = 64u + kPackLevels * kPackLevelBytes;
+
+constexpr uint32_t kPlanWords = 40;
 struct XcdShares { uint32_t cum[8]; };
 __host__ __device__ inline void units_plan(uint32_t n_h, uint32_t n_v, uint32_t n_m, const uint32_t *cum, uint32_t stamps, uint32_t *plan,
                                            uint32_t n_ml, uint32_t n_hs);
@@ -47,18 +74,22 @@
 
 __global__ __launch_bounds__(1024) void classify_units_kernel(TileArgs p, uint32_t nregions, int32_t probe_steps,
                                                               uint32_t *order, uint32_t *counters, int32_t m_late, double settle_thr,
-                                                              uint32_t *extra, uint32_t *plan, XcdShares shares, uint32_t stamps)
+                                                              uint32_t *extra, uint32_t *plan, XcdShares shares, uint32_t stamps,
+                                                              uint32_t pack, uint32_t pack_g)
 {
     __shared__ uint32_t s_last;
     __shared__ uint32_t s_cnt[5][16], s_base[5];
+    __shared__ uint8_t s_map[kPackPatch * kPackPatch];
     const uint32_t r = blockIdx.x * blockDim.x + threadIdx.x;
     const uint32_t lane = threadIdx.x & 63u, wave = threadIdx.x >> 6;
-    const bool valid = r < nregions;
+    const bool valid = pack != 0u || r < nregions;
     uint32_t cls = 5u;
     uint32_t by = 0, bx = 0;
+    bool regular = false;
     if (valid) {
         by = r / p.blocks_x;
         bx = r - by * p.blocks_x;
+        if (pack != 0u) pack_patch_block(blockIdx.x, threadIdx.x, p.blocks_x, bx, by);
         uint32_t lc = bx * 8u + 4u, lr = by * 8u + 4u;
         lc = lc < p.ncols ? lc : p.ncols - 1u;
         lr = lr < p.nrows ? lr : p.nrows - 1u;
@@ -66,8 +97,13 @@
         const int32_t cap = p.mrd < probe_steps ? p.mrd : probe_steps;
         double delta = 1e300;
         const int32_t cnt = cap > 1 ? (settle_thr > 0.0 ? probe_settling(cr, ci, cap, &delta) : escape_count<true>(cr, ci, cap)) : 1;
-        const bool regular = bx < p.fast_bx_end && by < p.fast_by_end;
+        regular = bx < p.fast_bx_end && by < p.fast_by_end;
         cls = cnt == 0 ? (delta <= settle_thr ? 4u : 0u) : (cnt <= 3 && regular ? 1u : (m_late > 0 && cnt >= m_late ? 3u : 2u));
+    }
+    if (pack != 0u) {
+        s_map[threadIdx.x] = (uint8_t)cls;
+        __syncthreads();
+        cls = pack_class(s_map, threadIdx.x & (kPackPatch - 1u), threadIdx.x / kPackPatch, cls, regular, pack);
     }
     const unsigned long long vmask = __ballot(cls == 1u);
     const uint32_t seg = (uint32_t)(vmask >> (lane & ~7u)) & 0xffu;
@@ -106,16 +142,19 @@
     if (s_last != 0u && threadIdx.x == 0) {
         __threadfence();
         const uint32_t n_h = atomicExch(&counters[0], 0u), n_v = atomicExch(&counters[1], 0u), n_m = atomicExch(&counters[2], 0u);
-        const uint32_t n_ml = atomicExch(&extra[0], 0u), n_hs = atomicExch(&extra[1], 0u);
+        uint32_t n_ml = atomicExch(&extra[0], 0u);
+        const uint32_t n_hs = atomicExch(&extra[1], 0u);
         atomicExch(&extra[2], 0u);
+        if (pack != 0u) {
+            plan[kPlanWords] = n_ml;
+            n_ml = (n_ml + pack_g - 1u) / pack_g;
+        }
         units_plan(n_h + n_ml + n_hs, n_v, n_m, shares.cum, stamps, plan, n_ml, n_hs);
     }
 }
 
 constexpr uint32_t kStampTail = 8;
 constexpr uint32_t kStampWords = 8u + 8u * kStampTail;
-constexpr uint32_t kPlanWords = 40;
-
 __host__ __device__ inline void units_plan(uint32_t n_h, uint32_t n_v, uint32_t n_m, const uint32_t *cum, uint32_t stamps, uint32_t *plan,
                                            uint32_t n_ml, uint32_t n_hs)
 {
@@ -195,7 +234,172 @@
         reinterpret_cast<unsigned long long *>(base)[slot] = (wall_clock64() & 0xffffffffffffull) | ((unsigned long long)tag << 48);
 }
 
-template <typename T, int kGroup, bool kCycle, bool kCounts, bool kBytes, bool kStats = false>
+template <typename T>
+__device__ __forceinline__ void pack_coords(uint32_t col, uint32_t row, T &cr, T &ci)
+{
+    double re[2], im[2];
+    asm volatile("s_load_dwordx2 %0, %4, %5\n\t"
+                 "s_load_dwordx2 %1, %4, %6\n\t"
+                 "s_load_dwordx2 %2, %4, %7\n\t"
+                 "s_load_dwordx2 %3, %4, %8\n\t"
+                 "s_waitcnt lgkmcnt(0)"
+                 : "=&s"(re[0]), "=&s"(re[1]), "=&s"(im[0]), "=&s"(im[1])
+                 : "s"(__builtin_amdgcn_kernarg_segment_ptr()), "n"(offsetof(TileArgs, re.start)), "n"(offsetof(TileArgs, re.step)),
+                   "n"(offsetof(TileArgs, im.start)), "n"(offsetof(TileArgs, im.step))
+                 : "memory");
+    cr = (T)((double)col * re[1] + re[0]);
+    ci = (T)((double)row * im[1] + im[0]);
+}
+
+template <typename T, bool kCycle, bool kCounts, bool kBytes, bool kStats>
+__device__ __forceinline__ void packed_job(const TileArgs &p, uint32_t job, uint32_t n_p, unsigned long long &heavy, uint32_t never_cap)
+{
+    const uint32_t n = p.ngrid, e0 = job * p.pack_g;
+    const uint32_t nk = n_p - e0 < p.pack_g ? n_p - e0 : p.pack_g;
+    char *slice = reinterpret_cast<char *>(uniform_u64(reinterpret_cast<unsigned long long>(p.pack_pool) + (unsigned long long)job * kPackSliceBytes));
+    uint32_t *hdr = reinterpret_cast<uint32_t *>(slice);
+    const uint32_t total = p.mrd > 1 ? (uint32_t)p.mrd - 1u : 0u;
+    const uint32_t first = total < p.exact_steps ? total : p.exact_steps;
+    uint32_t fill = 0u;
+    uint32_t k = 0u;
+    bool flushing = false;
+    for (;;) {
+        int src = -1;
+        for (int l = 0; l < (int)kPackLevels; ++l)
+            if (((fill >> (8 * l)) & 0xffu) >= 64u) src = l;
+        if (src < 0 && flushing)
+            for (int l = (int)kPackLevels - 1; l >= 0; --l)
+                if (((fill >> (8 * l)) & 0xffu) != 0u) src = l;
+        if (src < 0 && k >= nk) {
+            if (flushing) break;
+            flushing = true;
+            continue;
+        }
+        T cr, ci, zr, zi, a, b, m = 0, szr, szi;
+        int32_t cnt;
+        uint32_t pix, lvl, n0, cyc_tc = 0u, cyc_win = 1u;
+        bool valid = true;
+        if (src >= 0) {
+            __builtin_amdgcn_fence(__ATOMIC_ACQUIRE, "workgroup");
+            const uint32_t have = (fill >> (8 * src)) & 0xffu, take = have < 64u ? have : 64u;
+            fill = uniform_u32(fill - (take << (8 * src)));
+            const uint32_t lane = __lane_id();
+            valid = lane < take;
+            const uint32_t slot = (have - take + lane) & (kPackCap - 1u);
+            const char *pool = slice + 64u + (uint32_t)src * kPackLevelBytes;
+            zr = zi = szr = szi = 0;
+            pix = 0u;
+            if (valid) {
+                zr = reinterpret_cast<const T *>(pool)[slot];
+                zi = reinterpret_cast<const T *>(pool + 8u * kPackCap)[slot];
+                if (kCycle) {
+                    szr = reinterpret_cast<const T *>(pool + 16u * kPackCap)[slot];
+                    szi = reinterpret_cast<const T *>(pool + 24u * kPackCap)[slot];
+                }
+                pix = reinterpret_cast<const uint32_t *>(pool + 32u * kPackCap)[slot];
+            }
+            if (kCycle) {
+                cyc_tc = uniform_u32(hdr[2 * src]);
+                cyc_win = uniform_u32(hdr[2 * src + 1]);
+            }
+            const uint32_t lc = ((pix >> 6) & 0x7ffu) * 8u + (pix & 7u), lr = (pix >> 17) * 8u + ((pix >> 3) & 7u);
+            pack_coords<T>(p.col0 + lc, p.row0 + lr, cr, ci);
+            a = zr * zr;
+            b = zi * zi;
+            cnt = valid ? 0 : 1;
+            lvl = (uint32_t)src + 1u;
+            n0 = first + (p.pack_first << src);
+        } else {
+            const uint32_t e = scalar_load_u32(p.order, 2u * n + 2u - (e0 + k));
+            ++k;
+            const uint32_t by = e >> 16, bx = e & 0xffffu;
+            const uint32_t lane = __lane_id();
+            pix = (by << 17) | (bx << 6) | lane;
+            pack_coords<T>(p.col0 + bx * 8u + (lane & 7u), p.row0 + by * 8u + (lane >> 3), cr, ci);
+            bool risky = false;
+            if (p.ring_possible != 0u) {
+                const T c2 = cr * cr + ci * ci;
+                const T margin = sizeof(T) == 8 ? (T)1e-9 : (T)1e-3;
+                risky = __ballot(__builtin_fabs((double)(c2 - (T)4)) < (double)margin) != 0ull;
+            }
+            zr = cr;
+            zi = ci;
+            a = zr * zr;
+            b = zi * zi;
+            cnt = 0;
+            if (risky) {
+                cnt = escape_count_asm<true>(cr, ci, p.mrd);
+                lvl = kPackLevels;
+                n0 = total;
+            } else {
+                escape_steps_asm<true>(cr, ci, zr, zi, a, b, m, cnt, 0u, first);
+                lvl = 0u;
+                n0 = first;
+            }
+            szr = zr;
+            szi = zi;
+        }
+        bool pushed = false;
+        for (;;) {
+            uint32_t stop = total;
+            if (lvl < kPackLevels) {
+                const uint32_t cp = first + (p.pack_first << lvl);
+                stop = cp < total ? cp : total;
+            }
+            if (stop > n0) {
+                if (cnt == 0) {
+                    if (kCycle) escape_steps_carry<8>(cr, ci, zr, zi, a, b, m, cnt, n0, stop, p.cyc_window, szr, szi, cyc_tc, cyc_win);
+                    else escape_steps_tail<8, false, false>(cr, ci, zr, zi, a, b, m, cnt, n0, stop);
+                }
+                if (kCycle) {
+                    cyc_tc = uniform_u32(cyc_tc);
+                    cyc_win = uniform_u32(cyc_win);
+                }
+            }
+            const unsigned long long alive = __ballot(cnt == 0);
+            const uint32_t ka = (uint32_t)__popcll(alive);
+            if (stop >= total || ka == 0u) break;
+            if (ka == 64u) {
+                n0 = stop;
+                ++lvl;
+                continue;
+            }
+            const uint32_t have = (fill >> (8 * lvl)) & 0xffu;
+            char *pool = slice + 64u + lvl * kPackLevelBytes;
+            if (cnt == 0) {
+                const uint32_t rank = __builtin_amdgcn_mbcnt_hi((uint32_t)(alive >> 32), __builtin_amdgcn_mbcnt_lo((uint32_t)alive, 0u));
+                const uint32_t slot = (have + rank) & (kPackCap - 1u);
+                reinterpret_cast<T *>(pool)[slot] = zr;
+                reinterpret_cast<T *>(pool + 8u * kPackCap)[slot] = zi;
+                if (kCycle) {
+                    reinterpret_cast<T *>(pool + 16u * kPackCap)[slot] = szr;
+                    reinterpret_cast<T *>(pool + 24u * kPackCap)[slot] = szi;
+                    if (rank == 0u) {
+                        hdr[2u * lvl] = cyc_tc;
+                        hdr[2u * lvl + 1u] = cyc_win;
+                    }
+                }
+                reinterpret_cast<uint32_t *>(pool + 32u * kPackCap)[slot] = pix;
+            }
+            fill = uniform_u32(fill + (ka << (8 * lvl)));
+            pushed = true;
+            break;
+        }
+        if (pushed) __builtin_amdgcn_fence(__ATOMIC_RELEASE, "workgroup");
+        const bool pooled = pushed && cnt == 0;
+        escape_fixup(cr, ci, zr, zi, a, b, m, cnt);
+        if (valid && !pooled) {
+            const int32_t count = (kCycle && cnt == -1) ? 0 : cnt;
+            const uint32_t lc = ((pix >> 6) & 0x7ffu) * 8u + (pix & 7u), lr = (pix >> 17) * 8u + ((pix >> 3) & 7u);
+            const size_t o = (size_t)(lr + p.out_row0) * p.out_pitch + lc + p.out_col0;
+            if (kCounts) p.counts[o] = count;
+            if (kBytes) p.bytes[o] = quantise(count, p);
+            if (kStats) heavy += count > 0 ? (unsigned long long)(uint32_t)count : (1ull << 47) + never_cap;
+        }
+    }
+}
+
+template <typename T, int kGroup, bool kCycle, bool kCounts, bool kBytes, bool kStats = false, bool kPack = false>
 __global__ __launch_bounds__(64) __attribute__((amdgpu_waves_per_eu(8, 8))) void tile_units_kernel(TileArgs args, uint32_t qtab)
 {
     static_assert(!kStats || (!kCounts && kBytes), "fused statistics exist for the bytes-only instantiation");
@@ -228,6 +432,10 @@
         if (!units_lookup(u, hmin, lmin, h_x, l_x, hbase_x, lbase_x, is_h, i)) break;
         if (is_h || i < n_m) {
             const bool late = is_h && i < n_ml;
+            if (kPack && late) {
+                packed_job<T, kCycle, kCounts, kBytes, kStats>(p, i, scalar_load_u32(args.plan, kPlanWords), heavy, never_cap);
+                continue;
+            }
             const uint32_t e = scalar_load_u32(p.order, is_h ? (late ? 2u * n + 2u - i : (i < hs0 ? i - n_ml : (uint32_t)units_settled_base(n) + (i - hs0)))
                                                               : n + 3u + i);
             const uint32_t by = e >> 16, bx = e & 0xffffu;
diff --git a/distributedmandelbrot_amd/device.py b/distributedmandelbrot_amd/device.py
--- a/distributedmandelbrot_amd/device.py
+++ b/distributedmandelbrot_amd/device.py
@@ -415,6 +415,11 @@
         self._check(self._lib.mbk_get_option(self._h, L.MBK_INFO_SPILL + 1, C.byref(b)))
         return {"lanes_last_launch": int(a.value), "launches": int(b.value)}
 
+    def pack_launches(self) -> int:
+        v = C.c_uint32(0)
+        self._check(self._lib.mbk_get_option(self._h, L.MBK_INFO_PACK, C.byref(v)))
+        return int(v.value)
+
     def quantise_counts(self, counts: np.ndarray, mrd: int) -> np.ndarray:
         counts = np.ascontiguousarray(counts, dtype=np.int32)
         out = np.empty(counts.shape, np.uint8)
diff --git a/include/mbk.h b/include/mbk.h
--- a/include/mbk.h
+++ b/include/mbk.h
@@ -374,16 +374,20 @@
     MBK_OPT_SPILL_MIN_MRD,
     MBK_OPT_SPILL_MIN_BLOCKS,
     MBK_OPT_SPILL_CYC_SHIFT,
+    MBK_OPT_PACK,
     MBK_OPT_COUNT_
 };
 #define MBK_INFO_SCAN_WG_PER_CU 100
 #define MBK_INFO_XCD_SHARE 110
 #define MBK_INFO_SPILL 130
+#define MBK_INFO_PACK 140
 int mbk_set_option(mbk_ctx *ctx, int option, uint32_t value);
 int mbk_get_option(mbk_ctx *ctx, int option, uint32_t *value);
 
 int mbk_units_plan(uint32_t n_h, uint32_t n_v, uint32_t n_m, const double *fractions, uint32_t *plan);
 int mbk_units_lookup(const uint32_t *plan, uint32_t id, uint32_t *list, uint32_t *index);
+int mbk_units_pack(const uint8_t *classes, uint32_t blocks_x, uint32_t blocks_y, uint32_t fast_bx_end, uint32_t fast_by_end, uint32_t pack,
+                   uint32_t pack_g, uint8_t *filed, uint32_t *order, uint32_t *n_packed, uint32_t *n_jobs);
 
 int mbk_quantise_counts(mbk_ctx *ctx, const int32_t *h_counts, uint64_t n, uint32_t mrd, uint8_t *h_bytes);
 
```
